# facebookresearch/faiss

Hardware: NVIDIA B200
Metric: queries/sec (GpuIndexFlatL2 exact k-NN, recall@k = 1) (higher is better)
Workload: dtype f16 mma (fp32 accumulate) + f32 exact re-rank

## Files before the change

faiss_b200/__init__.py:

```python
import ctypes
import json
import os

import numpy as np

from ._lib import lib, check, FaissError

METRIC_INNER_PRODUCT = 0
METRIC_L2 = 1

_c_f = ctypes.POINTER(ctypes.c_float)
_c_i64 = ctypes.POINTER(ctypes.c_int64)
_c_u8 = ctypes.POINTER(ctypes.c_uint8)


def _is_torch(x):
    return type(x).__module__.startswith("torch")


def _ptr(x, ctype):
    if x is None:
        return ctypes.cast(None, ctype)
    if _is_torch(x):
        assert x.is_contiguous(), "tensor must be contiguous"
        return ctypes.cast(x.data_ptr(), ctype)
    assert x.flags["C_CONTIGUOUS"], "array must be C-contiguous"
    return x.ctypes.data_as(ctype)


def _as_f32(x):
    if _is_torch(x):
        import torch

        assert x.dtype == torch.float32
        return x.contiguous()
    return np.ascontiguousarray(x, dtype=np.float32)


def _as_i64(x):
    if x is None:
        return None
    if _is_torch(x):
        import torch

        assert x.dtype == torch.int64
        return x.contiguous()
    return np.ascontiguousarray(x, dtype=np.int64)


def _empty_like_residency(x, shape, dtype):
    if _is_torch(x) and x.is_cuda:
        import torch

        tdt = {np.float32: torch.float32, np.int64: torch.int64}[dtype]
        return torch.empty(shape, dtype=tdt, device=x.device)
    return np.empty(shape, dtype=dtype)


class StandardGpuResources:

    def __init__(self):
        self._h = ctypes.c_void_p()
        check(lib.faiss_StandardGpuResources_new(ctypes.byref(self._h)))

    def __del__(self):
        if getattr(self, "_h", None) and lib is not None:
            lib.faiss_StandardGpuResources_free(self._h)
            self._h = None

    def noTempMemory(self):
        check(lib.faiss_StandardGpuResources_noTempMemory(self._h))

    def setTempMemory(self, size):
        check(lib.faiss_StandardGpuResources_setTempMemory(self._h, ctypes.c_size_t(size)))

    def setPinnedMemory(self, size):
        check(lib.faiss_StandardGpuResources_setPinnedMemory(self._h, ctypes.c_size_t(size)))

    def setDefaultStream(self, device, stream):
        check(lib.faiss_StandardGpuResources_setDefaultStream(self._h, int(device), ctypes.c_void_p(int(stream))))

    def setDefaultNullStreamAllDevices(self):
        check(lib.faiss_StandardGpuResources_setDefaultNullStreamAllDevices(self._h))

    def getDefaultStream(self, device):
        out = ctypes.c_void_p()
        check(lib.faiss_StandardGpuResources_getDefaultStream(self._h, int(device), ctypes.byref(out)))
        return out.value or 0

    def syncDefaultStream(self, device):
        check(lib.faiss_StandardGpuResources_syncDefaultStream(self._h, int(device)))

    def getMemoryInfo(self):
        buf = ctypes.create_string_buffer(1 << 16)
        check(lib.faiss_StandardGpuResources_getMemoryInfo(self._h, buf, ctypes.c_size_t(len(buf))))
        raw = json.loads(buf.value.decode())
        return {int(d): {k: tuple(v) for k, v in m.items()} for d, m in raw.items()}

    def ncclInitAll(self, devices):
        arr = (ctypes.c_int * len(devices))(*[int(d) for d in devices])
        check(lib.faiss_StandardGpuResources_ncclInitAll(self._h, len(devices), arr))

    def ncclInitRank(self, device, nranks, rank, unique_id):
        unique_id = bytes(unique_id)
        assert len(unique_id) == 128
        check(lib.faiss_StandardGpuResources_ncclInitRank(self._h, int(device), int(nranks), int(rank), unique_id))

    def ncclRank(self, device):
        r, n = ctypes.c_int(), ctypes.c_int()
        check(lib.faiss_StandardGpuResources_ncclRank(self._h, int(device), ctypes.byref(r), ctypes.byref(n)))
        return r.value, n.value

    def getTempMemoryAvailable(self, device):
        out = ctypes.c_size_t()
        check(lib.faiss_StandardGpuResources_getTempMemoryAvailable(self._h, int(device), ctypes.byref(out)))
        return out.value


class Index:

    def __init__(self):
        self._h = ctypes.c_void_p()
        self._keep = []

    def __del__(self):
        if getattr(self, "_h", None) and lib is not None:
            lib.faiss_Index_free(self._h)
            self._h = None

    def _use_torch_stream(self, *tensors):
        for t in tensors:
            if t is not None and _is_torch(t) and t.is_cuda:
                import torch

                dev = t.device.index if t.device.index is not None else torch.cuda.current_device()
                for r in self._resources():
                    r.setDefaultStream(dev, torch.cuda.current_stream(dev).cuda_stream)
                return

    def _resources(self):
        return [r for r in self._keep if isinstance(r, StandardGpuResources)]

    @property
    def d(self):
        return lib.faiss_Index_d(self._h)

    @property
    def ntotal(self):
        return lib.faiss_Index_ntotal(self._h)

    @property
    def is_trained(self):
        return bool(lib.faiss_Index_is_trained(self._h))

    @property
    def metric_type(self):
        return lib.faiss_Index_metric_type(self._h)

    @property
    def verbose(self):
        return bool(lib.faiss_Index_verbose(self._h))

    @verbose.setter
    def verbose(self, v):
        lib.faiss_Index_set_verbose(self._h, int(bool(v)))

    def _check_x(self, x):
        x = _as_f32(x)
        assert x.ndim == 2 and x.shape[1] == self.d, "x must be [n, d=%d], got %s" % (self.d, tuple(x.shape))
        return x

    def train(self, x):
        x = self._check_x(x)
        self._use_torch_stream(x)
        check(lib.faiss_Index_train(self._h, ctypes.c_int64(x.shape[0]), _ptr(x, _c_f)))

    def add(self, x):
        x = self._check_x(x)
        self._use_torch_stream(x)
        check(lib.faiss_Index_add(self._h, ctypes.c_int64(x.shape[0]), _ptr(x, _c_f)))

    def add_with_ids(self, x, ids):
        x = self._check_x(x)
        ids = _as_i64(ids)
        assert ids.shape == (x.shape[0],)
        self._use_torch_stream(x, ids)
        check(lib.faiss_Index_add_with_ids(self._h, ctypes.c_int64(x.shape[0]), _ptr(x, _c_f), _ptr(ids, _c_i64)))

    def setMinPagingSize(self, size):
        check(lib.faiss_GpuIndex_setMinPagingSize(self._h, ctypes.c_size_t(size)))

    def getMinPagingSize(self):
        out = ctypes.c_size_t()
        check(lib.faiss_GpuIndex_getMinPagingSize(self._h, ctypes.byref(out)))
        return int(out.value)

    def search(self, x, k, D=None, I=None, params=None):
        x = self._check_x(x)
        n = x.shape[0]
        if D is None:
            D = _empty_like_residency(x, (n, k), np.float32)
        if I is None:
            I = _empty_like_residency(x, (n, k), np.int64)
        self._use_torch_stream(x, D, I)
        if params is not None:
            check(
                lib.faiss_Index_search_with_params(
                    self._h, ctypes.c_int64(n), _ptr(x, _c_f), ctypes.c_int64(k), params._h, _ptr(D, _c_f), _ptr(I, _c_i64)
                )
            )
            return D, I
        check(
            lib.faiss_Index_search(
                self._h, ctypes.c_int64(n), _ptr(x, _c_f), ctypes.c_int64(k), _ptr(D, _c_f), _ptr(I, _c_i64)
            )
        )
        return D, I

    def assign(self, x, k=1):
        x = self._check_x(x)
        n = x.shape[0]
        I = _empty_like_residency(x, (n, k), np.int64)
        self._use_torch_stream(x)
        check(lib.faiss_Index_assign(self._h, ctypes.c_int64(n), _ptr(x, _c_f), _ptr(I, _c_i64), ctypes.c_int64(k)))
        return I

    def reset(self):
        check(lib.faiss_Index_reset(self._h))

    def reconstruct(self, key):
        out = np.empty(self.d, dtype=np.float32)
        check(lib.faiss_Index_reconstruct(self._h, ctypes.c_int64(key), _ptr(out, _c_f)))
        return out

    def reconstruct_n(self, i0=0, ni=-1):
        if ni < 0:
            ni = self.ntotal - i0
        out = np.empty((ni, self.d), dtype=np.float32)
        check(lib.faiss_Index_reconstruct_n(self._h, ctypes.c_int64(i0), ctypes.c_int64(ni), _ptr(out, _c_f)))
        return out

    def reconstruct_batch(self, keys):
        keys = _as_i64(np.asarray(keys))
        out = np.empty((keys.shape[0], self.d), dtype=np.float32)
        check(lib.faiss_Index_reconstruct_batch(self._h, ctypes.c_int64(keys.shape[0]), _ptr(keys, _c_i64), _ptr(out, _c_f)))
        return out

    def compute_residual(self, x, key):
        x = _as_f32(x).reshape(1, -1)
        return self.compute_residual_n(x, np.array([key], dtype=np.int64))[0]

    def compute_residual_n(self, x, keys):
        x = self._check_x(x)
        keys = _as_i64(keys)
        out = _empty_like_residency(x, tuple(x.shape), np.float32)
        self._use_torch_stream(x, keys)
        check(
            lib.faiss_Index_compute_residual_n(
                self._h, ctypes.c_int64(x.shape[0]), _ptr(x, _c_f), _ptr(out, _c_f), _ptr(keys, _c_i64)
            )
        )
        return out


class SearchParametersIVF:

    def __init__(self, nprobe=1, max_codes=0):
        self._h = ctypes.c_void_p()
        check(lib.faiss_SearchParametersIVF_new_with(ctypes.byref(self._h), ctypes.c_size_t(int(nprobe)), ctypes.c_size_t(int(max_codes))))

    def __del__(self):
        if getattr(self, "_h", None) and lib is not None:
            lib.faiss_SearchParameters_free(self._h)
            self._h = None


_INTERRUPT_CB = None


def set_interrupt_callback(fn):
    global _INTERRUPT_CB
    proto = ctypes.CFUNCTYPE(ctypes.c_int, ctypes.c_void_p)
    if fn is None:
        lib.faiss_b200_set_interrupt_callback(ctypes.cast(None, proto), None)
        _INTERRUPT_CB = None
        return
    _INTERRUPT_CB = proto(lambda _ctx: 1 if fn() else 0)
    lib.faiss_b200_set_interrupt_callback(_INTERRUPT_CB, None)


class GpuIndexFlat(Index):

    def __init__(self, res, d, metric=METRIC_L2, device=0, use_tensor_cores=True, use_float16=False):
        super().__init__()
        self._keep.append(res)
        check(
            lib.faiss_GpuIndexFlat_new_with_config(
                ctypes.byref(self._h), res._h, int(d), int(metric), int(device), int(bool(use_tensor_cores)),
                int(bool(use_float16)),
            )
        )

    def copyFrom(self, xb):
        xb = _as_f32(xb)
        check(lib.faiss_GpuIndexFlat_copyFrom(self._h, ctypes.c_int64(xb.shape[0]), _ptr(xb, _c_f)))

    def copyTo(self):
        out = np.empty((self.ntotal, self.d), dtype=np.float32)
        check(lib.faiss_GpuIndexFlat_copyTo(self._h, _ptr(out, _c_f)))
        return out

    def setUseTensorCores(self, enable):
        check(lib.faiss_GpuIndexFlat_setUseTensorCores(self._h, int(bool(enable))))

    def lastSearchInfo(self):
        out = (ctypes.c_int * 2)()
        check(lib.faiss_GpuIndexFlat_lastSearchInfo(self._h, out))
        return {"tensor_cores": int(out[0]), "fallback_queries": int(out[1])}


class GpuIndexFlatL2(GpuIndexFlat):
    def __init__(self, res, d, device=0, use_tensor_cores=True, use_float16=False):
        super().__init__(res, d, METRIC_L2, device, use_tensor_cores, use_float16)


class GpuIndexFlatIP(GpuIndexFlat):
    def __init__(self, res, d, device=0, use_tensor_cores=True, use_float16=False):
        super().__init__(res, d, METRIC_INNER_PRODUCT, device, use_tensor_cores, use_float16)


class GpuIndexIVF(Index):

    @property
    def nprobe(self):
        return lib.faiss_GpuIndexIVF_nprobe(self._h)

    @nprobe.setter
    def nprobe(self, v):
        check(lib.faiss_GpuIndexIVF_set_nprobe(self._h, ctypes.c_size_t(int(v))))

    @property
    def nlist(self):
        return lib.faiss_GpuIndexIVF_nlist(self._h)

    def setClustering(self, niter=-1, seed=-1, max_points_per_centroid=-1):
        check(lib.faiss_GpuIndexIVF_set_clustering(self._h, int(niter), int(seed), int(max_points_per_centroid)))

    def reserveMemory(self, n):
        check(lib.faiss_GpuIndexIVF_reserveMemory(self._h, ctypes.c_size_t(int(n))))

    def reclaimMemory(self):
        out = ctypes.c_size_t()
        check(lib.faiss_GpuIndexIVF_reclaimMemory(self._h, ctypes.byref(out)))
        return out.value

    def getListLength(self, l):
        return lib.faiss_GpuIndexIVF_get_list_size(self._h, ctypes.c_size_t(int(l)))

    def _code_size(self):
        raise NotImplementedError

    def getListVectorData(self, l):
        n = self.getListLength(l)
        out = np.empty(n * self._code_size(), dtype=np.uint8)
        check(lib.faiss_GpuIndexIVF_getListVectorData(self._h, ctypes.c_size_t(int(l)), _ptr(out, _c_u8)))
        return out

    def getListIndices(self, l):
        n = self.getListLength(l)
        out = np.empty(n, dtype=np.int64)
        check(lib.faiss_GpuIndexIVF_getListIndices(self._h, ctypes.c_size_t(int(l)), _ptr(out, _c_i64)))
        return out

    def setCoarseCentroids(self, c):
        c = _as_f32(c)
        assert tuple(c.shape) == (self.nlist, self.d)
        check(lib.faiss_GpuIndexIVF_setCoarseCentroids(self._h, _ptr(c, _c_f)))

    def getCoarseCentroids(self):
        out = np.empty((self.nlist, self.d), dtype=np.float32)
        check(lib.faiss_GpuIndexIVF_getCoarseCentroids(self._h, _ptr(out, _c_f)))
        return out

    def setList(self, l, codes, ids):
        codes = np.ascontiguousarray(codes, dtype=np.uint8).reshape(-1)
        ids = np.ascontiguousarray(ids, dtype=np.int64)
        assert codes.size == ids.size * self._code_size()
        check(
            lib.faiss_GpuIndexIVF_setList(
                self._h, ctypes.c_size_t(int(l)), ctypes.c_int64(ids.size), _ptr(codes, _c_u8), _ptr(ids, _c_i64)
            )
        )

    def setListSizes(self, lens):
        lens = np.ascontiguousarray(lens, dtype=np.int64)
        assert lens.shape == (self.nlist,)
        check(lib.faiss_GpuIndexIVF_setListSizes(self._h, _ptr(lens, _c_i64)))

    def setIsTrained(self, v=True):
        check(lib.faiss_GpuIndexIVF_set_is_trained(self._h, int(bool(v))))

    def search_preassigned(self, x, k, assign, centroid_dis=None):
        x = self._check_x(x)
        n = x.shape[0]
        assign = _as_i64(assign)
        if centroid_dis is None:
            centroid_dis = np.zeros(assign.shape, dtype=np.float32)
            if _is_torch(x) and x.is_cuda:
                import torch

                centroid_dis = torch.zeros(tuple(assign.shape), dtype=torch.float32, device=x.device)
        centroid_dis = _as_f32(centroid_dis)
        D = _empty_like_residency(x, (n, k), np.float32)
        I = _empty_like_residency(x, (n, k), np.int64)
        self._use_torch_stream(x, assign)
        check(
            lib.faiss_GpuIndexIVF_search_preassigned(
                self._h,
                ctypes.c_int64(n),
                _ptr(x, _c_f),
                ctypes.c_int64(k),
                _ptr(assign, _c_i64),
                _ptr(centroid_dis, _c_f),
                _ptr(D, _c_f),
                _ptr(I, _c_i64),
            )
        )
        return D, I


class GpuIndexIVFFlat(GpuIndexIVF):

    def __init__(self, res, d, nlist, metric=METRIC_L2, device=0, quantizer=None):
        super().__init__()
        self._keep.append(res)
        if quantizer is not None:
            self._keep.append(quantizer)
            check(
                lib.faiss_GpuIndexIVFFlat_new_with_quantizer(
                    ctypes.byref(self._h), res._h, quantizer._h, int(d), ctypes.c_int64(nlist), int(metric), int(device)
                )
            )
            return
        check(
            lib.faiss_GpuIndexIVFFlat_new(
                ctypes.byref(self._h), res._h, int(d), ctypes.c_int64(nlist), int(metric), int(device)
            )
        )

    def _code_size(self):
        return 4 * self.d


class GpuIndexIVFPQ(GpuIndexIVF):

    def __init__(self, res, d, nlist, M, nbits=8, metric=METRIC_L2, device=0, quantizer=None):
        super().__init__()
        self._keep.append(res)
        self.M = int(M)
        if quantizer is not None:
            self._keep.append(quantizer)
            check(
                lib.faiss_GpuIndexIVFPQ_new_with_quantizer(
                    ctypes.byref(self._h), res._h, quantizer._h, int(d), ctypes.c_int64(nlist), ctypes.c_int64(M), ctypes.c_int64(nbits),
                    int(metric), int(device),
                )
            )
            return
        check(
            lib.faiss_GpuIndexIVFPQ_new(
                ctypes.byref(self._h),
                res._h,
                int(d),
                ctypes.c_int64(nlist),
                ctypes.c_int64(M),
                ctypes.c_int64(nbits),
                int(metric),
                int(device),
            )
        )

    def _code_size(self):
        return self.M

    def setPQCentroids(self, c):
        c = _as_f32(c)
        assert c.size == 256 * self.d
        check(lib.faiss_GpuIndexIVFPQ_setPQCentroids(self._h, _ptr(c, _c_f)))

    def getPQCentroids(self):
        out = np.empty((self.M, 256, self.d // self.M), dtype=np.float32)
        check(lib.faiss_GpuIndexIVFPQ_getPQCentroids(self._h, _ptr(out, _c_f)))
        return out

    def setPQClustering(self, niter=-1, seed=-1, max_points_per_centroid=-1):
        check(lib.faiss_GpuIndexIVFPQ_set_pq_clustering(self._h, int(niter), int(seed), int(max_points_per_centroid)))

    def setPrecomputedCodes(self, enable):
        check(lib.faiss_GpuIndexIVFPQ_setPrecomputedCodes(self._h, int(bool(enable))))


class IndexShards(Index):

    def __init__(self, d, threaded=False, successive_ids=True):
        super().__init__()
        check(
            lib.faiss_IndexShards_new_with_options(
                ctypes.byref(self._h), ctypes.c_int64(d), int(bool(threaded)), int(bool(successive_ids))
            )
        )
        self._shards = []

    def add_shard(self, index):
        check(lib.faiss_IndexShards_add_shard(self._h, index._h))
        self._shards.append(index)

    def _resources(self):
        out = []
        for s in self._shards:
            out.extend(s._resources())
        return out

    def remove_shard(self, index):
        check(lib.faiss_IndexShards_remove_shard(self._h, index._h))
        self._shards.remove(index)

    def at(self, i):
        return self._shards[i]

    def count(self):
        return len(self._shards)

    def lastSearchPath(self):
        return {0: "host", 1: "nccl"}.get(lib.faiss_IndexShards_lastSearchPath(self._h), "?")

    def __del__(self):
        if getattr(self, "_h", None) and lib is not None:
            lib.faiss_Index_free(self._h)
            self._h = None
        self._shards = []


class IndexShardsIVF(IndexShards):

    def __init__(self, quantizer, nlist, threaded=False, successive_ids=True):
        Index.__init__(self)
        self._keep.append(quantizer)
        check(lib.faiss_IndexShardsIVF_new(ctypes.byref(self._h), quantizer._h, ctypes.c_int64(nlist), int(bool(threaded)), int(bool(successive_ids))))
        self._shards = []

    def add_shard(self, index):
        check(lib.faiss_IndexShardsIVF_add_shard(self._h, index._h))
        self._shards.append(index)


def nccl_unique_id():
    buf = ctypes.create_string_buffer(128)
    check(lib.faiss_b200_nccl_unique_id(buf))
    return buf.raw


class DistributedIndexShards(Index):

    def __init__(self, res, local, successive_ids=True):
        super().__init__()
        self._keep.append(res)
        self._local = local
        check(lib.faiss_DistributedIndexShards_new(ctypes.byref(self._h), res._h, local._h, int(bool(successive_ids))))

    def _resources(self):
        return [r for r in self._keep if isinstance(r, StandardGpuResources)]

    def sync(self):
        check(lib.faiss_DistributedIndexShards_sync(self._h))

    def info(self):
        r, n, o = ctypes.c_int(), ctypes.c_int(), ctypes.c_int64()
        check(lib.faiss_DistributedIndexShards_info(self._h, ctypes.byref(r), ctypes.byref(n), ctypes.byref(o)))
        return {"rank": r.value, "world": n.value, "id_offset": o.value}

    def __del__(self):
        if getattr(self, "_h", None) and lib is not None:
            lib.faiss_Index_free(self._h)
            self._h = None
        self._local = None


def kmeans(res, x, k, niter=25, seed=1234, max_points_per_centroid=256, device=0):
    x = _as_f32(x)
    n, d = x.shape
    cent = np.empty((k, d), dtype=np.float32)
    obj = np.zeros(niter, dtype=np.float32)
    check(
        lib.faiss_b200_kmeans(
            res._h,
            int(device),
            ctypes.c_size_t(d),
            ctypes.c_size_t(n),
            ctypes.c_size_t(k),
            _ptr(x, _c_f),
            int(niter),
            int(seed),
            int(max_points_per_centroid),
            _ptr(cent, _c_f),
            _ptr(obj, _c_f),
        )
    )
    return cent, obj


def kmeans_ex(res, x, k, niter=25, seed=1234, max_points_per_centroid=256, metric=METRIC_L2, spherical=False, device=0):
    x = _as_f32(x)
    n, d = x.shape
    cent = np.empty((k, d), dtype=np.float32)
    obj = np.zeros(niter, dtype=np.float32)
    check(
        lib.faiss_b200_kmeans_ex(
            res._h, int(device), ctypes.c_size_t(d), ctypes.c_size_t(n), ctypes.c_size_t(k), _ptr(x, _c_f), int(niter), int(seed),
            int(max_points_per_centroid), int(metric), int(bool(spherical)), _ptr(cent, _c_f), _ptr(obj, _c_f),
        )
    )
# ... 147 lines not shown
```

faiss_b200/csrc/c_api.cu:

```cuda
#include <cstring>
#include <sstream>

#include "comm.h"
#include "faiss_b200_c.h"
#include "index.h"

using namespace fb200;

static thread_local std::string g_last_error;

#define CATCH_AND_HANDLE                              \
    catch (const fb200::FaissException& e) {          \
        g_last_error = e.what();                      \
        return -2;                                    \
    }                                                 \
    catch (const std::exception& e) {                 \
        g_last_error = e.what();                      \
        return -4;                                    \
    }                                                 \
    catch (...) {                                     \
        g_last_error = "unknown exception";           \
        return -1;                                    \
    }                                                 \
    return 0;

struct FaissStandardGpuResources_H {
    std::shared_ptr<StandardGpuResources> res;
};
struct FaissIndex_H {
    Index* index;
    std::shared_ptr<StandardGpuResources> res;
};

static Index* IX(const FaissIndex* p) {
    if (!p || !p->index)
        FB_THROW_MSG("null index handle");
    return p->index;
}
template <typename T>
static T* AS(const FaissIndex* p, const char* what) {
    T* t = dynamic_cast<T*>(IX(p));
    if (!t)
        FB_THROW_FMT("index handle is not a %s", what);
    return t;
}
static std::shared_ptr<StandardGpuResources> RES(FaissStandardGpuResources* r) {
    if (!r || !r->res)
        FB_THROW_MSG("null resources handle");
    return r->res;
}
static MetricType MT(FaissMetricType m) {
    if (m != ::METRIC_L2 && m != ::METRIC_INNER_PRODUCT)
        FB_THROW_MSG("unsupported metric type");
    return m == ::METRIC_L2 ? fb200::METRIC_L2 : fb200::METRIC_INNER_PRODUCT;
}

extern "C" {

const char* faiss_get_last_error(void) {
    return g_last_error.c_str();
}
const char* faiss_b200_version(void) {
    return "faiss_b200 0.1 (sm_100a)";
}

int faiss_StandardGpuResources_new(FaissStandardGpuResources** p) {
    try {
        auto* h = new FaissStandardGpuResources_H();
        h->res = std::make_shared<StandardGpuResources>();
        *p = h;
    }
    CATCH_AND_HANDLE
}
void faiss_StandardGpuResources_free(FaissStandardGpuResources* r) {
    delete r;
}
int faiss_StandardGpuResources_noTempMemory(FaissStandardGpuResources* r) {
    try {
        RES(r)->noTempMemory();
    }
    CATCH_AND_HANDLE
}
int faiss_StandardGpuResources_setTempMemory(FaissStandardGpuResources* r, size_t size) {
    try {
        RES(r)->setTempMemory(size);
    }
    CATCH_AND_HANDLE
}
int faiss_StandardGpuResources_setPinnedMemory(FaissStandardGpuResources* r, size_t size) {
    try {
        RES(r)->setPinnedMemory(size);
    }
    CATCH_AND_HANDLE
}
int faiss_StandardGpuResources_setDefaultStream(FaissStandardGpuResources* r, int device, void* stream) {
    try {
        RES(r)->setDefaultStream(device, (cudaStream_t)stream);
    }
    CATCH_AND_HANDLE
}
int faiss_StandardGpuResources_setDefaultNullStreamAllDevices(FaissStandardGpuResources* r) {
    try {
        RES(r)->setDefaultNullStreamAllDevices();
    }
    CATCH_AND_HANDLE
}
int faiss_StandardGpuResources_getDefaultStream(FaissStandardGpuResources* r, int device, void** out) {
    try {
        *out = (void*)RES(r)->getDefaultStream(device);
    }
    CATCH_AND_HANDLE
}
int faiss_StandardGpuResources_syncDefaultStream(FaissStandardGpuResources* r, int device) {
    try {
        DeviceScope s(device);
        RES(r)->syncDefaultStream(device);
    }
    CATCH_AND_HANDLE
}
int faiss_StandardGpuResources_getMemoryInfo(FaissStandardGpuResources* r, char* buf, size_t buflen) {
    try {
        auto info = RES(r)->getMemoryInfo();
        std::ostringstream os;
        os << "{";
        bool firstD = true;
        for (auto& dv : info) {
            if (!firstD)
                os << ",";
            firstD = false;
            os << "\"" << dv.first << "\":{";
            bool first = true;
            for (auto& kv : dv.second) {
                if (!first)
                    os << ",";
                first = false;
                os << "\"" << kv.first << "\":[" << kv.second.first << "," << kv.second.second << "]";
            }
            os << "}";
        }
        os << "}";
        std::string s = os.str();
        FB_THROW_IF_NOT_MSG(s.size() + 1 <= buflen, "buffer too small");
        memcpy(buf, s.c_str(), s.size() + 1);
    }
    CATCH_AND_HANDLE
}
int faiss_StandardGpuResources_getTempMemoryAvailable(FaissStandardGpuResources* r, int device, size_t* out) {
    try {
        RES(r)->initializeForDevice(device);
        *out = RES(r)->getTempMemoryAvailable(device);
    }
    CATCH_AND_HANDLE
}

void faiss_Index_free(FaissIndex* p) {
    if (p) {
        delete p->index;
        delete p;
    }
}
int faiss_Index_d(const FaissIndex* p) {
    return p && p->index ? p->index->d : 0;
}
int faiss_Index_is_trained(const FaissIndex* p) {
    return p && p->index ? (int)p->index->is_trained : 0;
}
idx_t faiss_Index_ntotal(const FaissIndex* p) {
    return p && p->index ? p->index->ntotal : 0;
}
FaissMetricType faiss_Index_metric_type(const FaissIndex* p) {
    return p && p->index && p->index->metric_type == fb200::METRIC_INNER_PRODUCT ? ::METRIC_INNER_PRODUCT : ::METRIC_L2;
}
int faiss_Index_verbose(const FaissIndex* p) {
    return p && p->index ? (int)p->index->verbose : 0;
}
void faiss_Index_set_verbose(FaissIndex* p, int v) {
    if (p && p->index)
        p->index->verbose = v != 0;
}
int faiss_Index_train(FaissIndex* p, idx_t n, const float* x) {
    try {
        IX(p)->train(n, x);
    }
    CATCH_AND_HANDLE
}
int faiss_Index_add(FaissIndex* p, idx_t n, const float* x) {
    try {
        IX(p)->add(n, x);
    }
    CATCH_AND_HANDLE
}
int faiss_Index_add_with_ids(FaissIndex* p, idx_t n, const float* x, const idx_t* xids) {
    try {
        IX(p)->add_with_ids(n, x, xids);
    }
    CATCH_AND_HANDLE
}
int faiss_Index_search(const FaissIndex* p, idx_t n, const float* x, idx_t k, float* D, idx_t* I) {
    try {
        IX(p)->search(n, x, k, D, I);
    }
    CATCH_AND_HANDLE
}
int faiss_Index_assign(FaissIndex* p, idx_t n, const float* x, idx_t* labels, idx_t k) {
    try {
        IX(p)->assign(n, x, labels, k);
    }
    CATCH_AND_HANDLE
}
int faiss_Index_reset(FaissIndex* p) {
    try {
        IX(p)->reset();
    }
    CATCH_AND_HANDLE
}
int faiss_Index_reconstruct(const FaissIndex* p, idx_t key, float* out) {
    try {
        IX(p)->reconstruct(key, out);
    }
    CATCH_AND_HANDLE
}
int faiss_Index_reconstruct_n(const FaissIndex* p, idx_t i0, idx_t ni, float* out) {
    try {
        IX(p)->reconstruct_n(i0, ni, out);
    }
    CATCH_AND_HANDLE
}
int faiss_Index_reconstruct_batch(const FaissIndex* p, idx_t n, const idx_t* keys, float* out) {
    try {
        IX(p)->reconstruct_batch(n, keys, out);
    }
    CATCH_AND_HANDLE
}
int faiss_Index_compute_residual(const FaissIndex* p, const float* x, float* r, idx_t key) {
    try {
        IX(p)->compute_residual(x, r, key);
    }
    CATCH_AND_HANDLE
}
int faiss_Index_compute_residual_n(const FaissIndex* p, idx_t n, const float* x, float* r, const idx_t* keys) {
    try {
        IX(p)->compute_residual_n(n, x, r, keys);
    }
    CATCH_AND_HANDLE
}

int faiss_GpuIndexFlat_new(
        FaissGpuIndex** p,
        FaissStandardGpuResources* r,
        int d,
        FaissMetricType metric,
        int device,
        int use_tc) {
    try {
        GpuIndexFlatConfig c;
        c.device = device;
        c.useTensorCores = use_tc != 0;
        auto res = RES(r);
        auto* h = new FaissIndex_H();
        h->res = res;
        h->index = new GpuIndexFlat(res, d, MT(metric), c);
        *p = h;
    }
    CATCH_AND_HANDLE
}
int faiss_GpuIndexFlat_new_with_config(
        FaissGpuIndex** p,
        FaissStandardGpuResources* r,
        int d,
        FaissMetricType metric,
        int device,
        int use_tc,
        int use_float16) {
    try {
        GpuIndexFlatConfig c;
        c.device = device;
        c.useTensorCores = use_tc != 0;
        c.useFloat16 = use_float16 != 0;
        auto res = RES(r);
        auto* h = new FaissIndex_H();
        h->res = res;
        h->index = new GpuIndexFlat(res, d, MT(metric), c);
        *p = h;
    }
    CATCH_AND_HANDLE
}
int faiss_GpuIndexFlatL2_new(FaissGpuIndex** p, FaissStandardGpuResources* r, int d, int device) {
    return faiss_GpuIndexFlat_new(p, r, d, ::METRIC_L2, device, 1);
}
int faiss_GpuIndexFlatIP_new(FaissGpuIndex** p, FaissStandardGpuResources* r, int d, int device) {
    return faiss_GpuIndexFlat_new(p, r, d, ::METRIC_INNER_PRODUCT, device, 1);
}
int faiss_GpuIndexFlat_copyFrom(FaissGpuIndex* p, idx_t n, const float* xb) {
    try {
        AS<GpuIndexFlat>(p, "GpuIndexFlat")->copyFrom(n, xb);
    }
    CATCH_AND_HANDLE
}
int faiss_GpuIndexFlat_copyTo(const FaissGpuIndex* p, float* out) {
    try {
        AS<GpuIndexFlat>(p, "GpuIndexFlat")->copyTo(out);
    }
    CATCH_AND_HANDLE
}
int faiss_GpuIndex_setMinPagingSize(FaissGpuIndex* p, size_t size) {
    try {
        AS<GpuIndex>(p, "GpuIndex")->setMinPagingSize(size);
    }
    CATCH_AND_HANDLE
}
int faiss_GpuIndex_getMinPagingSize(const FaissGpuIndex* p, size_t* out) {
    try {
        *out = AS<GpuIndex>(p, "GpuIndex")->getMinPagingSize();
    }
    CATCH_AND_HANDLE
}
int faiss_GpuIndexFlat_setUseTensorCores(FaissGpuIndex* p, int enable) {
    try {
        AS<GpuIndexFlat>(p, "GpuIndexFlat")->setUseTensorCores(enable != 0);
    }
    CATCH_AND_HANDLE
}
int faiss_GpuIndexFlat_lastSearchInfo(const FaissGpuIndex* p, int* out2) {
    try {
        auto* f = AS<GpuIndexFlat>(p, "GpuIndexFlat");
        out2[0] = f->lastSearchUsedTensorCores;
        out2[1] = f->lastSearchFallbackQueries;
    }
    CATCH_AND_HANDLE
}

int faiss_GpuIndexIVF_set_nprobe(FaissGpuIndex* p, size_t nprobe) {
    try {
        AS<GpuIndexIVF>(p, "GpuIndexIVF")->nprobe = nprobe;
    }
    CATCH_AND_HANDLE
}
size_t faiss_GpuIndexIVF_nprobe(const FaissGpuIndex* p) {
    auto* i = p ? dynamic_cast<GpuIndexIVF*>(p->index) : nullptr;
    return i ? i->nprobe : 0;
}
size_t faiss_GpuIndexIVF_nlist(const FaissGpuIndex* p) {
    auto* i = p ? dynamic_cast<GpuIndexIVF*>(p->index) : nullptr;
    return i ? (size_t)i->nlist : 0;
}
int faiss_GpuIndexIVF_set_clustering(FaissGpuIndex* p, int niter, int seed, int maxppc) {
    try {
        auto* i = AS<GpuIndexIVF>(p, "GpuIndexIVF");
        if (niter > 0)
            i->cp.niter = niter;
        if (seed >= 0)
            i->cp.seed = seed;
        if (maxppc > 0)
            i->cp.max_points_per_centroid = maxppc;
    }
    CATCH_AND_HANDLE
}
int faiss_GpuIndexIVF_reserveMemory(FaissGpuIndex* p, size_t n) {
    try {
        AS<GpuIndexIVF>(p, "GpuIndexIVF")->reserveMemory(n);
    }
    CATCH_AND_HANDLE
}
int faiss_GpuIndexIVF_reclaimMemory(FaissGpuIndex* p, size_t* out) {
    try {
        size_t r = AS<GpuIndexIVF>(p, "GpuIndexIVF")->reclaimMemory();
        if (out)
            *out = r;
    }
    CATCH_AND_HANDLE
}
size_t faiss_GpuIndexIVF_get_list_size(const FaissGpuIndex* p, size_t l) {
    auto* i = p ? dynamic_cast<GpuIndexIVF*>(p->index) : nullptr;
    if (!i || (idx_t)l >= i->nlist)
        return 0;
    return (size_t)i->getListLength((idx_t)l);
}
int faiss_GpuIndexIVF_getListVectorData(const FaissGpuIndex* p, size_t l, uint8_t* out) {
    try {
        auto v = AS<GpuIndexIVF>(p, "GpuIndexIVF")->getListVectorData((idx_t)l);
        if (!v.empty())
            memcpy(out, v.data(), v.size());
    }
    CATCH_AND_HANDLE
}
int faiss_GpuIndexIVF_getListIndices(const FaissGpuIndex* p, size_t l, idx_t* out) {
    try {
        auto v = AS<GpuIndexIVF>(p, "GpuIndexIVF")->getListIndices((idx_t)l);
        if (!v.empty())
            memcpy(out, v.data(), v.size() * sizeof(idx_t));
    }
    CATCH_AND_HANDLE
}
int faiss_GpuIndexIVF_setCoarseCentroids(FaissGpuIndex* p, const float* c) {
    try {
        AS<GpuIndexIVF>(p, "GpuIndexIVF")->setCoarseCentroids(c);
    }
    CATCH_AND_HANDLE
}
int faiss_GpuIndexIVF_getCoarseCentroids(const FaissGpuIndex* p, float* out) {
    try {
        AS<GpuIndexIVF>(p, "GpuIndexIVF")->getCoarseCentroids(out);
    }
    CATCH_AND_HANDLE
}
int faiss_GpuIndexIVF_setList(FaissGpuIndex* p, size_t l, idx_t len, const uint8_t* codes, const idx_t* ids) {
    try {
        AS<GpuIndexIVF>(p, "GpuIndexIVF")->setList((idx_t)l, len, codes, ids);
    }
    CATCH_AND_HANDLE
}
int faiss_GpuIndexIVF_setListSizes(FaissGpuIndex* p, const idx_t* lens) {
    try {
        AS<GpuIndexIVF>(p, "GpuIndexIVF")->setListSizes(lens);
    }
    CATCH_AND_HANDLE
}
int faiss_GpuIndexIVF_set_is_trained(FaissGpuIndex* p, int v) {
    try {
        AS<GpuIndexIVF>(p, "GpuIndexIVF")->is_trained = v != 0;
    }
    CATCH_AND_HANDLE
}
int faiss_GpuIndexIVF_search_preassigned(
        const FaissGpuIndex* p,
        idx_t n,
        const float* x,
        idx_t k,
        const idx_t* assign,
        const float* cdis,
        float* D,
        idx_t* I) {
    try {
        AS<GpuIndexIVF>(p, "GpuIndexIVF")->search_preassigned(n, x, k, assign, cdis, D, I);
    }
    CATCH_AND_HANDLE
}
int faiss_GpuIndexIVFFlat_new(
        FaissGpuIndex** p,
        FaissStandardGpuResources* r,
        int d,
        idx_t nlist,
        FaissMetricType metric,
        int device) {
    try {
        GpuIndexIVFConfig c;
        c.device = device;
        auto res = RES(r);
        auto* h = new FaissIndex_H();
        h->res = res;
        h->index = new GpuIndexIVFFlat(res, d, nlist, MT(metric), c);
        *p = h;
    }
    CATCH_AND_HANDLE
}

int faiss_GpuIndexIVFPQ_new(
        FaissGpuIndex** p,
        FaissStandardGpuResources* r,
        int d,
        idx_t nlist,
        idx_t M,
        idx_t nbits,
        FaissMetricType metric,
        int device) {
    try {
        GpuIndexIVFPQConfig c;
        c.device = device;
        auto res = RES(r);
        auto* h = new FaissIndex_H();
        h->res = res;
        h->index = new GpuIndexIVFPQ(res, d, nlist, M, nbits, MT(metric), c);
        *p = h;
    }
    CATCH_AND_HANDLE
}
int faiss_GpuIndexIVFPQ_setPQCentroids(FaissGpuIndex* p, const float* c) {
    try {
        AS<GpuIndexIVFPQ>(p, "GpuIndexIVFPQ")->setPQCentroids(c);
    }
    CATCH_AND_HANDLE
}
int faiss_GpuIndexIVFPQ_getPQCentroids(const FaissGpuIndex* p, float* out) {
    try {
        AS<GpuIndexIVFPQ>(p, "GpuIndexIVFPQ")->getPQCentroids(out);
    }
    CATCH_AND_HANDLE
}
int faiss_GpuIndexIVFPQ_set_pq_clustering(FaissGpuIndex* p, int niter, int seed, int maxppc) {
    try {
        auto* i = AS<GpuIndexIVFPQ>(p, "GpuIndexIVFPQ");
        if (niter > 0)
            i->pq_cp.niter = niter;
        if (seed >= 0)
            i->pq_cp.seed = seed;
        if (maxppc > 0)
            i->pq_cp.max_points_per_centroid = maxppc;
    }
    CATCH_AND_HANDLE
}
int faiss_GpuIndexIVFPQ_setPrecomputedCodes(FaissGpuIndex* p, int enable) {
    try {
        AS<GpuIndexIVFPQ>(p, "GpuIndexIVFPQ")->setPrecomputedCodes(enable != 0);
    }
    CATCH_AND_HANDLE
}

int faiss_IndexShards_new(FaissIndexShards** p, idx_t d) {
    return faiss_IndexShards_new_with_options(p, d, 0, 1);
}
int faiss_IndexShards_new_with_options(FaissIndexShards** p, idx_t d, int threaded, int successive_ids) {
    try {
        auto* h = new FaissIndex_H();
        h->index = new IndexShards((int)d, threaded != 0, successive_ids != 0);
        *p = h;
    }
    CATCH_AND_HANDLE
}
int faiss_IndexShards_add_shard(FaissIndexShards* p, FaissIndex* shard) {
    try {
        AS<IndexShards>(p, "IndexShards")->add_shard(IX(shard));
    }
    CATCH_AND_HANDLE
}
int faiss_IndexShards_remove_shard(FaissIndexShards* p, FaissIndex* shard) {
    try {
        AS<IndexShards>(p, "IndexShards")->remove_shard(IX(shard));
    }
    CATCH_AND_HANDLE
}
FaissIndex* faiss_IndexShards_at(FaissIndexShards*, int) {
    return nullptr;
}
int faiss_IndexShards_own_indices(const FaissIndexShards* p) {
    auto* s = p ? dynamic_cast<IndexShards*>(p->index) : nullptr;
    return s ? (int)s->own_indices : 0;
}
void faiss_IndexShards_set_own_indices(FaissIndexShards* p, int v) {
    (void)p;
    (void)v;
}
int faiss_IndexShards_successive_ids(const FaissIndexShards* p) {
    auto* s = p ? dynamic_cast<IndexShards*>(p->index) : nullptr;
    return s ? (int)s->successive_ids : 0;
}
void faiss_IndexShards_set_successive_ids(FaissIndexShards* p, int v) {
    auto* s = p ? dynamic_cast<IndexShards*>(p->index) : nullptr;
    if (s)
        s->successive_ids = v != 0;
}

struct FaissSearchParameters_H {
    SearchParameters* p;
};
int faiss_SearchParametersIVF_new_with(FaissSearchParametersIVF** out, size_t nprobe, size_t max_codes) {
    try {
        auto* sp = new SearchParametersIVF();
        sp->nprobe = nprobe;
        sp->max_codes = max_codes;
        *out = new FaissSearchParameters_H{sp};
    }
    CATCH_AND_HANDLE
}
void faiss_SearchParameters_free(FaissSearchParameters* p) {
    if (p) {
        delete p->p;
        delete p;
    }
}
int faiss_Index_search_with_params(
        const FaissIndex* p, idx_t n, const float* x, idx_t k, const FaissSearchParameters* params, float* D, idx_t* I) {
    try {
        Index* ix = IX(p);
        if (!params || !params->p) {
            ix->search(n, x, k, D, I);
        } else if (auto* g = dynamic_cast<GpuIndex*>(ix)) {
            g->search(n, x, k, D, I, params->p);
        } else {
            FB_THROW_MSG("search parameters are only supported on GPU indexes");
        }
    }
    CATCH_AND_HANDLE
}
void faiss_b200_set_interrupt_callback(int (*want_interrupt)(void*), void* ctx) {
    InterruptCallback::set(want_interrupt, ctx);
}
int faiss_GpuIndexIVFFlat_new_with_quantizer(
        FaissGpuIndex** p, FaissStandardGpuResources* r, FaissGpuIndex* coarse, int d, idx_t nlist, FaissMetricType metric, int device) {
    try {
        auto res = RES(r);
        GpuIndexIVFConfig cfg;
        cfg.device = device;
        auto* h = new FaissIndex_H{nullptr, res};
        try {
            h->index = new GpuIndexIVFFlat(res, AS<GpuIndexFlat>(coarse, "GpuIndexFlat"), d, nlist, MT(metric), cfg);
        } catch (...) {
            delete h;
            throw;
        }
        *p = h;
    }
    CATCH_AND_HANDLE
}
int faiss_GpuIndexIVFPQ_new_with_quantizer(
        FaissGpuIndex** p,
        FaissStandardGpuResources* r,
        FaissGpuIndex* coarse,
        int d,
        idx_t nlist,
        idx_t M,
        idx_t nbits,
        FaissMetricType metric,
        int device) {
    try {
        auto res = RES(r);
        GpuIndexIVFPQConfig cfg;
        cfg.device = device;
        auto* h = new FaissIndex_H{nullptr, res};
        try {
            h->index = new GpuIndexIVFPQ(res, AS<GpuIndexFlat>(coarse, "GpuIndexFlat"), d, nlist, M, nbits, MT(metric), cfg);
        } catch (...) {
            delete h;
            throw;
        }
        *p = h;
    }
    CATCH_AND_HANDLE
}

int faiss_b200_nccl_unique_id(char* out128) {
// ... 543 lines not shown
```

faiss_b200/csrc/flat_tc.cu:

```cuda
#include <cuda_fp16.h>

#include <cfloat>
#include <cmath>
#include <cub/cub.cuh>
#include <cstdlib>
#include <mutex>
#include <string>
#include <vector>

#include "comm.h"
#include "kernels.h"
#include "select.cuh"
#include "tc_ptx.cuh"
#include "flat_tc_kernel.cuh"

namespace fb200 {

void runMergeTopKKeyspace(
        const float*, const idx_t*, int64_t, int, int, int, MetricType, int64_t, float*, idx_t*, cudaStream_t);

namespace {

using namespace tc;

// ... 397 lines not shown
        }
    }
    if (lane == 0) {
        thr[q] = tNew;
        if (overflow)
            flags[q] = 1;
    }
}

__global__ void tc_pooled_thr_kernel(int nq, const float* __restrict__ contrib, const float* __restrict__ eps, float* __restrict__ thr) {
    const int q = blockIdx.x * blockDim.x + threadIdx.x;
    if (q >= nq)
        return;
    const float T = fmaxf(contrib[q], -contrib[nq + q]);
    if (T > -CUDART_INF_F) {
        const float t = nextafterf(T - eps[q], -CUDART_INF_F);
        thr[q] = fmaxf(thr[q], t);
    }
}

template <bool IS_L2, bool YH>
__global__ void tc_rerank_kernel(
        int nq,
        int d,
        int k,
        int LIST,
        int KL,
        const float* __restrict__ Q,
        const void* __restrict__ Y,
        const int* __restrict__ perm,
        const int* __restrict__ baseId,
        const float* __restrict__ baseKey,
        const float* __restrict__ thr,
        float* __restrict__ outD,
        idx_t* __restrict__ outI) {
    extern __shared__ __align__(16) unsigned char smem_raw[];
    const int warp = threadIdx.x >> 5;
    const int lane = lane_id();
    const int q = blockIdx.x * (blockDim.x >> 5) + warp;
    if (q >= nq)
        return;
    constexpr int BUF = 64;
    unsigned char* base = smem_raw + SmemTopK<int>::bytes(KL, BUF) * warp;
    WarpTopK<int> w;
    w.init(reinterpret_cast<float*>(base), reinterpret_cast<int*>(base + sizeof(float) * (KL + BUF)), KL, BUF, k);
    const float* qp = Q + (int64_t)q * d;
    const int* bi = baseId + (int64_t)q * LIST;
    const float tq = thr ? thr[q] : -CUDART_INF_F;
    for (int e0 = 0; e0 < LIST; e0 += 32) {
        int id = bi[e0 + lane];
        const bool present = id != IdLimits<int>::max();
        bool valid = present;
        if (valid && thr)
            valid = -baseKey[(int64_t)q * LIST + e0 + lane] > tq;
        if (valid && perm)
            id = perm[id];
        float acc = 0.f;
        if (valid) {
            const int64_t yo = (int64_t)id * d;
            int i = 0;
            if ((d & 3) == 0) {
#pragma unroll 8
                for (; i < d; i += 4) {
                    const float4 a4 = *reinterpret_cast<const float4*>(qp + i);
                    const float4 b4 = row_load4<YH>(Y, yo + i);
                    const float aa[4] = {a4.x, a4.y, a4.z, a4.w};
                    const float bb[4] = {b4.x, b4.y, b4.z, b4.w};
#pragma unroll
                    for (int u = 0; u < 4; u++) {
                        if (IS_L2) {
                            float df = aa[u] - bb[u];
                            acc = fmaf(df, df, acc);
                        } else {
                            acc = fmaf(aa[u], bb[u], acc);
                        }
                    }
                }
            }
            for (; i < d; i++) {
                float a = qp[i], b = row_load1<YH>(Y, yo + i);
                if (IS_L2) {
                    float df = a - b;
                    acc = fmaf(df, df, acc);
                } else {
                    acc = fmaf(a, b, acc);
                }
            }
            if (!IS_L2)
                acc = -acc;
        }
        if (!__any_sync(kFullMask, present))
            break;
        w.add(valid, acc, id);
    }
    w.finish();
    for (int j = lane; j < k; j += 32) {
        int id = w.q.ids[j];
        bool ok = id != IdLimits<int>::max();
        float key = w.q.keys[j];
        outD[(int64_t)q * k + j] = ok ? (IS_L2 ? key : -key) : (IS_L2 ? FLT_MAX : -FLT_MAX);
        outI[(int64_t)q * k + j] = ok ? (idx_t)id : -1;
    }
}

__global__ void tc_init_base_kernel(float* baseKey, int* baseId, int64_t count) {
    int64_t i = (int64_t)blockIdx.x * blockDim.x + threadIdx.x;
    if (i < count) {
        baseKey[i] = CUDART_INF_F;
        baseId[i] = IdLimits<int>::max();
    }
}

template <bool IS_L2, bool YH>
__global__ void tc_argmin_finish_kernel(
        int nq,
        int d,
        int slices,
        int parts,
        const uint2* __restrict__ cand,
        int cap,
        const int* __restrict__ candCount,
        const float* __restrict__ eps,
        const float* __restrict__ Q,
        const void* __restrict__ Y,
        const int* __restrict__ perm,
        float* __restrict__ outD,
        idx_t* __restrict__ outI,
        int* __restrict__ flags) {
    const int warp = threadIdx.x >> 5;
    const int lane = lane_id();
    const int q = blockIdx.x * (blockDim.x >> 5) + warp;
    if (q >= nq)
        return;
    const int pair = q / kPairM, prow = q % kPairM;
    const int qPairs = (nq + kPairM - 1) / kPairM;
    const int nseg = slices * parts;
    float m = -CUDART_INF_F;
    int overflow = 0;
    for (int si = 0; si < nseg; si++) {
        const int s = si / parts, h = si - s * parts;
        const long long seg = ((long long)(s * qPairs + pair) * kPairM + prow) * parts + h;
        int c = candCount[seg];
        if (c > cap) {
            overflow = 1;
            c = cap;
        }
        const uint2* sp = cand + seg * cap;
        for (int e = lane; e < c; e += 32)
            m = fmaxf(m, __uint_as_float(sp[e].x));
    }
#pragma unroll
    for (int o = 16; o > 0; o >>= 1)
        m = fmaxf(m, __shfl_xor_sync(kFullMask, m, o));
    const float t = nextafterf(m - 2.f * eps[q], -CUDART_INF_F);
    float bestD = CUDART_INF_F;
    int bestI = IdLimits<int>::max();
    const float* qp = Q + (int64_t)q * d;
    for (int si = 0; si < nseg; si++) {
        const int s = si / parts, h = si - s * parts;
        const long long seg = ((long long)(s * qPairs + pair) * kPairM + prow) * parts + h;
        const int c = min(candCount[seg], cap);
        const uint2* sp = cand + seg * cap;
        for (int e0 = 0; e0 < c; e0 += 32) {
            const int e = e0 + lane;
            const uint2 v = e < c ? sp[e] : make_uint2(0, 0);
            if (e < c && __uint_as_float(v.x) > t) {
                int id = (int)v.y;
                if (perm)
                    id = perm[id];
                const int64_t yo = (int64_t)id * d;
                float acc = 0.f;
                for (int i = 0; i < d; i++) {
                    const float a = qp[i], b = row_load1<YH>(Y, yo + i);
                    if (IS_L2) {
                        const float df = a - b;
                        acc = fmaf(df, df, acc);
                    } else {
                        acc = fmaf(a, b, acc);
                    }
                }
                if (!IS_L2)
                    acc = -acc;
                if (acc < bestD || (acc == bestD && id < bestI)) {
                    bestD = acc;
                    bestI = id;
                }
            }
        }
    }
#pragma unroll
    for (int o = 16; o > 0; o >>= 1) {
        const float od = __shfl_xor_sync(kFullMask, bestD, o);
        const int oi = __shfl_xor_sync(kFullMask, bestI, o);
        if (od < bestD || (od == bestD && oi < bestI)) {
            bestD = od;
            bestI = oi;
        }
    }
    if (lane == 0) {
        const bool ok = bestI != IdLimits<int>::max();
        outD[q] = ok ? (IS_L2 ? bestD : -bestD) : (IS_L2 ? FLT_MAX : -FLT_MAX);
        outI[q] = ok ? (idx_t)bestI : -1;
        if (overflow || !ok)
            flags[q] = 1;
    }
}

__global__ void tc_collect_flags_kernel(const int* flags, int nq, int* list, int* count) {
    int q = blockIdx.x * blockDim.x + threadIdx.x;
    if (q < nq && flags[q]) {
        int pos = atomicAdd(count, 1);
        list[pos] = q;
    }
}
__global__ void tc_gather_queries_kernel(const float* Q, const int* list, int d, float* out) {
    int i = blockIdx.x;
    int q = list[i];
    for (int j = threadIdx.x; j < d; j += blockDim.x)
        out[(int64_t)i * d + j] = Q[(int64_t)q * d + j];
}
__global__ void tc_scatter_results_kernel(
        const float* D,
        const idx_t* I,
        const int* list,
        int k,
        float* outD,
        idx_t* outI) {
    int i = blockIdx.x;
    int q = list[i];
    for (int j = threadIdx.x; j < k; j += blockDim.x) {
        outD[(int64_t)q * k + j] = D[(int64_t)i * k + j];
        outI[(int64_t)q * k + j] = I[(int64_t)i * k + j];
    }
}

typedef CUresult (*PFN_encodeTiled)(
        CUtensorMap*,
        CUtensorMapDataType,
        cuuint32_t,
        void*,
        const cuuint64_t*,
        const cuuint64_t*,
        const cuuint32_t*,
        const cuuint32_t*,
        CUtensorMapInterleave,
        CUtensorMapSwizzle,
        CUtensorMapL2promotion,
        CUtensorMapFloatOOBfill);

PFN_encodeTiled getEncodeTiled() {
    static PFN_encodeTiled fn = nullptr;
    static std::once_flag once;
    std::call_once(once, [] {
        void* p = nullptr;
        cudaDriverEntryPointQueryResult qres;
        cudaError_t err = cudaGetDriverEntryPoint("cuTensorMapEncodeTiled", &p, cudaEnableDefault, &qres);
        if (err == cudaSuccess && qres == cudaDriverEntryPointSuccess)
            fn = reinterpret_cast<PFN_encodeTiled>(p);
    });
    FB_THROW_IF_NOT_MSG(fn != nullptr, "cuTensorMapEncodeTiled not available from the driver");
    return fn;
}

CUtensorMap makeTileMap(const __half* base, int64_t rows, int dpad, int boxRows, int boxK = 0) {
    CUtensorMap m;
    cuuint64_t dims[3] = {(cuuint64_t)kKBlock, (cuuint64_t)rows, (cuuint64_t)(dpad / kKBlock)};
    cuuint64_t strides[2] = {(cuuint64_t)dpad * 2, (cuuint64_t)kKBlock * 2};
    cuuint32_t box[3] = {(cuuint32_t)kKBlock, (cuuint32_t)boxRows, (cuuint32_t)(boxK > 0 ? boxK : dpad / kKBlock)};
    cuuint32_t estr[3] = {1, 1, 1};
    CUresult r = getEncodeTiled()(
            &m,
            CU_TENSOR_MAP_DATA_TYPE_FLOAT16,
            3,
            const_cast<__half*>(base),
            dims,
            strides,
            box,
            estr,
            CU_TENSOR_MAP_INTERLEAVE_NONE,
            CU_TENSOR_MAP_SWIZZLE_128B,
            CU_TENSOR_MAP_L2_PROMOTION_L2_256B,
            CU_TENSOR_MAP_FLOAT_OOB_FILL_NONE);
    FB_THROW_IF_NOT_FMT(r == CUDA_SUCCESS, "cuTensorMapEncodeTiled failed with %d", (int)r);
    return m;
}

unsigned long long gcd64(unsigned long long a, unsigned long long b) {
    while (b) {
        unsigned long long t = a % b;
        a = b;
        b = t;
    }
    return a;
}

struct SmemPlan {
    int yStages;
    size_t bytes;
    int ksplit;
};

constexpr int kMaxKB = 4;

SmemPlan planSmem(int KB) {
    const size_t qtiles = (size_t)2 * KB * kTileM * kKBlock * 2;
    const size_t fixed = 1024  + 512  + qtiles;
    if (KB <= 2) {
        const size_t stage = (size_t)KB * kTileN * kKBlock * 2;
        const size_t budget = 220 * 1024;
        int ys = (int)std::min<size_t>(kMaxYStages, (budget - fixed) / stage);
        return {ys, fixed + ys * stage, 0};
    }
    FB_THROW_IF_NOT_MSG(KB <= kMaxKB, "dimension too large for the tensor-core Flat kernel");
    const size_t stage = (size_t)kTileN * kKBlock * 2;
    const size_t budget = 226 * 1024;
    int ys = (int)std::min<size_t>(kMaxYStages, (budget - fixed) / stage);
    FB_THROW_IF_NOT(ys >= 3);
    return {ys, fixed + ys * stage, 1};
}

int tcParts() {
    static const int parts = getenv("FB200_TC_PARTS") ? atoi(getenv("FB200_TC_PARTS")) : 4;
    return parts == 2 ? 2 : 4;
}

template <bool DUMP>
void launchTc(const CUtensorMap& mq, const CUtensorMap& my, const TcParams& p, int grid, size_t smem, cudaStream_t stream, bool self = false) {
    static const bool dbg = getenv("FB200_TC_DEBUG_SKIP") && atoi(getenv("FB200_TC_DEBUG_SKIP")) != 0;
    const int parts = tcParts();
    auto kern = parts == 2 ? (dbg ? flat_tc_kernel<DUMP, 1, 2> : flat_tc_kernel<DUMP, 0, 2>)
                           : (dbg ? flat_tc_kernel<DUMP, 1, 4> : flat_tc_kernel<DUMP, 0, 4>);
    if (self && !DUMP)
        kern = parts == 2 ? flat_tc_kernel<false, 0, 2, true> : flat_tc_kernel<false, 0, 4, true>;
    CUDA_VERIFY(cudaFuncSetAttribute(kern, cudaFuncAttributeMaxDynamicSharedMemorySize, (int)smem));
    KernelTiming::begin("flat_tc", stream);
    kern<<<grid, tcThreads(parts), smem, stream>>>(mq, my, p);
    KernelTiming::end("flat_tc", stream);
    CUDA_CHECK_LAST();
}

}

void runAbsMax(const void* x, int64_t count, float* out, cudaStream_t stream, int yHalf) {
    if (count == 0)
        return;
    int blocks = (int)std::min<int64_t>(1184, ceil_div(count, 256));
    absmax_kernel<<<blocks, 256, 0, stream>>>(x, yHalf, count, out);
    CUDA_CHECK_LAST();
}

void runMaxOf(const float* x, int64_t count, float* out, cudaStream_t stream) {
    runAbsMax(x, count, out, stream, 0);
}

void runFlatTcPrepareRows(
        GpuResources* res,
        int device,
        const void* Y,
        int64_t n,
        int d,
        int dpad,
        float scale,
        MetricType metric,
        __half* Y16,
        float* bias,
        int* perm,
        float* tileMaxBias,
        float* norms,
        cudaStream_t stream,
        int yHalf) {
    if (n == 0)
        return;
    const int warps = 8;
    const unsigned rowBlocks = (unsigned)ceil_div(n, warps);
    const int isL2 = metric == METRIC_L2 ? 1 : 0;
    tc_prepare_rows_kernel<<<rowBlocks, warps * 32, 0, stream>>>(Y, yHalf, n, d, dpad, scale, isL2, nullptr, nullptr, nullptr, norms);
    CUDA_CHECK_LAST();
    if (perm) {
        auto keysOut = res->temp(device, sizeof(float) * n);
        auto valsIn = res->temp(device, sizeof(int) * n);
        tc_iota_kernel<<<(unsigned)ceil_div(n, 256), 256, 0, stream>>>(valsIn.as<int>(), n);
        CUDA_CHECK_LAST();
        size_t tmpBytes = 0;
        CUDA_VERIFY(cub::DeviceRadixSort::SortPairs(
                nullptr, tmpBytes, norms, keysOut.as<float>(), valsIn.as<int>(), perm, (int)n, 0, 32, stream));
        auto tmp = res->temp(device, tmpBytes);
        CUDA_VERIFY(cub::DeviceRadixSort::SortPairs(
                tmp.data, tmpBytes, norms, keysOut.as<float>(), valsIn.as<int>(), perm, (int)n, 0, 32, stream));
    }
    tc_prepare_rows_kernel<<<rowBlocks, warps * 32, 0, stream>>>(Y, yHalf, n, d, dpad, scale, isL2, perm, Y16, bias, nullptr);
    CUDA_CHECK_LAST();
    const int64_t numTiles = ceil_div(n, kTileN);
    tc_tile_max_bias_kernel<<<(unsigned)ceil_div(numTiles, warps), warps * 32, 0, stream>>>(bias, numTiles, tileMaxBias);
    CUDA_CHECK_LAST();
}

bool flatTcSupported(int d, int k, int64_t n) {
    int dpad = (int)round_up(d, kKBlock);
    return dpad <= kMaxKB * kKBlock && k >= 1 && k <= 2048 && n >= (k == 1 ? 2048 : 32768) && n < (int64_t(1) << 31) - 512;
}

void runFlatTcScoresDebug(
        const __half* Q16,
        int64_t nq,
        const __half* Y16,
        int64_t n,
        int dpad,
        float* S,
        cudaStream_t stream) {
    FB_THROW_IF_NOT(dpad % kKBlock == 0 && dpad <= kMaxKB * kKBlock);
    const int KB = dpad / kKBlock;
    SmemPlan sp = planSmem(KB);
    CUtensorMap my = makeTileMap(Y16, n, dpad, kTileN, sp.ksplit);
    const int64_t numTiles = ceil_div(n, kTileN);
    const int64_t qPairs = ceil_div(nq, kPairM);
    __half* qpad = nullptr;
    CUDA_VERIFY(cudaMallocAsync(&qpad, sizeof(__half) * qPairs * kPairM * dpad, stream));
    CUDA_VERIFY(cudaMemsetAsync(qpad, 0, sizeof(__half) * qPairs * kPairM * dpad, stream));
    CUDA_VERIFY(cudaMemcpyAsync(qpad, Q16, sizeof(__half) * nq * dpad, cudaMemcpyDeviceToDevice, stream));
    float* one = nullptr;
    CUDA_VERIFY(cudaMallocAsync(&one, sizeof(float), stream));
    float h1 = 1.f;
    CUDA_VERIFY(cudaMemcpyAsync(one, &h1, sizeof(float), cudaMemcpyHostToDevice, stream));
    TcParams p{};
    p.slices = 1;
    p.qPairs = (int)qPairs;
    p.numUnits = (int)qPairs;
    CUtensorMap mq = makeTileMap(qpad, qPairs * kPairM, dpad, kTileM);
    p.tileBegin = 0;
    p.tileEnd = (int)numTiles;
    p.tilesPerSlice = (int)numTiles;
    p.permA = 1;
    p.permB = 0;
    p.numTiles = (unsigned long long)numTiles;
    p.KB = KB;
    p.ksplit = sp.ksplit;
    p.kSteps = dpad / 16;
    p.yStages = sp.yStages;
    p.invScalePtr = one;
    p.bias = nullptr;
    p.tileMaxBias = nullptr;
    p.thr = nullptr;
    p.cand = nullptr;
    p.cap = 0;
    p.candCount = nullptr;
    p.dump = S;
    p.dumpLd = numTiles * kTileN;
    p.nq = (int)nq;
    int dev = 0, sms = 0;
    CUDA_VERIFY(cudaGetDevice(&dev));
    CUDA_VERIFY(cudaDeviceGetAttribute(&sms, cudaDevAttrMultiProcessorCount, dev));
    launchTc<true>(mq, my, p, (int)std::min<int64_t>(p.numUnits, sms), sp.bytes, stream);
    CUDA_VERIFY(cudaFreeAsync(qpad, stream));
    CUDA_VERIFY(cudaFreeAsync(one, stream));
}

void runFlatTcSearch(
        GpuResources* res,
        int device,
        const float* Q,
        int64_t nqAll,
        const void* Y,
        const __half* Y16,
        const float* bias,
        const int* perm,
        const float* tileMaxBias,
        float yScale,
        float yMaxNorm,
        int64_t n,
        int d,
        int dpad,
        int k,
        MetricType metric,
        float* outD,
        idx_t* outI,
        cudaStream_t stream,
        const FlatTcShard* shard,
        int yHalf) {
    if (nqAll == 0)
        return;
    FB_THROW_IF_NOT(flatTcSupported(d, k, n));
    const int KB = dpad / kKBlock;
    const SmemPlan sp = planSmem(KB);
    const int sms = res->numSMs(device);
    const int64_t T = ceil_div(n, kTileN);
    const int nShards = shard ? shard->comm->size() : 1;
    const int64_t Tsched = shard ? std::max<int64_t>(T, shard->maxTiles) : T;
    const int kFrac = (k + nShards - 1) / nShards;
    const int LIST = std::max(128, next_pow2(2 * k));
    const int KL = std::max(64, next_pow2(k));

    unsigned long long A = (unsigned long long)((double)T * 0.6180339887498949);
    if (A < 1)
        A = 1;
    while (gcd64(A, (unsigned long long)T) != 1)
        A++;
    const unsigned long long B = (unsigned long long)(T / 3);

    const float c1 = 1.01f * (ldexpf(1.f, -10) + (float)dpad * ldexpf(1.f, -22));
    const float c2 = (float)(dpad + 16) * ldexpf(1.f, -24);

    CUtensorMap mapY = makeTileMap(Y16, n, dpad, kTileN, sp.ksplit);

    static const int r0Env = getenv("FB200_TC_R0") ? atoi(getenv("FB200_TC_R0")) : 0;
    int r0Tiles = std::max(r0Env > 0 ? r0Env : std::max(1, (40 * k + kTileN - 1) / kTileN), (k + 127) / 128 * 2);
    if (nShards > 1)
        r0Tiles = std::max<int>((r0Tiles + nShards - 1) / nShards, std::max(2, (2 * kFrac + kTileN - 1) / kTileN));
    static const bool selSortEnv = getenv("FB200_TC_SELECT") && std::string(getenv("FB200_TC_SELECT")) == "sort";
    const bool useBisect = LIST <= 256 && !selSortEnv;
    if (useBisect)
        r0Tiles = std::min(r0Tiles, std::max(2, kSelCap * 3 / 4 / kTileN));
    static const bool noStream = getenv("FB200_TC_NO_STREAM") && atoi(getenv("FB200_TC_NO_STREAM")) != 0;
    const bool streaming = k == 1 && !shard && !noStream;
    const int64_t kQFloor = r0Tiles > 64 ? 2048 : 16384;
    const int64_t kQBatch = streaming ? (int64_t)sms * kPairM * 4
                                      : std::min<int64_t>(131072, std::max<int64_t>(kQFloor, (int64_t)kPairM * 1024 / r0Tiles));
    for (int64_t qb = 0; qb < nqAll; qb += kQBatch) {
        const int64_t nq = std::min(kQBatch, nqAll - qb);
        const float* Qb = Q + qb * d;
        const int64_t qPairs = ceil_div(nq, kPairM);

        auto q16 = res->temp(device, sizeof(__half) * qPairs * kPairM * dpad);
        auto scal = res->temp(device, sizeof(float) * 4);
        auto eps = res->temp(device, sizeof(float) * nq);
        auto thr = res->temp(device, sizeof(float) * nq);
        auto flags = res->temp(device, sizeof(int) * (nq + 1));
        auto baseKey = res->temp(device, streaming ? sizeof(float) : sizeof(float) * nq * LIST);
        auto baseId = res->temp(device, streaming ? sizeof(int) : sizeof(int) * nq * LIST);

        CUDA_VERIFY(cudaMemsetAsync(scal.data, 0, sizeof(float) * 4, stream));
        CUDA_VERIFY(cudaMemsetAsync(flags.data, 0, sizeof(int) * (nq + 1), stream));
        CUDA_VERIFY(cudaMemsetAsync(q16.data, 0, sizeof(__half) * qPairs * kPairM * dpad, stream));
        float* sc = scal.as<float>();
        runAbsMax(Qb, nq * d, sc + 0, stream);
        tc_query_scale_kernel<<<1, 1, 0, stream>>>(sc + 0, yScale, sc + 1, sc + 2);
        CUDA_CHECK_LAST();
        tc_prepare_queries_kernel<<<(unsigned)ceil_div(nq, 8), 256, 0, stream>>>(
                Qb, nq, d, dpad, sc + 1, c1, c2, yMaxNorm, q16.as<__half>(), eps.as<float>(), thr.as<float>());
        CUDA_CHECK_LAST();
        if (!streaming) {
            int64_t cnt = nq * LIST;
            tc_init_base_kernel<<<(unsigned)ceil_div(cnt, 256), 256, 0, stream>>>(
                    baseKey.as<float>(), baseId.as<int>(), cnt);
            CUDA_CHECK_LAST();
        }

        struct Round {
            int begin, end, slices, tilesPerSlice, cap;
        };
        const int parts = tcParts();
        std::vector<Round> rounds;
        {
            int64_t seen = 0;
            while (seen < Tsched) {
                static const double gEarly = getenv("FB200_TC_G_EARLY") ? atof(getenv("FB200_TC_G_EARLY")) : 4.0;
                static const double gLate = getenv("FB200_TC_G_LATE") ? atof(getenv("FB200_TC_G_LATE")) : 4.0;
                static const int64_t lateFrom = getenv("FB200_TC_LATE_FROM") ? atol(getenv("FB200_TC_LATE_FROM")) : 8192;
                static const double gShard = getenv("FB200_TC_G_SHARD") ? atof(getenv("FB200_TC_G_SHARD")) : 8.0;
                const double g = nShards > 1 ? std::max(gEarly, std::min(gShard, 2.0 * nShards)) : (seen >= lateFrom ? gLate : gEarly);
                int64_t end = seen == 0 ? std::min<int64_t>(Tsched, r0Tiles)
                                        : std::min<int64_t>(Tsched, (int64_t)(seen * g));
                if (Tsched - end < end / 4)
                    end = Tsched;
                if (streaming)
                    end = Tsched;
                int64_t tiles = end - seen;
                int bestS = 1;
                double bestCost = 1e300;
                int64_t maxS = std::max<int64_t>(1, std::min<int64_t>(512, tiles / 8));
                for (int64_t S = 1; S <= maxS; S++) {
                    int64_t tps = ceil_div(tiles, S);
                    int64_t units = qPairs * ceil_div(tiles, tps);
                    int64_t waves = ceil_div(units, sms);
                    double cost = (double)waves * (double)(tps + 6);
                    if (cost < bestCost * 0.999) {
                        bestCost = cost;
                        bestS = (int)S;
                    }
                }
                int64_t tps = ceil_div(tiles, bestS);
                int S = (int)ceil_div(tiles, tps);
                int cap;
                if (streaming) {
                    cap = 64;
                } else if (seen == 0) {
                    cap = (int)(tps * (kTileN / parts));
                } else {
                    double expect = 1.5 * k * ((double)tps / (double)seen) / parts;
                    cap = next_pow2((int)std::min<double>(1 << 20, 4.0 * expect + 32.0));
                    cap = std::max(cap, 32);
                }
                rounds.push_back({(int)seen, (int)end, S, (int)tps, cap});
                seen = end;
            }
        }
        size_t arenaBytes = 0, countBytes = 0;
        for (auto& r : rounds) {
            size_t units = (size_t)qPairs * r.slices;
            arenaBytes = std::max(arenaBytes, units * tcSegsPerUnit(parts) * (size_t)r.cap * sizeof(uint2));
            countBytes = std::max(countBytes, units * tcSegsPerUnit(parts) * sizeof(int));
        }
        auto arena = res->temp(device, arenaBytes);
        auto counts = res->temp(device, countBytes);

        const int selWarps = (int)std::max<size_t>(1, std::min<size_t>(8, (48 * 1024) / SmemTopK<int>::bytes(LIST, kSelectBuf)));
        const size_t selSmem = SmemTopK<int>::bytes(LIST, kSelectBuf) * selWarps;
        CUDA_VERIFY(cudaFuncSetAttribute(tc_select_kernel, cudaFuncAttributeMaxDynamicSharedMemorySize, (int)selSmem));

        GpuMemoryReservation contrib;
        if (shard)
            contrib = res->temp(device, sizeof(float) * 2 * nq);
        for (auto& r : rounds) {
            TcParams p{};
            p.slices = r.slices;
            p.qPairs = (int)qPairs;
            p.numUnits = (int)(qPairs * r.slices);
            CUtensorMap mapQ = makeTileMap(q16.as<__half>(), qPairs * kPairM, dpad, kTileM);
            p.tileBegin = (int)std::min<int64_t>(r.begin, T);
            p.tileEnd = (int)std::min<int64_t>(r.end, T);
            p.tilesPerSlice = r.tilesPerSlice;
            p.permA = A;
            p.permB = B;
            p.numTiles = (unsigned long long)T;
            p.KB = KB;
            p.ksplit = sp.ksplit;
            p.kSteps = (d + 15) / 16;
            p.yStages = sp.yStages;
            p.invScalePtr = sc + 2;
            p.bias = bias;
            p.tileMaxBias = tileMaxBias;
            p.tileMinBias = tileMaxBias + T + 1;
            p.thr = thr.as<float>();
            p.eps = eps.as<float>();
            p.cand = arena.as<uint2>();
            p.cap = r.cap;
            p.candCount = counts.as<int>();
            p.dump = nullptr;
            p.dumpLd = 0;
            p.nq = (int)nq;
            if (p.tileBegin < p.tileEnd) {
                launchTc<false>(mapQ, mapY, p, std::min(p.numUnits, sms), sp.bytes, stream, streaming);
            } else {
                CUDA_VERIFY(cudaMemsetAsync(counts.data, 0, (size_t)p.numUnits * tcSegsPerUnit(parts) * sizeof(int), stream));
            }
            if (streaming) {
                const int fw = 8;
                float* oD1 = outD + qb;
                idx_t* oI1 = outI + qb;
                KernelTiming::begin("tc_argmin_finish", stream);
                auto launchFin = [&](auto kern) {
                    kern<<<(unsigned)ceil_div(nq, fw), fw * 32, 0, stream>>>(
                            (int)nq, d, r.slices, parts, arena.as<uint2>(), r.cap, counts.as<int>(), eps.as<float>(), Qb, Y, perm,
                            oD1, oI1, flags.as<int>());
                };
                if (metric == METRIC_L2)
                    yHalf ? launchFin(tc_argmin_finish_kernel<true, true>) : launchFin(tc_argmin_finish_kernel<true, false>);
                else
                    yHalf ? launchFin(tc_argmin_finish_kernel<false, true>) : launchFin(tc_argmin_finish_kernel<false, false>);
                KernelTiming::end("tc_argmin_finish", stream);
                CUDA_CHECK_LAST();
                continue;
            }
            KernelTiming::begin("tc_select", stream);
            if (useBisect) {
                const size_t bsmem = sizeof(uint2) * kSelCap * kSelWarps;
                CUDA_VERIFY(cudaFuncSetAttribute(tc_select_bisect_kernel, cudaFuncAttributeMaxDynamicSharedMemorySize, (int)bsmem));
                tc_select_bisect_kernel<<<(unsigned)ceil_div(nq, kSelWarps), kSelWarps * 32, bsmem, stream>>>(
                        (int)nq, k, LIST, r.slices, parts, arena.as<uint2>(), r.cap, counts.as<int>(), eps.as<float>(),
                        baseKey.as<float>(), baseId.as<int>(), thr.as<float>(), flags.as<int>(),
                        shard ? contrib.as<float>() : nullptr, kFrac);
            } else {
                tc_select_kernel<<<(unsigned)ceil_div(nq, selWarps), selWarps * 32, selSmem, stream>>>(
                        (int)nq,
                        k,
                        LIST,
                        r.slices,
                        parts,
                        arena.as<uint2>(),
                        r.cap,
                        counts.as<int>(),
                        eps.as<float>(),
                        baseKey.as<float>(),
                        baseId.as<int>(),
                        thr.as<float>(),
                        flags.as<int>(),
                        shard ? contrib.as<float>() : nullptr,
                        kFrac);
            }
            KernelTiming::end("tc_select", stream);
            CUDA_CHECK_LAST();
            if (shard) {
                KernelTiming::begin("tc_pool", stream);
                shard->comm->allReduceMax(contrib.as<float>(), (size_t)2 * nq, stream);
                tc_pooled_thr_kernel<<<(unsigned)ceil_div(nq, 256), 256, 0, stream>>>(
                        (int)nq, contrib.as<float>(), eps.as<float>(), thr.as<float>());
                KernelTiming::end("tc_pool", stream);
                CUDA_CHECK_LAST();
            }
        }

        if (!streaming) {
            const int rrWarps = (int)std::max<size_t>(1, std::min<size_t>(8, (48 * 1024) / SmemTopK<int>::bytes(KL, 64)));
            const size_t rrSmem = SmemTopK<int>::bytes(KL, 64) * rrWarps;
            float* oD = outD + qb * k;
            idx_t* oI = outI + qb * k;
            auto launchRr = [&](auto kern) {
                CUDA_VERIFY(cudaFuncSetAttribute(kern, cudaFuncAttributeMaxDynamicSharedMemorySize, (int)rrSmem));
                kern<<<(unsigned)ceil_div(nq, rrWarps), rrWarps * 32, rrSmem, stream>>>(
                        (int)nq, d, k, LIST, KL, Qb, Y, perm, baseId.as<int>(), baseKey.as<float>(),
                        shard ? thr.as<float>() : nullptr, oD, oI);
            };
            KernelTiming::begin("tc_rerank", stream);
            if (metric == METRIC_L2)
                yHalf ? launchRr(tc_rerank_kernel<true, true>) : launchRr(tc_rerank_kernel<true, false>);
            else
                yHalf ? launchRr(tc_rerank_kernel<false, true>) : launchRr(tc_rerank_kernel<false, false>);
            KernelTiming::end("tc_rerank", stream);
            CUDA_CHECK_LAST();
        }

        {
            auto list = res->temp(device, sizeof(int) * nq);
            int* countDev = flags.as<int>() + nq;
            tc_collect_flags_kernel<<<(unsigned)ceil_div(nq, 256), 256, 0, stream>>>(
                    flags.as<int>(), (int)nq, list.as<int>(), countDev);
            CUDA_CHECK_LAST();
            int nflag = 0;
            CUDA_VERIFY(cudaMemcpyAsync(&nflag, countDev, sizeof(int), cudaMemcpyDeviceToHost, stream));
            CUDA_VERIFY(cudaStreamSynchronize(stream));
            if (nflag > 0) {
                auto fq = res->temp(device, sizeof(float) * (size_t)nflag * d);
                auto fD = res->temp(device, sizeof(float) * (size_t)nflag * k);
                auto fI = res->temp(device, sizeof(idx_t) * (size_t)nflag * k);
                tc_gather_queries_kernel<<<nflag, 128, 0, stream>>>(Qb, list.as<int>(), d, fq.as<float>());
                CUDA_CHECK_LAST();
                runFlatExact(res, device, fq.as<float>(), nflag, Y, n, d, k, metric, 0, fD.as<float>(), fI.as<idx_t>(), stream, yHalf);
                tc_scatter_results_kernel<<<nflag, 128, 0, stream>>>(
                        fD.as<float>(), fI.as<idx_t>(), list.as<int>(), k, outD + qb * k, outI + qb * k);
                CUDA_CHECK_LAST();
                CUDA_VERIFY(cudaStreamSynchronize(stream));
            }
            lastFlatTcFallbacks() = nflag;
        }
    }
}

int& lastFlatTcFallbacks() {
    static thread_local int v = 0;
    return v;
}

}
```

faiss_b200/csrc/flat_tc_kernel.cuh:

```cuda
#pragma once

#include <cuda_fp16.h>

#include "select.cuh"
#include "tc_ptx.cuh"

namespace fb200 {
namespace tc {

constexpr int kTileM = 128;
constexpr int kPairM = 256;
constexpr int kTileN = 256;
constexpr int kKBlock = 64;
constexpr int kMaxParts = 4;
constexpr int kMaxYStages = 6;
__host__ __device__ constexpr int tcThreads(int parts) {
    return 64 + 128 * parts;
}
__host__ __device__ constexpr int tcSegsPerUnit(int parts) {
    return kPairM * parts;
}

struct TcParams {
    int numUnits;
    int slices;
    int qPairs;
    int tileBegin;
    int tileEnd;
    int tilesPerSlice;
    unsigned long long permA, permB, numTiles;
    int KB;
    int kSteps;
    int ksplit;
    int yStages;
    const float* invScalePtr;
    const float* bias;
    const float* tileMaxBias;
    const float* tileMinBias;
    const float* thr;
    const float* eps;
    uint2* cand;
    int cap;
    int* candCount;
    float* dump;
    long long dumpLd;
    int nq;
};

__device__ __forceinline__ int perm_tile(const TcParams& p, int pos) {
    return (int)(((unsigned long long)pos * p.permA + p.permB) % p.numTiles);
}

template <bool DUMP, bool SELF>
__device__ __forceinline__ void epi_filter32(
        const TcParams& p,
        const uint32_t (&r)[32],
        int q,
        long long colBase,
        float inv,
        float& thr,
        float slack,
        float maxb,
        uint2* buf,
        int& cnt,
        float minb = 0.f) {
    if (DUMP) {
        if (q < p.nq) {
            float* dst = p.dump + (long long)q * p.dumpLd + colBase;
#pragma unroll
            for (int j = 0; j < 32; j++)
                dst[j] = __uint_as_float(r[j]);
        }
        return;
    }
    float mg[4];
#pragma unroll
    for (int g = 0; g < 4; g++) {
        const int o = 8 * g;
        const float a = ptx::max3(__uint_as_float(r[o + 0]), __uint_as_float(r[o + 1]), __uint_as_float(r[o + 2]));
        const float c = ptx::max3(__uint_as_float(r[o + 3]), __uint_as_float(r[o + 4]), __uint_as_float(r[o + 5]));
        mg[g] = ptx::max3(a, c, fmaxf(__uint_as_float(r[o + 6]), __uint_as_float(r[o + 7])));
    }
    const float m = ptx::max3(mg[0], mg[1], fmaxf(mg[2], mg[3]));
    if (SELF) {
        thr = fmaxf(thr, nextafterf(fmaf(m, inv, minb) - slack, -CUDART_INF_F));
    }
    if (fmaf(m, inv, maxb) > thr) {
        const float* bias = p.bias + colBase;
        const unsigned rowBase = (unsigned)colBase;
#pragma unroll
        for (int g = 0; g < 4; g++) {
            if (fmaf(mg[g], inv, maxb) > thr) {
#pragma unroll
                for (int j = 8 * g; j < 8 * g + 8; j++) {
                    const float v = fmaf(__uint_as_float(r[j]), inv, __ldg(bias + j));
                    if (v > thr) {
                        if (cnt < p.cap)
                            buf[cnt] = make_uint2(__float_as_uint(v), rowBase + j);
                        cnt++;
                        if (SELF)
                            thr = fmaxf(thr, nextafterf(v - slack, -CUDART_INF_F));
                    }
                }
            }
        }
    }
}

template <bool DUMP, bool SELF>
__device__ __forceinline__ void epi_filter64(
        const TcParams& p,
        const uint32_t (&r0)[32],
        const uint32_t (&r1)[32],
        int q,
        long long colBase,
        float inv,
        float& thr,
        float slack,
        float maxb,
        uint2* buf,
        int& cnt,
        float minb = 0.f) {
    epi_filter32<DUMP, SELF>(p, r0, q, colBase, inv, thr, slack, maxb, buf, cnt, minb);
    epi_filter32<DUMP, SELF>(p, r1, q, colBase + 32, inv, thr, slack, maxb, buf, cnt, minb);
}

template <bool DUMP, int DBG, int PARTS, bool SELF = false>
__global__ void __launch_bounds__(tcThreads(PARTS), 1) flat_tc_kernel(
        const __grid_constant__ CUtensorMap mapQ,
        const __grid_constant__ CUtensorMap mapY,
        const TcParams p) {
    extern __shared__ unsigned char smem_dyn[];
    unsigned char* smem = reinterpret_cast<unsigned char*>(
            (reinterpret_cast<uintptr_t>(smem_dyn) + 1023) & ~uintptr_t(1023));
    const int qBytes = p.KB * kTileM * kKBlock * 2;
    const int stageBytes = (p.ksplit ? 1 : p.KB) * kTileN * kKBlock * 2;
    unsigned char* sQ = smem;
    unsigned char* sY = smem + 2 * qBytes;
    uint64_t* bars = reinterpret_cast<uint64_t*>(sY + (size_t)p.yStages * stageBytes);
    uint64_t* q_full = bars + 0;
    uint64_t* q_empty = bars + 1;
    uint64_t* y_full = bars + 2;
    uint64_t* y_empty = y_full + kMaxYStages;
    uint64_t* t_full = y_empty + kMaxYStages;
    uint64_t* t_empty = t_full + 2;
    uint32_t* tmem_slot = reinterpret_cast<uint32_t*>(t_empty + 2);

    const int warp = threadIdx.x >> 5;
    const int lane = threadIdx.x & 31;
    constexpr int kEpiWarps = 4 * PARTS;
    constexpr int kColsPerThread = kTileN / PARTS;

    if (warp == 0 && lane == 0) {
        ptx::prefetch_tensormap(&mapQ);
        ptx::prefetch_tensormap(&mapY);
        ptx::mbar_init(q_full, 1);
        ptx::mbar_init(q_empty, 1);
        for (int i = 0; i < p.yStages; i++) {
            ptx::mbar_init(&y_full[i], 1);
            ptx::mbar_init(&y_empty[i], 1);
        }
        for (int i = 0; i < 2; i++) {
            ptx::mbar_init(&t_full[i], 1);
            ptx::mbar_init(&t_empty[i], kEpiWarps);
        }
        ptx::fence_barrier_init();
    }
    if (warp == 1) {
        ptx::tmem_alloc<512>(tmem_slot);
    }
    ptx::tc_fence_before();
    __syncthreads();
    ptx::tc_fence_after();
    const uint32_t tmem_base = *tmem_slot;

    if (warp == 0) {
        if (lane == 0) {
            int ys = 0;
            uint32_t yphase = 0;
            int it = 0;
            for (int u = blockIdx.x; u < p.numUnits; u += gridDim.x, it++) {
                const int pair = u % p.qPairs;
                const int sl = u / p.qPairs;
                ptx::mbar_wait(q_empty, (it & 1) ^ 1);
                ptx::mbar_arrive_expect_tx(q_full, (uint32_t)(2 * qBytes));
                ptx::tma_load_3d(sQ, &mapQ, q_full, 0, pair * kPairM, 0);
                ptx::tma_load_3d(sQ + qBytes, &mapQ, q_full, 0, pair * kPairM + kTileM, 0);
                const int pb = p.tileBegin + sl * p.tilesPerSlice;
                const int pe = min(p.tileEnd, pb + p.tilesPerSlice);
                for (int pp = pb; pp < pe; pp++) {
                    const int t = perm_tile(p, pp);
                    const int loads = p.ksplit ? 2 * p.KB : 1;
                    for (int l = 0; l < loads; l++) {
                        ptx::mbar_wait(&y_empty[ys], yphase ^ 1);
                        ptx::mbar_arrive_expect_tx(&y_full[ys], (uint32_t)stageBytes);
                        ptx::tma_load_3d(sY + (size_t)ys * stageBytes, &mapY, &y_full[ys], 0, t * kTileN, p.ksplit ? l % p.KB : 0);
                        if (++ys == p.yStages) {
                            ys = 0;
                            yphase ^= 1;
                        }
                    }
                }
            }
        }
    } else if (warp == 1) {
        if (lane == 0) {
            constexpr uint32_t idesc = ptx::make_idesc_f16(kTileM, kTileN);
            int ys = 0;
            uint32_t yphase = 0, tphase = 0;
            int it = 0;
            const uint32_t sQaddr = ptx::smem_u32(sQ);
            const uint32_t sYaddr = ptx::smem_u32(sY);
            const int qkb = kTileM * kKBlock * 2;
            const int ykb = kTileN * kKBlock * 2;
            for (int u = blockIdx.x; u < p.numUnits; u += gridDim.x, it++) {
                const int sl = u / p.qPairs;
                const int pb = p.tileBegin + sl * p.tilesPerSlice;
                const int pe = min(p.tileEnd, pb + p.tilesPerSlice);
                ptx::mbar_wait(q_full, it & 1);
                ptx::tc_fence_after();
                for (int pp = pb; pp < pe; pp++) {
                    if (p.ksplit) {
#pragma unroll 1
                        for (int h = 0; h < 2; h++) {
                            ptx::mbar_wait(&t_empty[h], tphase ^ 1);
                            ptx::tc_fence_after();
                            const uint32_t dcol = tmem_base + (uint32_t)h * kTileN;
                            const uint32_t qaddr = sQaddr + (uint32_t)h * (uint32_t)qBytes;
                            for (int kb = 0; kb < p.KB; kb++) {
                                ptx::mbar_wait(&y_full[ys], yphase);
                                ptx::tc_fence_after();
                                const uint32_t yaddr = sYaddr + (uint32_t)ys * (uint32_t)stageBytes;
                                const int k4n = min(4, p.kSteps - 4 * kb);
                                for (int k4 = 0; k4 < k4n; k4++) {
                                    uint64_t da = ptx::make_smem_desc_sw128(qaddr + kb * qkb + k4 * 32);
                                    uint64_t db = ptx::make_smem_desc_sw128(yaddr + k4 * 32);
                                    ptx::mma_f16_ss(dcol, da, db, idesc, (kb | k4) != 0 ? 1u : 0u);
                                }
                                ptx::mma_commit(&y_empty[ys]);
                                if (++ys == p.yStages) {
                                    ys = 0;
                                    yphase ^= 1;
                                }
                            }
                            ptx::mma_commit(&t_full[h]);
                        }
                        tphase ^= 1;
                        continue;
                    }
                    ptx::mbar_wait(&y_full[ys], yphase);
                    ptx::tc_fence_after();
                    const uint32_t yaddr = sYaddr + (uint32_t)ys * (uint32_t)stageBytes;
#pragma unroll 1
                    for (int h = 0; h < 2; h++) {
                        ptx::mbar_wait(&t_empty[h], tphase ^ 1);
                        ptx::tc_fence_after();
                        const uint32_t dcol = tmem_base + (uint32_t)h * kTileN;
                        const uint32_t qaddr = sQaddr + (uint32_t)h * (uint32_t)qBytes;
                        for (int ks = 0; ks < p.kSteps; ks++) {
                            const int kb = ks >> 2, k4 = ks & 3;
                            uint64_t da = ptx::make_smem_desc_sw128(qaddr + kb * qkb + k4 * 32);
                            uint64_t db = ptx::make_smem_desc_sw128(yaddr + kb * ykb + k4 * 32);
                            ptx::mma_f16_ss(dcol, da, db, idesc, ks != 0 ? 1u : 0u);
                        }
                        ptx::mma_commit(&t_full[h]);
                    }
                    ptx::mma_commit(&y_empty[ys]);
                    tphase ^= 1;
                    if (++ys == p.yStages) {
                        ys = 0;
                        yphase ^= 1;
                    }
                }
                ptx::mma_commit(q_empty);
            }
        }
    } else {
        const int ew = warp - 2;
        const int quarter = warp & 3;
        const int half = ew >> 2;
        const int row = quarter * 32 + lane;
        const float inv = *p.invScalePtr;
        const uint32_t lane_acc = tmem_base + ((uint32_t)(quarter * 32) << 16) + (uint32_t)(half * kColsPerThread);
        uint32_t tphase = 0;
        const int permStep = (int)(p.permA % p.numTiles);
        for (int u = blockIdx.x; u < p.numUnits; u += gridDim.x) {
            const int pair = u % p.qPairs;
            const int sl = u / p.qPairs;
            const int q0 = pair * kPairM + row;
            const int q1 = q0 + kTileM;
            float thr0 = (!DUMP && q0 < p.nq) ? p.thr[q0] : CUDART_INF_F;
            float thr1 = (!DUMP && q1 < p.nq) ? p.thr[q1] : CUDART_INF_F;
            const float slack0 = (SELF && q0 < p.nq) ? 2.f * p.eps[q0] : 0.f;
            const float slack1 = (SELF && q1 < p.nq) ? 2.f * p.eps[q1] : 0.f;
            const long long seg0 = ((long long)u * kPairM + row) * PARTS + half;
            const long long seg1 = ((long long)u * kPairM + kTileM + row) * PARTS + half;
            uint2* buf0 = DUMP ? nullptr : p.cand + seg0 * p.cap;
            uint2* buf1 = DUMP ? nullptr : p.cand + seg1 * p.cap;
            int cnt0 = 0, cnt1 = 0;
            const int pb = p.tileBegin + sl * p.tilesPerSlice;
            const int pe = min(p.tileEnd, pb + p.tilesPerSlice);

            uint32_t a0[32], a1[PARTS == 2 ? 32 : 1];
            int t = pb < pe ? perm_tile(p, pb) : 0;
            float maxbNext = (!DUMP && pb < pe) ? __ldg(p.tileMaxBias + t) : 0.f;
            float minbNext = (SELF && pb < pe) ? __ldg(p.tileMinBias + t) : 0.f;
            for (int pp = pb; pp < pe; pp++) {
                const long long colBase = (long long)t * kTileN + half * kColsPerThread;
                const float maxb = maxbNext;
                const float minb = minbNext;
                t += permStep;
                if (t >= (int)p.numTiles)
                    t -= (int)p.numTiles;
                if (!DUMP && pp + 1 < pe)
                    maxbNext = __ldg(p.tileMaxBias + t);
                if (SELF && pp + 1 < pe)
                    minbNext = __ldg(p.tileMinBias + t);
#pragma unroll 1
                for (int h = 0; h < 2; h++) {
                    const int q = h ? q1 : q0;
                    float thr = h ? thr1 : thr0;
                    const float slack = h ? slack1 : slack0;
                    uint2* buf = h ? buf1 : buf0;
                    int cnt = h ? cnt1 : cnt0;
                    const uint32_t acc = lane_acc + (uint32_t)h * kTileN;
                    ptx::mbar_wait(&t_full[h], tphase);
                    ptx::tc_fence_after();
#pragma unroll 1
                    for (int blk = 0; blk < 2; blk++) {
                        if constexpr (PARTS == 2) {
                            ptx::tmem_ld_32x32b_x32(acc + (uint32_t)(blk * 64), a0);
                            ptx::tmem_ld_32x32b_x32(acc + (uint32_t)(blk * 64 + 32), a1);
                        } else {
                            ptx::tmem_ld_32x32b_x32(acc + (uint32_t)(blk * 32), a0);
                        }
                        ptx::tmem_ld_wait();
                        if (blk == 1) {
                            ptx::tc_fence_before();
                            __syncwarp();
                            if (lane == 0)
                                ptx::mbar_arrive(&t_empty[h]);
                        }
                        if (DBG == 0) {
                            if constexpr (PARTS == 2)
                                epi_filter64<DUMP, SELF>(p, a0, a1, q, colBase + blk * 64, inv, thr, slack, maxb, buf, cnt, minb);
                            else
                                epi_filter32<DUMP, SELF>(p, a0, q, colBase + blk * 32, inv, thr, slack, maxb, buf, cnt, minb);
                        }
                    }
                    if (h) {
                        cnt1 = cnt;
                        if (SELF)
                            thr1 = thr;
                    } else {
                        cnt0 = cnt;
                        if (SELF)
                            thr0 = thr;
                    }
                }
                tphase ^= 1;
            }
            if (!DUMP) {
                p.candCount[seg0] = cnt0;
                p.candCount[seg1] = cnt1;
            }
        }
    }

    ptx::tc_fence_before();
    __syncthreads();
    if (warp == 1) {
        ptx::tc_fence_after();
        ptx::tmem_dealloc<512>(tmem_base);
    }
}

}
}
```

faiss_b200/csrc/index.cu:

```cuda
#include "index.h"

#include "comm.h"

#include <algorithm>
#include <cfloat>
#include <chrono>
#include <condition_variable>
#include <cmath>
#include <cstring>
#include <future>
#include <mutex>
#include <numeric>
#include <random>
#include <thread>

namespace fb200 {

namespace {

double now_ms() {
    return std::chrono::duration<double, std::milli>(std::chrono::steady_clock::now().time_since_epoch()).count();
}

void validateKSelect(idx_t k) {
// ... 225 lines not shown
    g_intCtx = ctx;
}
void InterruptCallback::clear() {
    set(nullptr, nullptr);
}
bool InterruptCallback::is_interrupted() {
    std::lock_guard<std::mutex> g(g_intMu);
    return g_intFn != nullptr && g_intFn(g_intCtx) != 0;
}
void InterruptCallback::check() {
    if (is_interrupted())
        FB_THROW_MSG("computation interrupted");
}

void GpuIndex::search(idx_t n, const float* x, idx_t k, float* distances, idx_t* labels, const SearchParameters* params) const {
    FB_THROW_IF_NOT_MSG(!params || params->sel == nullptr, "GPU index does not support IDSelector search parameters");
    struct Guard {
        const SearchParameters*& slot;
        ~Guard() {
            slot = nullptr;
        }
    } guard{callParams_};
    callParams_ = params;
    search(n, x, k, distances, labels);
}

void GpuIndex::search(idx_t n, const float* x, idx_t k, float* distances, idx_t* labels) const {
    DeviceScope scope(config_.device);
    FB_THROW_IF_NOT_MSG(this->is_trained, "Index not trained");
    validateKSelect(k);
    if (n == 0)
        return;
    FB_THROW_IF_NOT_MSG(x && distances && labels, "null pointer passed to search");
    auto stream = stream_();
    constexpr size_t kSearchPageBytes = size_t(256) << 20;
    const bool hostQueries = getDeviceForAddress(x) != config_.device;
    idx_t maxQ = idx_t(1) << 18;
    if (hostQueries && (size_t)n * d * sizeof(float) >= minPagedSize_)
        maxQ = std::min<idx_t>(maxQ, (idx_t)(kSearchPageBytes / (sizeof(float) * d)));
    maxQ = std::min<idx_t>(maxQ, (idx_t)((size_t(1) << 30) / ((size_t)k * 12 * 8)));
    maxQ = std::max<idx_t>(maxQ, 1);
    if (hostQueries && (size_t)n * d * sizeof(float) >= minPagedSize_ && searchFromCpuPaged_(n, x, k, distances, labels, maxQ))
        return;
    for (idx_t i0 = 0; i0 < n; i0 += maxQ) {
        InterruptCallback::check();
        const idx_t nb = std::min(maxQ, n - i0);
        DeviceView<float> xv(resources_.get(), config_.device, x + (size_t)i0 * d, (size_t)nb * d, stream);
        DeviceOut<float> dv(resources_.get(), config_.device, distances + (size_t)i0 * k, (size_t)nb * k);
        DeviceOut<idx_t> lv(resources_.get(), config_.device, labels + (size_t)i0 * k, (size_t)nb * k);
        searchImpl_(nb, xv.ptr, (int)k, dv.ptr, lv.ptr);
        dv.finish(stream);
        lv.finish(stream);
        if (dv.staged || lv.staged || xv.hold.data)
            CUDA_VERIFY(cudaStreamSynchronize(stream));
    }
}

bool GpuIndex::searchFromCpuPaged_(idx_t n, const float* x, idx_t k, float* distances, idx_t* labels, idx_t maxQ) const {
    auto pinned = resources_->getPinnedMemory();
    const size_t half = pinned.second / 2;
    const idx_t pageQ = std::min<idx_t>(maxQ, (idx_t)(half / (sizeof(float) * d)));
    if (!pinned.first || pageQ < 1 || n <= pageQ)
        return false;
    auto stream = stream_();
    auto copyStream = resources_->getAsyncCopyStream(config_.device);
    const idx_t numPages = ceil_div(n, pageQ);
    GpuMemoryReservation devBuf[2] = {
            resources_->temp(config_.device, sizeof(float) * (size_t)pageQ * d),
            resources_->temp(config_.device, sizeof(float) * (size_t)pageQ * d)};
    float* pin[2] = {reinterpret_cast<float*>(pinned.first), reinterpret_cast<float*>((char*)pinned.first + half)};
    cudaEvent_t ready[2];
    for (auto& e : ready)
        CUDA_VERIFY(cudaEventCreateWithFlags(&e, cudaEventDisableTiming));

    std::mutex mu;
    std::condition_variable cv;
    idx_t issued = 0;
    idx_t consumed = 0;
    bool abort = false;
    std::string stagerError;
    const int device = config_.device;
    std::thread stager([&] {
        try {
            CUDA_VERIFY(cudaSetDevice(device));
            for (idx_t p = 0; p < numPages; p++) {
                {
                    std::unique_lock<std::mutex> lk(mu);
                    cv.wait(lk, [&] { return abort || p < consumed + 2; });
                    if (abort)
                        return;
                }
                const int b = (int)(p & 1);
                const idx_t i0 = p * pageQ, nb = std::min(pageQ, n - i0);
                const size_t bytes = sizeof(float) * (size_t)nb * d;
                std::memcpy(pin[b], x + (size_t)i0 * d, bytes);
                CUDA_VERIFY(cudaMemcpyAsync(devBuf[b].data, pin[b], bytes, cudaMemcpyHostToDevice, copyStream));
                CUDA_VERIFY(cudaEventRecord(ready[b], copyStream));
                {
                    std::lock_guard<std::mutex> lk(mu);
                    issued = p + 1;
                }
                cv.notify_all();
            }
        } catch (const std::exception& e) {
            std::lock_guard<std::mutex> lk(mu);
            stagerError = e.what();
            abort = true;
            cv.notify_all();
        }
    });
    auto finish = [&](bool failed) {
        {
            std::lock_guard<std::mutex> lk(mu);
            if (failed)
                abort = true;
        }
        cv.notify_all();
        stager.join();
        cudaStreamSynchronize(copyStream);
        for (auto& e : ready)
            cudaEventDestroy(e);
    };
    try {
        for (idx_t p = 0; p < numPages; p++) {
            InterruptCallback::check();
            {
                std::unique_lock<std::mutex> lk(mu);
                cv.wait(lk, [&] { return abort || issued > p; });
                if (abort)
                    FB_THROW_FMT("query staging failed: %s", stagerError.c_str());
            }
            const int b = (int)(p & 1);
            const idx_t i0 = p * pageQ, nb = std::min(pageQ, n - i0);
            CUDA_VERIFY(cudaStreamWaitEvent(stream, ready[b], 0));
            DeviceOut<float> dv(resources_.get(), config_.device, distances + (size_t)i0 * k, (size_t)nb * k);
            DeviceOut<idx_t> lv(resources_.get(), config_.device, labels + (size_t)i0 * k, (size_t)nb * k);
            searchImpl_(nb, devBuf[b].as<float>(), (int)k, dv.ptr, lv.ptr);
            dv.finish(stream);
            lv.finish(stream);
            CUDA_VERIFY(cudaStreamSynchronize(stream));
            {
                std::lock_guard<std::mutex> lk(mu);
                consumed = p + 1;
            }
            cv.notify_all();
        }
    } catch (...) {
        finish(true);
        throw;
    }
    finish(false);
    return true;
}

void GpuIndex::compute_residual(const float* x, float* residual, idx_t key) const {
    compute_residual_n(1, x, residual, &key);
}
void GpuIndex::compute_residual_n(idx_t, const float*, float*, const idx_t*) const {
    FB_THROW_MSG("compute_residual not implemented for this type of index");
}

GpuIndexFlat::GpuIndexFlat(
        std::shared_ptr<GpuResources> resources,
        int dims,
        MetricType metric,
        GpuIndexFlatConfig config)
        : GpuIndex(std::move(resources), dims, metric, 0, config),
          flatConfig_(config),
          vecs_(resources_.get(), config.device, AllocType::FlatData),
          vecs16_(resources_.get(), config.device, AllocType::FlatData),
          y16_(resources_.get(), config.device, AllocType::FlatData),
          bias_(resources_.get(), config.device, AllocType::FlatData),
          perm_(resources_.get(), config.device, AllocType::FlatData),
          tileMaxBias_(resources_.get(), config.device, AllocType::FlatData) {
    this->is_trained = true;
    dpad_ = (int)round_up(dims, 64);
}

GpuIndexFlat::~GpuIndexFlat() {}

void GpuIndexFlat::reset() {
    DeviceScope scope(config_.device);
    vecs_.clear();
    vecs16_.clear();
    y16_.clear();
    bias_.clear();
    perm_.clear();
    tileMaxBias_.clear();
    tcDirty_ = true;
    this->ntotal = 0;
}

void GpuIndexFlat::train(idx_t, const float*) {
}

void GpuIndexFlat::copyFrom(idx_t n, const float* xb) {
    reset();
    if (n > 0)
        add(n, xb);
}

void GpuIndexFlat::copyTo(float* out) const {
    reconstruct_n(0, ntotal, out);
}

void GpuIndexFlat::add(idx_t n, const float* x) {
    GpuIndex::add_with_ids(n, x, nullptr);
}

void GpuIndexFlat::add_with_ids(idx_t n, const float* x, const idx_t* ids) {
    FB_THROW_IF_NOT_MSG(ids == nullptr, "add_with_ids not supported");
    GpuIndex::add_with_ids(n, x, nullptr);
}

void GpuIndexFlat::addImpl_(idx_t n, const float* xDev, const idx_t* idsDev) {
    FB_THROW_IF_NOT_MSG(idsDev == nullptr, "add_with_ids not supported");
    auto stream = stream_();
    if (flatConfig_.useFloat16) {
        const size_t old = vecs16_.size(), cnt = (size_t)n * d;
        vecs16_.resize(old + cnt, stream);
        float_to_half_kernel<<<(unsigned)std::min<size_t>(ceil_div(cnt, (size_t)256), 65535 * 16), 256, 0, stream>>>(
                xDev, vecs16_.data() + old, nullptr, (int64_t)cnt);
        CUDA_CHECK_LAST();
    } else {
        vecs_.append(xDev, (size_t)n * d, stream);
    }
    this->ntotal += n;
    tcDirty_ = true;
}

const float* GpuIndexFlat::roundedQueries_(idx_t n, const float* xDev, GpuMemoryReservation& hold) const {
    if (!flatConfig_.useFloat16 || n == 0)
        return xDev;
    auto stream = stream_();
    const size_t cnt = (size_t)n * d;
    hold = resources_->temp(config_.device, sizeof(float) * cnt);
    float_to_half_kernel<<<(unsigned)std::min<size_t>(ceil_div(cnt, (size_t)256), 65535 * 16), 256, 0, stream>>>(
            xDev, nullptr, hold.as<float>(), (int64_t)cnt);
    CUDA_CHECK_LAST();
    return hold.as<float>();
}

void GpuIndexFlat::replaceVectorsDevice(idx_t n, const float* xDev) {
    DeviceScope scope(config_.device);
    auto stream = stream_();
    if (flatConfig_.useFloat16) {
        vecs16_.resize(0, stream);
        this->ntotal = 0;
        if (n > 0)
            addImpl_(n, xDev, nullptr);
        return;
    }
    vecs_.resize((size_t)n * d, stream);
    if (n > 0)
        CUDA_VERIFY(cudaMemcpyAsync(vecs_.data(), xDev, sizeof(float) * n * d, cudaMemcpyDeviceToDevice, stream));
    this->ntotal = n;
    tcDirty_ = true;
}

void GpuIndexFlat::prepareTensorCoreData_() const {
    if (!tcDirty_)
        return;
    auto stream = stream_();
    const idx_t n = this->ntotal;
    const int64_t padRows = round_up(n, 256) + 256;
    y16_.resize((size_t)n * dpad_, stream);
    bias_.resize((size_t)padRows, stream);
    tileMaxBias_.resize((size_t)(padRows / 256) * 2, stream);
    const bool sorted = metric_type == METRIC_L2;
    if (sorted)
        perm_.resize((size_t)n, stream);
    else
        perm_.clear();
    auto scal = resources_->temp(config_.device, sizeof(float) * 2);
    auto norms = resources_->temp(config_.device, sizeof(float) * n);
    CUDA_VERIFY(cudaMemsetAsync(scal.data, 0, sizeof(float) * 2, stream));
    runAbsMax(rows_(), n * (int64_t)d, scal.as<float>(), stream, yHalf_());
    float h[2] = {0.f, 0.f};
    CUDA_VERIFY(cudaMemcpyAsync(h, scal.data, sizeof(float), cudaMemcpyDeviceToHost, stream));
    CUDA_VERIFY(cudaStreamSynchronize(stream));
    float scale = 1.f;
    if (h[0] > 0.f) {
        int e;
        std::frexp(h[0], &e);
        scale = std::ldexp(1.f, 14 - e);
    }
    fill_float_kernel<<<(unsigned)ceil_div(padRows, 256), 256, 0, stream>>>(bias_.data(), padRows, -INFINITY);
    CUDA_CHECK_LAST();
    runFlatTcPrepareRows(
            resources_.get(), config_.device, rows_(), n, d, dpad_, scale, metric_type, y16_.data(), bias_.data(),
            sorted ? perm_.data() : nullptr, tileMaxBias_.data(), norms.as<float>(), stream, yHalf_());
    runMaxOf(norms.as<float>(), n, scal.as<float>() + 1, stream);
    CUDA_VERIFY(cudaMemcpyAsync(h, scal.data, sizeof(float) * 2, cudaMemcpyDeviceToHost, stream));
    CUDA_VERIFY(cudaStreamSynchronize(stream));
    yScale_ = scale;
    yMaxNorm_ = std::sqrt(h[1]) * 1.0001f;
    tcDirty_ = false;
}

void GpuIndexFlat::searchImpl_(idx_t n, const float* xDev, int k, float* dDev, idx_t* iDev) const {
    auto stream = stream_();
    lastSearchUsedTensorCores = 0;
    lastSearchFallbackQueries = 0;
    if (this->ntotal == 0) {
        std::vector<float> hd((size_t)n * k, metric_type == METRIC_L2 ? FLT_MAX : -FLT_MAX);
        std::vector<idx_t> hi((size_t)n * k, -1);
        CUDA_VERIFY(cudaMemcpyAsync(dDev, hd.data(), hd.size() * sizeof(float), cudaMemcpyHostToDevice, stream));
        CUDA_VERIFY(cudaMemcpyAsync(iDev, hi.data(), hi.size() * sizeof(idx_t), cudaMemcpyHostToDevice, stream));
        CUDA_VERIFY(cudaStreamSynchronize(stream));
        return;
    }
    const bool tc = flatConfig_.useTensorCores && flatTcSupported(d, k, this->ntotal) && n >= 16;
    GpuMemoryReservation qHold;
    xDev = roundedQueries_(n, xDev, qHold);
    if (tc) {
        prepareTensorCoreData_();
        runFlatTcSearch(
                resources_.get(), config_.device, xDev, n, rows_(), y16_.data(), bias_.data(),
                metric_type == METRIC_L2 ? perm_.data() : nullptr, tileMaxBias_.data(), yScale_,
                yMaxNorm_, this->ntotal, d, dpad_, k, metric_type, dDev, iDev, stream, nullptr, yHalf_());
        lastSearchUsedTensorCores = 1;
        lastSearchFallbackQueries = lastFlatTcFallbacks();
    } else {
        runFlatExact(
                resources_.get(), config_.device, xDev, n, rows_(), this->ntotal, d, k, metric_type, 0, dDev, iDev,
                stream, yHalf_());
    }
}

bool GpuIndexFlat::shardPoolingEligible(int k, idx_t n) const {
    return flatConfig_.useTensorCores && this->ntotal > 0 && flatTcSupported(d, k, this->ntotal) && n >= 16;
}

void GpuIndexFlat::searchShardDevice(idx_t n, const float* xDev, int k, float* dDev, idx_t* iDev, const FlatTcShard* flatShard) const {
    if (!flatShard) {
        searchImpl_(n, xDev, k, dDev, iDev);
        return;
    }
    FB_THROW_IF_NOT_MSG(shardPoolingEligible(k, n), "pooled sharded search requested on a shard that cannot take the tensor-core path");
    auto stream = stream_();
    prepareTensorCoreData_();
    GpuMemoryReservation qHold;
    xDev = roundedQueries_(n, xDev, qHold);
    runFlatTcSearch(
            resources_.get(), config_.device, xDev, n, rows_(), y16_.data(), bias_.data(),
            metric_type == METRIC_L2 ? perm_.data() : nullptr, tileMaxBias_.data(), yScale_, yMaxNorm_, this->ntotal, d,
            dpad_, k, metric_type, dDev, iDev, stream, flatShard, yHalf_());
    lastSearchUsedTensorCores = 1;
    lastSearchFallbackQueries = lastFlatTcFallbacks();
}

void GpuIndexFlat::reconstruct(idx_t key, float* out) const {
    reconstruct_n(key, 1, out);
}

void GpuIndexFlat::reconstruct_n(idx_t i0, idx_t num, float* out) const {
    DeviceScope scope(config_.device);
    if (num == 0)
        return;
    FB_THROW_IF_NOT_MSG(i0 >= 0 && i0 + num <= this->ntotal, "reconstruct: index out of bounds");
    auto stream = stream_();
    if (flatConfig_.useFloat16) {
        const idx_t step = std::max<idx_t>(1, (idx_t)((size_t(64) << 20) / (sizeof(float) * d)));
        for (idx_t r = 0; r < num; r += step) {
            const idx_t m = std::min(step, num - r);
            const size_t cnt = (size_t)m * d;
            DeviceOut<float> ov(resources_.get(), config_.device, out + (size_t)r * d, cnt);
            half_to_float_kernel<<<(unsigned)std::min<size_t>(ceil_div(cnt, (size_t)256), 65535 * 16), 256, 0, stream>>>(
                    vecs16_.data() + (size_t)(i0 + r) * d, ov.ptr, (int64_t)cnt);
            CUDA_CHECK_LAST();
            ov.finish(stream);
            CUDA_VERIFY(cudaStreamSynchronize(stream));
        }
        return;
    }
    CUDA_VERIFY(cudaMemcpyAsync(out, vecs_.data() + (size_t)i0 * d, sizeof(float) * num * d, cudaMemcpyDefault, stream));
    CUDA_VERIFY(cudaStreamSynchronize(stream));
}

void GpuIndexFlat::reconstruct_batch(idx_t n, const idx_t* keys, float* out) const {
    DeviceScope scope(config_.device);
    if (n == 0)
        return;
    auto stream = stream_();
    DeviceView<idx_t> kv(resources_.get(), config_.device, keys, n, stream);
    DeviceOut<float> ov(resources_.get(), config_.device, out, (size_t)n * d);
    runGatherRows(rows_(), kv.ptr, n, d, ov.ptr, stream, yHalf_());
    ov.finish(stream);
    CUDA_VERIFY(cudaStreamSynchronize(stream));
}

void GpuIndexFlat::compute_residual(const float* x, float* residual, idx_t key) const {
    compute_residual_n(1, x, residual, &key);
}

void GpuIndexFlat::compute_residual_n(idx_t n, const float* xs, float* residuals, const idx_t* keys) const {
    DeviceScope scope(config_.device);
    if (n == 0)
        return;
    auto stream = stream_();
    DeviceView<float> xv(resources_.get(), config_.device, xs, (size_t)n * d, stream);
    DeviceView<idx_t> kv(resources_.get(), config_.device, keys, n, stream);
    DeviceOut<float> ov(resources_.get(), config_.device, residuals, (size_t)n * d);
    runCalcResidual(xv.ptr, rows_(), kv.ptr, n, d, ov.ptr, stream, yHalf_());
    ov.finish(stream);
    CUDA_VERIFY(cudaStreamSynchronize(stream));
}

void rand_perm(int* perm, size_t n, int64_t seed) {
    std::iota(perm, perm + n, 0);
    std::mt19937 mt((unsigned int)seed);
    for (size_t i = 0; i + 1 < n; i++) {
        int i2 = (int)(i + mt() % (n - i));
        std::swap(perm[i], perm[i2]);
    }
}

int split_clusters(size_t d, size_t k, size_t n, float* hassign, float* centroids) {
    const float EPS = 1.f / 1024.f;
    FB_THROW_IF_NOT_MSG(n > k, "split_clusters: n must exceed k to find a non-empty donor centroid");
    std::mt19937 mt(1234u);
    size_t nsplit = 0;
    for (size_t ci = 0; ci < k; ci++) {
        if (hassign[ci] != 0)
            continue;
        size_t cj = 0, tries = 0;
        const size_t maxTries = 10 * k;
        bool found = false;
        for (cj = 0; tries < maxTries; cj = (cj + 1) % k) {
            float p = (hassign[cj] - 1.0) / (float)(n - k);
            float r = mt() / float(mt.max());
            if (r < p) {
                found = true;
                break;
            }
            tries++;
        }
        if (!found) {
            cj = 0;
            for (size_t j = 1; j < k; j++)
                if (hassign[j] > hassign[cj])
                    cj = j;
        }
        memcpy(centroids + ci * d, centroids + cj * d, sizeof(float) * d);
        for (size_t j = 0; j < d; j++) {
            if (j % 2 == 0) {
                centroids[ci * d + j] *= 1 + EPS;
                centroids[cj * d + j] *= 1 - EPS;
            } else {
                centroids[ci * d + j] *= 1 - EPS;
                centroids[cj * d + j] *= 1 + EPS;
            }
        }
        hassign[ci] = hassign[cj] / 2;
        hassign[cj] -= hassign[ci];
        nsplit++;
    }
    return (int)nsplit;
}

void Clustering::train(idx_t nx, const float* x_in, GpuIndexFlat& index) {
    FB_THROW_IF_NOT_FMT(
            nx >= (idx_t)k,
            "Number of training points (%ld) should be at least as large as number of clusters (%zd)",
            (long)nx,
            k);
    FB_THROW_IF_NOT_FMT((size_t)index.d == d, "Index dimension %d not the same as data dimension %d", index.d, (int)d);
    FB_THROW_IF_NOT_MSG(!frozen_centroids, "Clustering: frozen_centroids (input centroids) is not supported by faiss_b200");
    GpuResources* res = index.getResources().get();
    const int device = index.getDevice();
    DeviceScope scope(device);
    cudaStream_t stream = res->getDefaultStream(device);
    const double t0 = now_ms();

    DeviceView<float> xall(res, device, x_in, (size_t)nx * d, stream);
    const float* x = xall.ptr;
    GpuMemoryReservation sub;
    if ((size_t)nx > k * (size_t)max_points_per_centroid) {
        FB_THROW_IF_NOT_MSG(nx <= (idx_t)0x7fffffff, "Dataset too large for standard subsampling");
        if (verbose)
            printf("Sampling a subset of %zd / %ld for training\n", k * max_points_per_centroid, (long)nx);
        std::vector<int> perm(nx);
        rand_perm(perm.data(), nx, seed);
        idx_t nnew = (idx_t)(k * max_points_per_centroid);
        auto pd = res->temp(device, sizeof(int) * nnew);
        CUDA_VERIFY(cudaMemcpyAsync(pd.data, perm.data(), sizeof(int) * nnew, cudaMemcpyHostToDevice, stream));
        sub = res->device_alloc(device, sizeof(float) * nnew * d, AllocType::Other);
        gather_rows_int_kernel<<<(unsigned)nnew, std::min<int>(256, (int)d), 0, stream>>>(
                x, pd.as<int>(), nnew, (int)d, sub.as<float>());
        CUDA_CHECK_LAST();
        CUDA_VERIFY(cudaStreamSynchronize(stream));
        x = sub.as<float>();
        nx = nnew;
    } else if ((size_t)nx < k * (size_t)min_points_per_centroid) {
        fprintf(stderr,
                "WARNING clustering %ld points to %zd centroids: please provide at least %ld training points\n",
                (long)nx,
                k,
                (long)(k * min_points_per_centroid));
    }

    centroids.resize(d * k);
    auto cDev = res->device_alloc(device, sizeof(float) * k * d, AllocType::Other);

    if ((size_t)nx == k) {
        CUDA_VERIFY(cudaMemcpyAsync(centroids.data(), x, sizeof(float) * d * k, cudaMemcpyDeviceToHost, stream));
        CUDA_VERIFY(cudaStreamSynchronize(stream));
        iteration_stats.push_back({0.f, 0.0, 0.0, 1.0, 0});
        index.reset();
        index.add(k, centroids.data());
        return;
    }
    if (verbose)
        printf("Clustering %ld points in %zdD to %zd clusters, redo %d times, %d iterations\n",
               (long)nx, d, k, nredo, niter);

    auto assign = res->device_alloc(device, sizeof(idx_t) * nx, AllocType::Other);
    auto dis = res->device_alloc(device, sizeof(float) * nx, AllocType::Other);
    auto sums = res->device_alloc(device, sizeof(float) * k * d, AllocType::Other);
    auto countsBuf = res->device_alloc(device, sizeof(float) * k, AllocType::Other);
    auto objBuf = res->device_alloc(device, sizeof(double), AllocType::Other);

    const bool lower_is_better = index.metric_type == METRIC_L2;
    float best_obj = lower_is_better ? HUGE_VALF : -HUGE_VALF;
    std::vector<ClusteringIterationStats> best_stats;
    std::vector<float> best_centroids;
    double t_search_tot = 0;

    for (int redo = 0; redo < nredo; redo++) {
        {
            std::vector<int> perm(nx);
            rand_perm(perm.data(), nx, (int64_t)seed + 1 + redo * 15486557L);
            auto pd = res->temp(device, sizeof(int) * k);
            CUDA_VERIFY(cudaMemcpyAsync(pd.data, perm.data(), sizeof(int) * k, cudaMemcpyHostToDevice, stream));
            gather_rows_int_kernel<<<(unsigned)k, std::min<int>(256, (int)d), 0, stream>>>(
                    x, pd.as<int>(), (int64_t)k, (int)d, cDev.as<float>());
            CUDA_CHECK_LAST();
            runKmeansPostProcess(cDev.as<float>(), (int64_t)k, (int)d, spherical, int_centroids, stream);
            CUDA_VERIFY(cudaStreamSynchronize(stream));
        }
        if (index.ntotal != 0)
            index.reset();
        if (!index.is_trained)
            index.train(k, cDev.as<float>());
        index.add(k, cDev.as<float>());

        float obj = 0;
        std::vector<float> hassign(k);
        for (int it = 0; it < niter; it++) {
            const double t0s = now_ms();
            index.searchDevice(nx, x, 1, dis.as<float>(), assign.as<idx_t>());
            CUDA_VERIFY(cudaMemsetAsync(objBuf.data, 0, sizeof(double), stream));
            sum_kernel<<<296, 256, 0, stream>>>(dis.as<float>(), nx, objBuf.as<double>());
            CUDA_CHECK_LAST();
            CUDA_VERIFY(cudaMemsetAsync(sums.data, 0, sizeof(float) * k * d, stream));
            CUDA_VERIFY(cudaMemsetAsync(countsBuf.data, 0, sizeof(float) * k, stream));
            runKmeansAccumulate(x, assign.as<idx_t>(), nx, (int)d, (int64_t)k, sums.as<float>(), countsBuf.as<float>(), stream);
            runKmeansFinalize(sums.as<float>(), countsBuf.as<float>(), (int64_t)k, (int)d, cDev.as<float>(), stream);
            double hobj = 0;
            CUDA_VERIFY(cudaMemcpyAsync(&hobj, objBuf.data, sizeof(double), cudaMemcpyDeviceToHost, stream));
            CUDA_VERIFY(cudaMemcpyAsync(hassign.data(), countsBuf.data, sizeof(float) * k, cudaMemcpyDeviceToHost, stream));
            CUDA_VERIFY(cudaStreamSynchronize(stream));
            t_search_tot += now_ms() - t0s;
            obj = (float)hobj;

            int nsplit = 0;
            double imb = 0;
            {
                double tot = 0, uf = 0;
                bool anyEmpty = false;
                for (size_t c = 0; c < k; c++) {
                    tot += hassign[c];
                    uf += (double)hassign[c] * hassign[c];
                    anyEmpty |= hassign[c] == 0;
                }
                imb = tot > 0 ? uf * k / (tot * tot) : 0;
                if (anyEmpty) {
                    CUDA_VERIFY(cudaMemcpyAsync(
                            centroids.data(), cDev.data, sizeof(float) * k * d, cudaMemcpyDeviceToHost, stream));
                    CUDA_VERIFY(cudaStreamSynchronize(stream));
                    nsplit = split_clusters(d, k, nx, hassign.data(), centroids.data());
                    CUDA_VERIFY(cudaMemcpyAsync(
                            cDev.data, centroids.data(), sizeof(float) * k * d, cudaMemcpyHostToDevice, stream));
                }
            }
            iteration_stats.push_back({obj, (now_ms() - t0) / 1000.0, t_search_tot / 1000.0, imb, nsplit});
            if (verbose) {
                printf("  Iteration %d (%.2f s, search %.2f s): objective=%g imbalance=%.3f nsplit=%d       \r",
                       it, (now_ms() - t0) / 1000.0, t_search_tot / 1000.0, obj, imb, nsplit);
                fflush(stdout);
            }
            runKmeansPostProcess(cDev.as<float>(), (int64_t)k, (int)d, spherical, int_centroids, stream);
            if (update_index) {
                index.reset();
                index.train(k, cDev.as<float>());
                index.add(k, cDev.as<float>());
            } else {
                index.replaceVectorsDevice(k, cDev.as<float>());
            }
            InterruptCallback::check();
            if (it > 0) {
                const float prev = iteration_stats[iteration_stats.size() - 2].obj;
                if (prev != 0 && std::fabs((double)prev - (double)obj) / std::fabs((double)prev) <= 0.0)
                    break;
            }
        }
        if (verbose)
            printf("\n");
        CUDA_VERIFY(cudaMemcpyAsync(centroids.data(), cDev.data, sizeof(float) * k * d, cudaMemcpyDeviceToHost, stream));
        CUDA_VERIFY(cudaStreamSynchronize(stream));
        if (nredo > 1) {
            if ((lower_is_better && obj < best_obj) || (!lower_is_better && obj > best_obj)) {
                best_centroids = centroids;
                best_stats = iteration_stats;
                best_obj = obj;
            }
            index.reset();
        }
    }
    if (nredo > 1) {
        centroids = best_centroids;
        iteration_stats = best_stats;
        index.reset();
        index.add(k, best_centroids.data());
    }
}

namespace {
__global__ void scatter_rows_kernel(const float* src, const int* srcRow, const int* dstRow, int64_t n, int d, float* dst) {
    const int64_t i = blockIdx.x;
    if (i >= n)
        return;
    for (int j = threadIdx.x; j < d; j += blockDim.x)
        dst[(int64_t)dstRow[i] * d + j] = src[(int64_t)srcRow[i] * d + j];
}
__global__ void store_obj_kernel(const double* acc, float* out) {
    *out = (float)*acc;
}
}

void Clustering::trainSharded(idx_t nLocal, const float* x_in, GpuIndexFlat& index, const Communicator& comm) {
    FB_THROW_IF_NOT_FMT((size_t)index.d == d, "Index dimension %d not the same as data dimension %d", index.d, (int)d);
    FB_THROW_IF_NOT_MSG(!frozen_centroids, "Clustering: frozen_centroids (input centroids) is not supported by faiss_b200");
    FB_THROW_IF_NOT_MSG(nredo == 1, "sharded clustering supports nredo == 1");
    GpuResources* res = index.getResources().get();
    const int device = index.getDevice();
    DeviceScope scope(device);
    cudaStream_t stream = res->getDefaultStream(device);
    const double t0 = now_ms();
    splitSeconds = 0;

    DeviceView<float> xall(res, device, x_in, (size_t)nLocal * d, stream);
// ... 1176 lines not shown
```

faiss_b200/csrc/index.h:

```cpp
#pragma once

#include <memory>
#include <string>
#include <vector>

#include "common.h"
#include "kernels.h"
#include "resources.h"

namespace fb200 {

template <typename T>
class DeviceVector {
   public:
    DeviceVector(GpuResources* res, int device, AllocType type) : res_(res), device_(device), type_(type) {}
    ~DeviceVector() {
        clear();
    }
    DeviceVector(const DeviceVector&) = delete;
    DeviceVector& operator=(const DeviceVector&) = delete;

    T* data() const {
        return data_;
    }
    size_t size() const {
        return size_;
    }
    size_t capacity() const {
        return cap_;
    }
    void clear() {
        if (data_)
            res_->deallocMemory(device_, data_);
        data_ = nullptr;
        size_ = cap_ = 0;
    }
    void reserve(size_t n, cudaStream_t stream, bool exact = false) {
        if (n <= cap_)
            return;
        size_t ncap = exact ? n : std::max(n, cap_ + cap_ / 2);
        AllocRequest r;
        r.type = type_;
        r.device = device_;
        r.space = MemorySpace::Device;
        r.stream = stream;
        r.size = ncap * sizeof(T);
        T* nd = (T*)res_->allocMemory(r);
        if (size_ > 0) {
            CUDA_VERIFY(cudaMemcpyAsync(nd, data_, size_ * sizeof(T), cudaMemcpyDeviceToDevice, stream));
            CUDA_VERIFY(cudaStreamSynchronize(stream));
        }
        if (data_)
            res_->deallocMemory(device_, data_);
        data_ = nd;
        cap_ = ncap;
    }
    void resize(size_t n, cudaStream_t stream) {
        reserve(n, stream);
        size_ = n;
    }
    void append(const T* src, size_t n, cudaStream_t stream) {
        if (n == 0)
            return;
        reserve(size_ + n, stream);
        CUDA_VERIFY(cudaMemcpyAsync(data_ + size_, src, n * sizeof(T), cudaMemcpyDefault, stream));
        size_ += n;
    }

   private:
    GpuResources* res_;
    int device_;
    AllocType type_;
    T* data_ = nullptr;
    size_t size_ = 0, cap_ = 0;
};

struct Index {
    int d;
    idx_t ntotal = 0;
    bool verbose = false;
    bool is_trained = true;
    MetricType metric_type;
    float metric_arg = 0.f;

    explicit Index(int d_ = 0, MetricType m = METRIC_L2) : d(d_), metric_type(m) {}
    virtual ~Index() = default;

    virtual void train(idx_t , const float* ) {}
    virtual void add(idx_t n, const float* x) = 0;
    virtual void add_with_ids(idx_t n, const float* x, const idx_t* xids);
    virtual void search(idx_t n, const float* x, idx_t k, float* distances, idx_t* labels) const = 0;
    virtual void assign(idx_t n, const float* x, idx_t* labels, idx_t k = 1) const;
    virtual void reset() = 0;
    virtual void reconstruct(idx_t key, float* recons) const;
    virtual void reconstruct_batch(idx_t n, const idx_t* keys, float* recons) const;
    virtual void reconstruct_n(idx_t i0, idx_t ni, float* recons) const;
    virtual void compute_residual(const float* x, float* residual, idx_t key) const;
    virtual void compute_residual_n(idx_t n, const float* xs, float* residuals, const idx_t* keys) const;
};

struct SearchParameters {
    void* sel = nullptr;
    virtual ~SearchParameters() {}
};
struct SearchParametersIVF : SearchParameters {
    size_t nprobe = 1;
    size_t max_codes = 0;
    SearchParameters* quantizer_params = nullptr;
};

struct InterruptCallback {
    typedef int (*Fn)(void* ctx);
    static void set(Fn fn, void* ctx);
    static void clear();
    static bool is_interrupted();
    static void check();
};

struct GpuIndexConfig {
    int device = 0;
    MemorySpace memorySpace = MemorySpace::Device;
};

class GpuIndex : public Index {
   public:
    GpuIndex(std::shared_ptr<GpuResources> resources, int dims, MetricType metric, float metricArg, GpuIndexConfig config);

    int getDevice() const {
        return config_.device;
    }
    std::shared_ptr<GpuResources> getResources() {
        return resources_;
    }
    void setMinPagingSize(size_t size) {
        minPagedSize_ = size;
    }
    size_t getMinPagingSize() const {
        return minPagedSize_;
    }

    void add(idx_t n, const float* x) override;
    void add_with_ids(idx_t n, const float* x, const idx_t* ids) override;
    void search(idx_t n, const float* x, idx_t k, float* distances, idx_t* labels) const override;
    void search(idx_t n, const float* x, idx_t k, float* distances, idx_t* labels, const SearchParameters* params) const;
    void assign(idx_t n, const float* x, idx_t* labels, idx_t k = 1) const override;
    void compute_residual(const float* x, float* residual, idx_t key) const override;
    void compute_residual_n(idx_t n, const float* xs, float* residuals, const idx_t* keys) const override;

   protected:
    mutable const SearchParameters* callParams_ = nullptr;
    virtual bool addImplRequiresIDs_() const = 0;
    virtual void addImpl_(idx_t n, const float* xDev, const idx_t* idsDev) = 0;
    virtual void searchImpl_(idx_t n, const float* xDev, int k, float* dDev, idx_t* iDev) const = 0;
    bool searchFromCpuPaged_(idx_t n, const float* x, idx_t k, float* distances, idx_t* labels, idx_t maxQ) const;

   public:
    virtual void searchShardDevice(idx_t n, const float* xDev, int k, float* dDev, idx_t* iDev, const FlatTcShard* flatShard) const {
        (void)flatShard;
        searchImpl_(n, xDev, k, dDev, iDev);
    }
    virtual bool shardPoolingEligible(int , idx_t ) const {
        return false;
    }

   protected:
    cudaStream_t stream_() const {
        return resources_->getDefaultStream(config_.device);
    }

    std::shared_ptr<GpuResources> resources_;
    GpuIndexConfig config_;
    size_t minPagedSize_ = size_t(256) << 20;
};

struct GpuIndexFlatConfig : GpuIndexConfig {
    bool useFloat16 = false;
    bool useTensorCores = true;
};

class GpuIndexFlat : public GpuIndex {
   public:
    GpuIndexFlat(
            std::shared_ptr<GpuResources> resources,
            int dims,
            MetricType metric,
            GpuIndexFlatConfig config = GpuIndexFlatConfig());
    ~GpuIndexFlat() override;

    void copyFrom(idx_t n, const float* xb);
    void copyTo(float* xbOut) const;
    size_t getNumVecs() const {
        return (size_t)ntotal;
    }

    void reset() override;
    void train(idx_t n, const float* x) override;
    void add(idx_t n, const float* x) override;
    void add_with_ids(idx_t n, const float* x, const idx_t* ids) override;
    void reconstruct(idx_t key, float* out) const override;
    void reconstruct_n(idx_t i0, idx_t num, float* out) const override;
    void reconstruct_batch(idx_t n, const idx_t* keys, float* out) const override;
    void compute_residual(const float* x, float* residual, idx_t key) const override;
    void compute_residual_n(idx_t n, const float* xs, float* residuals, const idx_t* keys) const override;

    void searchDevice(idx_t n, const float* xDev, int k, float* dDev, idx_t* iDev) const {
        searchImpl_(n, xDev, k, dDev, iDev);
    }
    void searchShardDevice(idx_t n, const float* xDev, int k, float* dDev, idx_t* iDev, const FlatTcShard* flatShard) const override;
    bool shardPoolingEligible(int k, idx_t n) const override;
    const float* vectorsDevice() const {
        FB_THROW_IF_NOT_MSG(!flatConfig_.useFloat16, "fp32 row access on a float16 GpuIndexFlat");
        return vecs_.data();
    }
    bool usesFloat16() const {
        return flatConfig_.useFloat16;
    }
    void setUseTensorCores(bool v) {
        flatConfig_.useTensorCores = v;
    }
    void replaceVectorsDevice(idx_t n, const float* xDev);
    mutable int lastSearchUsedTensorCores = 0;
    mutable int lastSearchFallbackQueries = 0;

   protected:
    bool addImplRequiresIDs_() const override {
        return false;
    }
    void addImpl_(idx_t n, const float* xDev, const idx_t* idsDev) override;
    void searchImpl_(idx_t n, const float* xDev, int k, float* dDev, idx_t* iDev) const override;
    void prepareTensorCoreData_() const;

    const void* rows_() const {
        return flatConfig_.useFloat16 ? (const void*)vecs16_.data() : (const void*)vecs_.data();
    }
    int yHalf_() const {
        return flatConfig_.useFloat16 ? 1 : 0;
    }
    const float* roundedQueries_(idx_t n, const float* xDev, GpuMemoryReservation& hold) const;

    GpuIndexFlatConfig flatConfig_;
    DeviceVector<float> vecs_;
    DeviceVector<__half> vecs16_;
    mutable DeviceVector<__half> y16_;
    mutable DeviceVector<float> bias_;
    mutable DeviceVector<int> perm_;
    mutable DeviceVector<float> tileMaxBias_;
    mutable bool tcDirty_ = true;
    mutable float yScale_ = 1.f;
    mutable float yMaxNorm_ = 0.f;
    mutable int dpad_ = 0;
};

class GpuIndexFlatL2 : public GpuIndexFlat {
   public:
    GpuIndexFlatL2(std::shared_ptr<GpuResources> r, int dims, GpuIndexFlatConfig c = GpuIndexFlatConfig())
            : GpuIndexFlat(std::move(r), dims, METRIC_L2, c) {}
};
class GpuIndexFlatIP : public GpuIndexFlat {
   public:
    GpuIndexFlatIP(std::shared_ptr<GpuResources> r, int dims, GpuIndexFlatConfig c = GpuIndexFlatConfig())
            : GpuIndexFlat(std::move(r), dims, METRIC_INNER_PRODUCT, c) {}
};

struct ClusteringParameters {
    int niter = 25;
    int nredo = 1;
    bool verbose = false;
    bool spherical = false;
    bool int_centroids = false;
    bool update_index = false;
    bool frozen_centroids = false;
    int min_points_per_centroid = 39;
    int max_points_per_centroid = 256;
    int seed = 1234;
};

struct ClusteringIterationStats {
    float obj;
    double time;
    double time_search;
    double imbalance_factor;
    int nsplit;
};

struct Clustering : ClusteringParameters {
    size_t d;
    size_t k;
    std::vector<float> centroids;
    std::vector<ClusteringIterationStats> iteration_stats;

    Clustering(int d, int k) : d(d), k(k) {}
    Clustering(int d, int k, const ClusteringParameters& cp) : ClusteringParameters(cp), d(d), k(k) {}
    void train(idx_t n, const float* x, GpuIndexFlat& index);
    void trainSharded(idx_t nLocal, const float* xLocal, GpuIndexFlat& index, const Communicator& comm);
    double splitSeconds = 0;
};

void trainProductQuantizer(
        std::shared_ptr<GpuResources> resources,
        int device,
        idx_t n,
        const float* xDev,
        int d,
        int M,
        const ClusteringParameters& cp,
        float* pqOut);

void rand_perm(int* perm, size_t n, int64_t seed);
int split_clusters(size_t d, size_t k, size_t n, float* hassign, float* centroids);

class IvfLists {
   public:
    IvfLists(GpuResources* res, int device, int64_t nlist, int codeSize, bool pqInterleaved = false);
    ~IvfLists();
    void reset();
    void reserve(size_t totalVecs, cudaStream_t stream);
    void reserveLists(const int64_t* lens, cudaStream_t stream);
    idx_t append(idx_t n, const uint8_t* rowsDev, const idx_t* idsDev, const idx_t* assignDev, cudaStream_t stream);
    void setListFromHost(int64_t l, int64_t len, const uint8_t* codes, const idx_t* ids, cudaStream_t stream);
    void getListToHost(int64_t l, uint8_t* codes, idx_t* ids, cudaStream_t stream) const;
    int64_t listLength(int64_t l) const {
        return hLen_[l];
    }
    size_t reclaim(cudaStream_t stream);

    const int64_t* dStart() const {
        return dStart_;
    }
    const int* dLen() const {
        return dLen_;
    }
    const uint8_t* codes() const {
        return codes_;
    }
    const idx_t* ids() const {
        return ids_;
    }
    int64_t nlist() const {
        return nlist_;
    }
    int codeSize() const {
        return codeSize_;
    }
    int maxListLength() const;
    int64_t arenaElems() const {
        return arenaElems_;
    }
    bool interleaved() const {
        return interleaved_;
    }

   private:
    void relayout_(const std::vector<int64_t>& newCap, cudaStream_t stream);
    void uploadMeta_(cudaStream_t stream);

    GpuResources* res_;
    int device_;
    int64_t nlist_;
    int codeSize_;
    bool interleaved_ = false;
    uint8_t* codes_ = nullptr;
    idx_t* ids_ = nullptr;
    int64_t arenaElems_ = 0;
    std::vector<int64_t> hStart_, hCap_;
    std::vector<int> hLen_;
    int64_t* dStart_ = nullptr;
    int* dLen_ = nullptr;
    int* dCounts_ = nullptr;
};

enum IndicesOptions { INDICES_CPU = 0, INDICES_IVF = 1, INDICES_32_BIT = 2, INDICES_64_BIT = 3 };

struct GpuIndexIVFConfig : GpuIndexConfig {
    IndicesOptions indicesOptions = INDICES_64_BIT;
    GpuIndexFlatConfig flatConfig;
    bool allowCpuCoarseQuantizer = false;
};

class GpuIndexIVF : public GpuIndex {
   public:
    GpuIndexIVF(
            std::shared_ptr<GpuResources> resources,
            int dims,
            MetricType metric,
            idx_t nlist,
            int codeSize,
            GpuIndexIVFConfig config,
            bool pqInterleaved = false);
    ~GpuIndexIVF() override;

    idx_t nlist;
    size_t nprobe = 1;
    size_t max_codes = 0;
    GpuIndexFlat* quantizer = nullptr;
    uint64_t coarseEpoch = 0;
    bool own_fields = true;
    ClusteringParameters cp;

    idx_t getNumLists() const {
        return nlist;
    }
    idx_t getListLength(idx_t listId) const;
    std::vector<uint8_t> getListVectorData(idx_t listId) const;
    std::vector<idx_t> getListIndices(idx_t listId) const;
    void reserveMemory(size_t numVecs);
    void setListSizes(const idx_t* lens);
    size_t reclaimMemory();
    void reset() override;
    void setQuantizer(GpuIndexFlat* coarse);
    void setCoarseCentroids(const float* centroidsHostOrDev);
    void getCoarseCentroids(float* out) const;
    void setList(idx_t listId, idx_t len, const uint8_t* codes, const idx_t* ids);

    void search_preassigned(
            idx_t n,
            const float* x,
            idx_t k,
            const idx_t* assign,
            const float* centroid_dis,
            float* distances,
            idx_t* labels) const;

   protected:
    bool addImplRequiresIDs_() const override {
        return true;
    }
    void trainQuantizer_(idx_t n, const float* xDev);
    virtual bool quantizerOnlyTraining_() const {
        return true;
    }
    void searchImpl_(idx_t n, const float* xDev, int k, float* dDev, idx_t* iDev) const override;
    virtual void scanImpl_(
            idx_t n,
            const float* xDev,
            const idx_t* probesDev,
            const float* coarseDisDev,
            int nprobe,
            int k,
            float* dDev,
            idx_t* iDev) const = 0;

    GpuIndexIVFConfig ivfConfig_;
    std::unique_ptr<IvfLists> lists_;
};

class GpuIndexIVFFlat : public GpuIndexIVF {
   public:
    GpuIndexIVFFlat(
            std::shared_ptr<GpuResources> resources,
            int dims,
            idx_t nlist,
            MetricType metric = METRIC_L2,
            GpuIndexIVFConfig config = GpuIndexIVFConfig());
    GpuIndexIVFFlat(
            std::shared_ptr<GpuResources> resources,
            GpuIndexFlat* coarseQuantizer,
            int dims,
            idx_t nlist,
            MetricType metric = METRIC_L2,
            GpuIndexIVFConfig config = GpuIndexIVFConfig());
    void train(idx_t n, const float* x) override;

   protected:
    void addImpl_(idx_t n, const float* xDev, const idx_t* idsDev) override;
    void scanImpl_(idx_t, const float*, const idx_t*, const float*, int, int, float*, idx_t*) const override;
};

struct GpuIndexIVFPQConfig : GpuIndexIVFConfig {
    bool useFloat16LookupTables = false;
    bool usePrecomputedTables = false;
    bool interleavedLayout = false;
    bool useMMCodeDistance = false;
};

class GpuIndexIVFPQ : public GpuIndexIVF {
   public:
    GpuIndexIVFPQ(
            std::shared_ptr<GpuResources> resources,
            int dims,
            idx_t nlist,
            idx_t subQuantizers,
            idx_t bitsPerCode,
            MetricType metric = METRIC_L2,
            GpuIndexIVFPQConfig config = GpuIndexIVFPQConfig());
    GpuIndexIVFPQ(
            std::shared_ptr<GpuResources> resources,
            GpuIndexFlat* coarseQuantizer,
            int dims,
            idx_t nlist,
            idx_t subQuantizers,
            idx_t bitsPerCode,
            MetricType metric = METRIC_L2,
            GpuIndexIVFPQConfig config = GpuIndexIVFPQConfig());
    ~GpuIndexIVFPQ() override;

    int getNumSubQuantizers() const {
        return M_;
    }
    int getBitsPerCode() const {
        return nbits_;
    }
    int getCentroidsPerSubQuantizer() const {
        return 1 << nbits_;
    }
    void setPrecomputedCodes(bool enable) {
        usePrecomputed_ = enable;
        precomputedExplicit_ = true;
    }
    bool getPrecomputedCodes() const {
        return usePrecomputed_;
    }
    ClusteringParameters pq_cp;
    void train(idx_t n, const float* x) override;
    void setPQCentroids(const float* c);
    void getPQCentroids(float* out) const;

   protected:
    bool quantizerOnlyTraining_() const override {
        return false;
    }
    void trainResidualQuantizer_(idx_t n, const float* xDev);
    void addImpl_(idx_t n, const float* xDev, const idx_t* idsDev) override;
    void scanImpl_(idx_t, const float*, const idx_t*, const float*, int, int, float*, idx_t*) const override;

    int M_, nbits_;
// ... 104 lines not shown
```

faiss_b200/csrc/kernels.h:

```cpp
#pragma once

#include <cuda_fp16.h>

#include "common.h"
#include "resources.h"

namespace fb200 {

void runL2Norms(const float* x, int64_t n, int d, float* norms, cudaStream_t stream);

void runFlatExact(
        GpuResources* res,
        int device,
        const float* Q,
        int64_t nq,
        const void* Y,
        int64_t n,
        int d,
        int k,
        MetricType metric,
        int64_t idBase,
        float* outD,
        idx_t* outI,
        cudaStream_t stream,
        int yHalf = 0);

void runFlatArgmin(
        GpuResources* res,
        int device,
        const float* Q,
        int64_t nq,
        const float* Y,
        int64_t n,
        int d,
        MetricType metric,
        float* outD,
        idx_t* outI,
        cudaStream_t stream);

void runMergeTopK(
        const float* inD,
        const idx_t* inI,
        int64_t rows,
        int nlists,
        int kin,
        const idx_t* idOffsets,
        int k,
        MetricType metric,
        float* outD,
        idx_t* outI,
        cudaStream_t stream);

void runMergeTopKListMajor(
        const float* inD,
        const idx_t* inI,
        int64_t rows,
        int nlists,
        int kin,
        const idx_t* idOffsets,
        int k,
        MetricType metric,
        float* outD,
        idx_t* outI,
        cudaStream_t stream);

void runCalcResidual(
        const float* x,
        const void* centroids,
        const idx_t* assign,
        int64_t n,
        int d,
        float* out,
        cudaStream_t stream,
        int yHalf = 0);
void runGatherRows(const void* src, const idx_t* ids, int64_t n, int d, float* out, cudaStream_t stream, int yHalf = 0);

struct FlatTcPlan;

void runFlatTcPrepareRows(
        GpuResources* res,
        int device,
        const void* Y,
        int64_t n,
        int d,
        int dpad,
        float scale,
        MetricType metric,
        __half* Y16,
        float* bias,
        int* perm,
        float* tileMaxBias,
        float* norms,
        cudaStream_t stream,
        int yHalf = 0);

void runAbsMax(const void* x, int64_t count, float* out , cudaStream_t stream, int yHalf = 0);
void runMaxOf(const float* x, int64_t count, float* out , cudaStream_t stream);

bool flatTcSupported(int d, int k, int64_t n);

class Communicator;
struct FlatTcShard {
    const Communicator* comm;
    int64_t maxTiles;
};

void runFlatTcSearch(
        GpuResources* res,
        int device,
        const float* Q,
        int64_t nq,
        const void* Y,
        const __half* Y16,
        const float* bias,
        const int* perm,
        const float* tileMaxBias,
        float yScale,
        float yMaxNorm,
        int64_t n,
        int d,
        int dpad,
        int k,
        MetricType metric,
        float* outD,
        idx_t* outI,
        cudaStream_t stream,
        const FlatTcShard* shard = nullptr,
        int yHalf = 0);

int& lastFlatTcFallbacks();

void runFlatTcScoresDebug(
        const __half* Q16,
        int64_t nq,
        const __half* Y16,
        int64_t n,
        int dpad,
        float* S,
        cudaStream_t stream);

void runKmeansAccumulate(
        const float* x,
        const idx_t* assign,
        int64_t n,
        int d,
        int64_t k,
        float* sums ,
        float* counts ,
        cudaStream_t stream);
void runKmeansFinalize(
        const float* sums,
        const float* counts,
        int64_t k,
        int d,
        float* centroids ,
        cudaStream_t stream);

void runKmeansPostProcess(float* centroids, int64_t k, int d, bool spherical, bool intCentroids, cudaStream_t stream);

void runPQEncode(
        const float* resid,
        int64_t n,
        int d,
        int M,
        int ksub,
        const float* pqCentroids ,
        uint8_t* codes ,
        cudaStream_t stream);

void runIvfCountAssign(const idx_t* assign, int64_t n, int64_t nlist, int* counts , cudaStream_t stream);
void runIvfAppendOffsets(
        const idx_t* assign,
        int64_t n,
        int64_t nlist,
        const int* listLenBefore ,
        int* offsets ,
        int* scratch ,
        cudaStream_t stream);
void runIvfScatter(
        const uint8_t* rows,
        const idx_t* ids,
        const idx_t* assign,
        const int* offsets,
        int64_t n,
        int codeSize,
        const int64_t* listStart ,
        uint8_t* arenaCodes,
        idx_t* arenaIds,
        cudaStream_t stream);

void runIvfFlatScan(
        GpuResources* res,
        int device,
        const float* Q,
        int64_t nq,
        int d,
        const idx_t* probes,
        int nprobe,
        const int64_t* listStart,
        const int* listLen,
        const float* arenaVecs,
        const idx_t* arenaIds,
        int64_t arenaElems,
        int k,
        MetricType metric,
        float* outD,
        idx_t* outI,
        cudaStream_t stream);

void runIvfPqScan(
        GpuResources* res,
        int device,
        const float* Q,
        int64_t nq,
        int d,
        const idx_t* probes,
        const float* coarseDis,
        int nprobe,
        const float* coarseCentroids ,
        const float* pqCentroids ,
        int M,
        const int64_t* listStart,
        const int* listLen,
        const uint8_t* arenaCodes,
        const idx_t* arenaIds,
        int k,
        MetricType metric,
        float* outD,
        idx_t* outI,
        cudaStream_t stream);

inline bool ivfPqInterleavedSupported(int M) {
    return (M == 16 || M == 32);
}
void runIvfPqScatterInterleaved(
        const uint8_t* codesFlat,
        const idx_t* ids,
        const idx_t* assign,
        const int* offsets,
        int64_t n,
        int M,
        const int64_t* listStart,
        uint8_t* arenaCodes,
        idx_t* arenaIds,
        cudaStream_t stream);
void runIvfPqListToInterleaved(const uint8_t* flat, int64_t len, int M, uint8_t* listCodes, cudaStream_t stream);
void runIvfPqListFromInterleaved(const uint8_t* listCodes, int64_t len, int M, uint8_t* flat, cudaStream_t stream);

void runIvfPqPrecomputeTerm2(
        const float* coarse, const float* pqT, int64_t nlist, int d, int M, float* term2, cudaStream_t stream);

void runIvfPqScanInterleaved(
        GpuResources* res,
        int device,
        const float* Q,
        int64_t nq,
        int d,
        const idx_t* probes,
        const float* coarseDis,
        int nprobe,
        const float* coarseCentroids,
        const float* pqCentroidsT,
        const float* term2,
        int M,
        const int64_t* listStart,
        const int* listLen,
        const uint8_t* arenaCodes,
        const idx_t* arenaIds,
        int64_t arenaElems,
        int k,
        MetricType metric,
        float* outD,
        idx_t* outI,
        cudaStream_t stream);

}
```

faiss_b200/csrc/tc_ptx.cuh:

```cuda
#pragma once

#include <cuda.h>
#include <cuda_runtime.h>

#include <cstdint>

namespace fb200 {
namespace ptx {

__device__ __forceinline__ uint32_t smem_u32(const void* p) {
    return static_cast<uint32_t>(__cvta_generic_to_shared(p));
}

__device__ __forceinline__ bool elect_one() {
    uint32_t pred = 0;
    asm volatile(
            "{\n"
            ".reg .pred P;\n"
            "elect.sync _|P, 0xffffffff;\n"
            "selp.u32 %0, 1, 0, P;\n"
            "}\n"
            : "=r"(pred));
    return pred != 0;
}

__device__ __forceinline__ void mbar_init(uint64_t* bar, uint32_t count) {
    asm volatile("mbarrier.init.shared::cta.b64 [%0], %1;" ::"r"(smem_u32(bar)), "r"(count));
}
__device__ __forceinline__ void fence_barrier_init() {
    asm volatile("fence.mbarrier_init.release.cluster;" ::: "memory");
}
__device__ __forceinline__ void fence_proxy_async() {
    asm volatile("fence.proxy.async.shared::cta;" ::: "memory");
}
__device__ __forceinline__ void mbar_arrive(uint64_t* bar) {
    asm volatile("mbarrier.arrive.shared::cta.b64 _, [%0];" ::"r"(smem_u32(bar)) : "memory");
}
__device__ __forceinline__ void mbar_arrive_expect_tx(uint64_t* bar, uint32_t bytes) {
    asm volatile("mbarrier.arrive.expect_tx.shared::cta.b64 _, [%0], %1;" ::"r"(smem_u32(bar)), "r"(bytes)
                 : "memory");
}
__device__ __forceinline__ bool mbar_try_wait(uint64_t* bar, uint32_t parity) {
    uint32_t ok;
    asm volatile(
            "{\n"
            ".reg .pred P;\n"
            "mbarrier.try_wait.parity.shared::cta.b64 P, [%1], %2;\n"
            "selp.u32 %0, 1, 0, P;\n"
            "}\n"
            : "=r"(ok)
            : "r"(smem_u32(bar)), "r"(parity)
            : "memory");
    return ok != 0;
}
__device__ __forceinline__ void mbar_wait(uint64_t* bar, uint32_t parity) {
    while (!mbar_try_wait(bar, parity)) {
    }
}

__device__ __forceinline__ void prefetch_tensormap(const void* desc) {
    asm volatile("prefetch.tensormap [%0];" ::"l"(reinterpret_cast<uint64_t>(desc)) : "memory");
}
__device__ __forceinline__ void tma_load_3d(
        void* smem_dst,
        const void* desc,
        uint64_t* bar,
        int32_t c0,
        int32_t c1,
        int32_t c2) {
    asm volatile(
            "cp.async.bulk.tensor.3d.shared::cluster.global.mbarrier::complete_tx::bytes"
            " [%0], [%1, {%3, %4, %5}], [%2];"
            ::"r"(smem_u32(smem_dst)),
            "l"(reinterpret_cast<uint64_t>(desc)),
            "r"(smem_u32(bar)),
            "r"(c0),
            "r"(c1),
            "r"(c2)
            : "memory");
}

__device__ __forceinline__ void bulk_load_1d(void* smem_dst, const void* gsrc, uint32_t bytes, uint64_t* bar) {
    asm volatile(
            "cp.async.bulk.shared::cluster.global.mbarrier::complete_tx::bytes [%0], [%1], %2, [%3];"
            ::"r"(smem_u32(smem_dst)),
            "l"(reinterpret_cast<uint64_t>(gsrc)),
            "r"(bytes),
            "r"(smem_u32(bar))
            : "memory");
}

__device__ __forceinline__ float4 lds128(uint32_t addr) {
    float4 v;
    asm volatile("ld.shared.v4.f32 {%0, %1, %2, %3}, [%4];" : "=f"(v.x), "=f"(v.y), "=f"(v.z), "=f"(v.w) : "r"(addr));
    return v;
}
__device__ __forceinline__ int lds32(uint32_t addr) {
    int v;
    asm volatile("ld.shared.b32 %0, [%1];" : "=r"(v) : "r"(addr));
    return v;
}
__device__ __forceinline__ void sts32(uint32_t addr, int v) {
    asm volatile("st.shared.b32 [%0], %1;" ::"r"(addr), "r"(v) : "memory");
}

__device__ __forceinline__ void fma2(float& o0, float& o1, float a0, float a1, float s, float c0, float c1) {
    asm("{\n.reg .b64 ra, rs, rc, rd;\nmov.b64 ra, {%2,%3};\nmov.b64 rs, {%4,%4};\nmov.b64 rc, {%5,%6};\n"
        "fma.rn.f32x2 rd, ra, rs, rc;\nmov.b64 {%0,%1}, rd;\n}"
        : "=f"(o0), "=f"(o1)
        : "f"(a0), "f"(a1), "f"(s), "f"(c0), "f"(c1));
}
__device__ __forceinline__ float max3(float a, float b, float c) {
    float d;
    asm("max.f32 %0, %1, %2, %3;" : "=f"(d) : "f"(a), "f"(b), "f"(c));
    return d;
}

template <uint32_t kCols>
__device__ __forceinline__ void tmem_alloc(uint32_t* smem_dst) {
    asm volatile("tcgen05.alloc.cta_group::1.sync.aligned.shared::cta.b32 [%0], %1;" ::"r"(smem_u32(smem_dst)),
                 "n"(kCols)
                 : "memory");
    asm volatile("tcgen05.relinquish_alloc_permit.cta_group::1.sync.aligned;" ::: "memory");
}
template <uint32_t kCols>
__device__ __forceinline__ void tmem_dealloc(uint32_t taddr) {
    asm volatile("tcgen05.dealloc.cta_group::1.sync.aligned.b32 %0, %1;" ::"r"(taddr), "n"(kCols) : "memory");
}
__device__ __forceinline__ void tc_fence_before() {
    asm volatile("tcgen05.fence::before_thread_sync;" ::: "memory");
}
__device__ __forceinline__ void tc_fence_after() {
    asm volatile("tcgen05.fence::after_thread_sync;" ::: "memory");
}
__device__ __forceinline__ void mma_f16_ss(
        uint32_t tmem_d,
        uint64_t desc_a,
        uint64_t desc_b,
        uint32_t idesc,
        uint32_t accumulate) {
    asm volatile(
            "{\n"
            ".reg .pred p;\n"
            "setp.ne.b32 p, %4, 0;\n"
            "tcgen05.mma.cta_group::1.kind::f16 [%0], %1, %2, %3, p;\n"
            "}\n" ::"r"(tmem_d),
            "l"(desc_a),
            "l"(desc_b),
            "r"(idesc),
            "r"(accumulate)
            : "memory");
}
__device__ __forceinline__ void mma_commit(uint64_t* bar) {
    asm volatile("tcgen05.commit.cta_group::1.mbarrier::arrive::one.shared::cluster.b64 [%0];" ::"r"(smem_u32(bar))
                 : "memory");
}
__device__ __forceinline__ void tmem_ld_32x32b_x32(uint32_t taddr, uint32_t (&r)[32]) {
    asm volatile(
            "tcgen05.ld.sync.aligned.32x32b.x32.b32 "
            "{%0, %1, %2, %3, %4, %5, %6, %7, %8, %9, %10, %11, %12, %13, %14, %15, "
            "%16, %17, %18, %19, %20, %21, %22, %23, %24, %25, %26, %27, %28, %29, %30, %31}, [%32];"
            : "=r"(r[0]), "=r"(r[1]), "=r"(r[2]), "=r"(r[3]), "=r"(r[4]), "=r"(r[5]), "=r"(r[6]), "=r"(r[7]),
              "=r"(r[8]), "=r"(r[9]), "=r"(r[10]), "=r"(r[11]), "=r"(r[12]), "=r"(r[13]), "=r"(r[14]),
              "=r"(r[15]), "=r"(r[16]), "=r"(r[17]), "=r"(r[18]), "=r"(r[19]), "=r"(r[20]), "=r"(r[21]),
              "=r"(r[22]), "=r"(r[23]), "=r"(r[24]), "=r"(r[25]), "=r"(r[26]), "=r"(r[27]), "=r"(r[28]),
              "=r"(r[29]), "=r"(r[30]), "=r"(r[31])
            : "r"(taddr)
            : "memory");
}
__device__ __forceinline__ void tmem_ld_wait() {
    asm volatile("tcgen05.wait::ld.sync.aligned;" ::: "memory");
}

__device__ __forceinline__ uint64_t make_smem_desc_sw128(uint32_t smem_addr) {
    uint64_t d = 0;
    d |= (uint64_t)((smem_addr & 0x3ffff) >> 4);
    d |= (uint64_t)1 << 16;
    d |= (uint64_t)(1024 >> 4) << 32;
    d |= (uint64_t)1 << 46;
    d |= (uint64_t)2 << 61;
    return d;
}
__host__ __device__ constexpr uint32_t make_idesc_f16(int M, int N) {
    return (1u << 4) | (0u << 7) | (0u << 10) | ((uint32_t)(N >> 3) << 17) | ((uint32_t)(M >> 4) << 24);
}

}
}
```

include/faiss_b200_c.h:

```cpp
#ifndef FAISS_B200_C_H
#define FAISS_B200_C_H

#include <stddef.h>
#include <stdint.h>

#ifdef __cplusplus
extern "C" {
#endif

#if defined(__GNUC__)
#define FB200_API __attribute__((visibility("default")))
#else
#define FB200_API
#endif

typedef int64_t idx_t;

typedef enum FaissErrorCode {
    OK = 0,
    UNKNOWN_EXCEPT = -1,
    FAISS_EXCEPT = -2,
    STD_EXCEPT = -4
} FaissErrorCode;

typedef enum FaissMetricType {
    METRIC_INNER_PRODUCT = 0,
    METRIC_L2 = 1
} FaissMetricType;

typedef struct FaissIndex_H FaissIndex;
typedef struct FaissIndex_H FaissGpuIndex;
typedef struct FaissIndex_H FaissIndexShards;
typedef struct FaissStandardGpuResources_H FaissStandardGpuResources;

FB200_API const char* faiss_get_last_error(void);
FB200_API const char* faiss_b200_version(void);

FB200_API int faiss_StandardGpuResources_new(FaissStandardGpuResources** p_res);
FB200_API void faiss_StandardGpuResources_free(FaissStandardGpuResources* res);
FB200_API int faiss_StandardGpuResources_noTempMemory(FaissStandardGpuResources* res);
FB200_API int faiss_StandardGpuResources_setTempMemory(FaissStandardGpuResources* res, size_t size);
FB200_API int faiss_StandardGpuResources_setPinnedMemory(FaissStandardGpuResources* res, size_t size);
FB200_API int faiss_StandardGpuResources_setDefaultStream(FaissStandardGpuResources* res, int device, void* cuda_stream);
FB200_API int faiss_StandardGpuResources_setDefaultNullStreamAllDevices(FaissStandardGpuResources* res);
FB200_API int faiss_StandardGpuResources_getDefaultStream(FaissStandardGpuResources* res, int device, void** out_stream);
FB200_API int faiss_StandardGpuResources_syncDefaultStream(FaissStandardGpuResources* res, int device);
FB200_API int faiss_StandardGpuResources_getMemoryInfo(FaissStandardGpuResources* res, char* buf, size_t buflen);
FB200_API int faiss_StandardGpuResources_getTempMemoryAvailable(FaissStandardGpuResources* res, int device, size_t* out);

FB200_API void faiss_Index_free(FaissIndex* index);
FB200_API int faiss_Index_d(const FaissIndex* index);
FB200_API int faiss_Index_is_trained(const FaissIndex* index);
FB200_API idx_t faiss_Index_ntotal(const FaissIndex* index);
FB200_API FaissMetricType faiss_Index_metric_type(const FaissIndex* index);
FB200_API int faiss_Index_verbose(const FaissIndex* index);
FB200_API void faiss_Index_set_verbose(FaissIndex* index, int v);
FB200_API int faiss_Index_train(FaissIndex* index, idx_t n, const float* x);
FB200_API int faiss_Index_add(FaissIndex* index, idx_t n, const float* x);
FB200_API int faiss_Index_add_with_ids(FaissIndex* index, idx_t n, const float* x, const idx_t* xids);
FB200_API int faiss_Index_search(const FaissIndex* index, idx_t n, const float* x, idx_t k, float* distances, idx_t* labels);
FB200_API int faiss_Index_assign(FaissIndex* index, idx_t n, const float* x, idx_t* labels, idx_t k);
FB200_API int faiss_Index_reset(FaissIndex* index);
FB200_API int faiss_Index_reconstruct(const FaissIndex* index, idx_t key, float* recons);
FB200_API int faiss_Index_reconstruct_n(const FaissIndex* index, idx_t i0, idx_t ni, float* recons);
FB200_API int faiss_Index_reconstruct_batch(const FaissIndex* index, idx_t n, const idx_t* keys, float* recons);
FB200_API int faiss_Index_compute_residual(const FaissIndex* index, const float* x, float* residual, idx_t key);
FB200_API int faiss_Index_compute_residual_n(const FaissIndex* index, idx_t n, const float* x, float* residuals, const idx_t* keys);

FB200_API int faiss_GpuIndex_setMinPagingSize(FaissGpuIndex* index, size_t size);
FB200_API int faiss_GpuIndex_getMinPagingSize(const FaissGpuIndex* index, size_t* out_size);

FB200_API int faiss_GpuIndexFlat_new(FaissGpuIndex** p_index, FaissStandardGpuResources* res, int d, FaissMetricType metric, int device, int use_tensor_cores);
FB200_API int faiss_GpuIndexFlat_new_with_config(FaissGpuIndex** p_index, FaissStandardGpuResources* res, int d, FaissMetricType metric, int device, int use_tensor_cores, int use_float16);
FB200_API int faiss_GpuIndexFlatL2_new(FaissGpuIndex** p_index, FaissStandardGpuResources* res, int d, int device);
FB200_API int faiss_GpuIndexFlatIP_new(FaissGpuIndex** p_index, FaissStandardGpuResources* res, int d, int device);
FB200_API int faiss_GpuIndexFlat_copyFrom(FaissGpuIndex* index, idx_t n, const float* xb);
FB200_API int faiss_GpuIndexFlat_copyTo(const FaissGpuIndex* index, float* xb_out);
FB200_API int faiss_GpuIndexFlat_setUseTensorCores(FaissGpuIndex* index, int enable);
FB200_API int faiss_GpuIndexFlat_lastSearchInfo(const FaissGpuIndex* index, int* out2);

FB200_API int faiss_GpuIndexIVF_set_nprobe(FaissGpuIndex* index, size_t nprobe);
FB200_API size_t faiss_GpuIndexIVF_nprobe(const FaissGpuIndex* index);
FB200_API size_t faiss_GpuIndexIVF_nlist(const FaissGpuIndex* index);
FB200_API int faiss_GpuIndexIVF_set_clustering(FaissGpuIndex* index, int niter, int seed, int max_points_per_centroid);
FB200_API int faiss_GpuIndexIVF_reserveMemory(FaissGpuIndex* index, size_t num_vecs);
FB200_API int faiss_GpuIndexIVF_reclaimMemory(FaissGpuIndex* index, size_t* reclaimed);
FB200_API size_t faiss_GpuIndexIVF_get_list_size(const FaissGpuIndex* index, size_t list_no);
FB200_API int faiss_GpuIndexIVF_getListVectorData(const FaissGpuIndex* index, size_t list_no, uint8_t* codes_out);
FB200_API int faiss_GpuIndexIVF_getListIndices(const FaissGpuIndex* index, size_t list_no, idx_t* ids_out);
FB200_API int faiss_GpuIndexIVF_setCoarseCentroids(FaissGpuIndex* index, const float* centroids);
FB200_API int faiss_GpuIndexIVF_getCoarseCentroids(const FaissGpuIndex* index, float* centroids_out);
FB200_API int faiss_GpuIndexIVF_setList(FaissGpuIndex* index, size_t list_no, idx_t len, const uint8_t* codes, const idx_t* ids);
FB200_API int faiss_GpuIndexIVF_setListSizes(FaissGpuIndex* index, const idx_t* lens);
FB200_API int faiss_GpuIndexIVF_set_is_trained(FaissGpuIndex* index, int v);
FB200_API int faiss_GpuIndexIVF_search_preassigned(const FaissGpuIndex* index, idx_t n, const float* x, idx_t k, const idx_t* assign, const float* centroid_dis, float* distances, idx_t* labels);

FB200_API int faiss_GpuIndexIVFFlat_new(FaissGpuIndex** p_index, FaissStandardGpuResources* res, int d, idx_t nlist, FaissMetricType metric, int device);

FB200_API int faiss_GpuIndexIVFPQ_new(FaissGpuIndex** p_index, FaissStandardGpuResources* res, int d, idx_t nlist, idx_t M, idx_t nbits, FaissMetricType metric, int device);
FB200_API int faiss_GpuIndexIVFPQ_setPQCentroids(FaissGpuIndex* index, const float* centroids );
FB200_API int faiss_GpuIndexIVFPQ_getPQCentroids(const FaissGpuIndex* index, float* centroids_out);
FB200_API int faiss_GpuIndexIVFPQ_set_pq_clustering(FaissGpuIndex* index, int niter, int seed, int max_points_per_centroid);
FB200_API int faiss_GpuIndexIVFPQ_setPrecomputedCodes(FaissGpuIndex* index, int enable);

FB200_API int faiss_IndexShards_new(FaissIndexShards** p_index, idx_t d);
FB200_API int faiss_IndexShards_new_with_options(FaissIndexShards** p_index, idx_t d, int threaded, int successive_ids);
FB200_API int faiss_IndexShards_add_shard(FaissIndexShards* index, FaissIndex* shard);
FB200_API int faiss_IndexShards_remove_shard(FaissIndexShards* index, FaissIndex* shard);
FB200_API FaissIndex* faiss_IndexShards_at(FaissIndexShards* index, int i);
FB200_API int faiss_IndexShards_own_indices(const FaissIndexShards* index);
FB200_API void faiss_IndexShards_set_own_indices(FaissIndexShards* index, int v);
FB200_API int faiss_IndexShards_successive_ids(const FaissIndexShards* index);
FB200_API void faiss_IndexShards_set_successive_ids(FaissIndexShards* index, int v);

typedef struct FaissSearchParameters_H FaissSearchParameters;
typedef struct FaissSearchParameters_H FaissSearchParametersIVF;
FB200_API int faiss_SearchParametersIVF_new_with(FaissSearchParametersIVF** p_sp, size_t nprobe, size_t max_codes);
FB200_API void faiss_SearchParameters_free(FaissSearchParameters* sp);
FB200_API int faiss_Index_search_with_params(const FaissIndex* index, idx_t n, const float* x, idx_t k, const FaissSearchParameters* params, float* distances, idx_t* labels);
FB200_API void faiss_b200_set_interrupt_callback(int (*want_interrupt)(void* ctx), void* ctx);
FB200_API int faiss_GpuIndexIVFFlat_new_with_quantizer(FaissGpuIndex** p_index, FaissStandardGpuResources* res, FaissGpuIndex* coarse, int d, idx_t nlist, FaissMetricType metric, int device);
FB200_API int faiss_GpuIndexIVFPQ_new_with_quantizer(FaissGpuIndex** p_index, FaissStandardGpuResources* res, FaissGpuIndex* coarse, int d, idx_t nlist, idx_t M, idx_t nbits, FaissMetricType metric, int device);

FB200_API int faiss_b200_nccl_unique_id(char* out128);
FB200_API int faiss_StandardGpuResources_ncclInitRank(FaissStandardGpuResources* res, int device, int nranks, int rank, const char* unique_id128);
FB200_API int faiss_StandardGpuResources_ncclInitAll(FaissStandardGpuResources* res, int ndev, const int* devices);
FB200_API int faiss_StandardGpuResources_ncclRank(FaissStandardGpuResources* res, int device, int* rank, int* nranks);
FB200_API int faiss_IndexShardsIVF_new(FaissIndexShards** p_index, FaissGpuIndex* quantizer, idx_t nlist, int threaded, int successive_ids);
FB200_API int faiss_IndexShardsIVF_add_shard(FaissIndexShards* index, FaissIndex* shard);
FB200_API int faiss_IndexShards_lastSearchPath(const FaissIndexShards* index);
FB200_API int faiss_DistributedIndexShards_new(FaissIndexShards** p_index, FaissStandardGpuResources* res, FaissGpuIndex* local_shard, int successive_ids);
FB200_API int faiss_DistributedIndexShards_sync(FaissIndexShards* index);
FB200_API int faiss_DistributedIndexShards_info(const FaissIndexShards* index, int* rank, int* nranks, idx_t* id_offset);
FB200_API int b200_shards_search(FaissStandardGpuResources* res, FaissGpuIndex* local_shard, int successive_ids, idx_t n, const float* x, idx_t k, float* distances, idx_t* labels);

FB200_API int faiss_b200_kmeans(FaissStandardGpuResources* res, int device, size_t d, size_t n, size_t k, const float* x, int niter, int seed, int max_points_per_centroid, float* centroids_out , float* obj_out );

FB200_API int faiss_b200_kmeans_ex(FaissStandardGpuResources* res, int device, size_t d, size_t n, size_t k, const float* x, int niter, int seed, int max_points_per_centroid, FaissMetricType metric, int spherical, float* centroids_out, float* obj_out);
FB200_API int faiss_b200_kmeans_sharded(FaissStandardGpuResources* res, int device, size_t d, size_t n_local, size_t k, const float* x_local, int niter, int seed, float* centroids_out, float* obj_out, double* stats_out);
FB200_API int faiss_b200_pq_train(FaissStandardGpuResources* res, int device, size_t d, size_t M, size_t n, const float* x, int niter, int seed, float* centroids_out);

FB200_API int faiss_b200_bfKnn(FaissStandardGpuResources* res, int device, FaissMetricType metric, idx_t k, int dims, const float* vectors, idx_t num_vectors, const float* queries, idx_t num_queries, float* out_distances, idx_t* out_indices);

FB200_API long long faiss_b200_launch_count(void);
FB200_API void faiss_b200_kernel_timing(int enable);
FB200_API int faiss_b200_kernel_timing_collect(const char* name, double* ms_out, int* launches_out);

FB200_API int faiss_b200_rand_perm(int* perm, size_t n, int64_t seed);
FB200_API int faiss_b200_split_clusters(size_t d, size_t k, size_t n, float* hassign, float* centroids, int* nsplit_out);
FB200_API int faiss_b200_merge_knn_results_host(idx_t n, idx_t k, int nshard, FaissMetricType metric, const float* all_distances, const idx_t* all_labels, float* distances, idx_t* labels);

FB200_API int b200_l2_norms(FaissStandardGpuResources* res, int device, const float* x, idx_t n, int d, float* norms);
FB200_API int b200_flat_search_exact(FaissStandardGpuResources* res, int device, const float* Y, idx_t N, int d, const float* Q, idx_t nq, int k, FaissMetricType metric, float* D, idx_t* I);
FB200_API int b200_topk_merge(FaissStandardGpuResources* res, int device, const float* D_in, const idx_t* I_in, idx_t nq, int nshard, int k_in, const idx_t* id_offsets , int k, FaissMetricType metric, float* D, idx_t* I);
FB200_API int b200_flat_tc_scores_debug(FaissStandardGpuResources* res, int device, const void* Q16, idx_t nq, const void* Y16, idx_t N, int dpad, float* S);
FB200_API int b200_ivf_coarse(FaissStandardGpuResources* res, int device, const float* centroids, idx_t nlist, int d, const float* Q, idx_t nq, int nprobe, FaissMetricType metric, float* coarse_dis, idx_t* coarse_ids);
FB200_API int b200_kmeans_assign(FaissStandardGpuResources* res, int device, const float* centroids, idx_t k, int d, const float* x, idx_t n, FaissMetricType metric, float* dis, idx_t* assign);
FB200_API int b200_ivfflat_scan(FaissStandardGpuResources* res, int device, const float* Q, idx_t nq, int d, const idx_t* probes, int nprobe, const int64_t* list_start, const int* list_len, const float* arena_vecs, const idx_t* arena_ids, idx_t arena_elems, int k, FaissMetricType metric, float* D, idx_t* I);
FB200_API int b200_ivfpq_scan(FaissStandardGpuResources* res, int device, const float* Q, idx_t nq, int d, const idx_t* probes, const float* coarse_dis, int nprobe, const float* coarse_centroids, const float* pq_centroids, int M, const int64_t* list_start, const int* list_len, const uint8_t* arena_codes, const idx_t* arena_ids, int k, FaissMetricType metric, float* D, idx_t* I);
FB200_API int b200_ivf_append(FaissStandardGpuResources* res, int device, const uint8_t* rows, const idx_t* ids, const idx_t* assign, idx_t n, int code_size, idx_t nlist, const int64_t* list_start, int* list_len, uint8_t* arena_codes, idx_t* arena_ids);
FB200_API int b200_pq_encode(FaissStandardGpuResources* res, int device, const float* residuals, idx_t n, int d, int M, const float* pq_centroids, uint8_t* codes);
FB200_API int b200_kmeans_update(FaissStandardGpuResources* res, int device, const float* x, const idx_t* assign, idx_t n, int d, idx_t k, float* sums, float* counts, float* centroids);

#ifdef __cplusplus
}
#endif
#endif
```

Baseline: 434,500.

## Add 2-CTA cluster tcgen05 MMA path for round-based Flat tensor-core search

Adds a cta_group::2 variant of the Flat tensor-core kernel. Two CTAs in a cluster share one MMA issuer, and each CTA loads half of the Y tile through paired TMA, so every Y stage holds half as many rows per CTA. The freed shared memory allows more pipeline stages and halves per-CTA Y traffic for each query-pair unit. Scheduling is reworked to count units per cluster and to size the grid from cluster occupancy. The path is on by default for non-streaming, non-ksplit searches; it adds cluster sync overhead and pads queries to an even number of pairs.

```diff
diff --git a/faiss_b200/__init__.py b/faiss_b200/__init__.py
--- a/faiss_b200/__init__.py
+++ b/faiss_b200/__init__.py
@@ -316,7 +316,9 @@
     def lastSearchInfo(self):
         out = (ctypes.c_int * 2)()
         check(lib.faiss_GpuIndexFlat_lastSearchInfo(self._h, out))
-        return {"tensor_cores": int(out[0]), "fallback_queries": int(out[1])}
+        cg = ctypes.c_int()
+        check(lib.faiss_GpuIndexFlat_lastSearchCtaGroup(self._h, ctypes.byref(cg)))
+        return {"tensor_cores": int(out[0]), "fallback_queries": int(out[1]), "tc_cta_group": int(cg.value)}
 
 
 class GpuIndexFlatL2(GpuIndexFlat):
diff --git a/faiss_b200/csrc/c_api.cu b/faiss_b200/csrc/c_api.cu
--- a/faiss_b200/csrc/c_api.cu
+++ b/faiss_b200/csrc/c_api.cu
@@ -326,6 +326,12 @@
         auto* f = AS<GpuIndexFlat>(p, "GpuIndexFlat");
         out2[0] = f->lastSearchUsedTensorCores;
         out2[1] = f->lastSearchFallbackQueries;
+    }
+    CATCH_AND_HANDLE
+}
+int faiss_GpuIndexFlat_lastSearchCtaGroup(const FaissGpuIndex* p, int* out) {
+    try {
+        *out = AS<GpuIndexFlat>(p, "GpuIndexFlat")->lastSearchTcCtaGroup;
     }
     CATCH_AND_HANDLE
 }
diff --git a/faiss_b200/csrc/flat_tc.cu b/faiss_b200/csrc/flat_tc.cu
--- a/faiss_b200/csrc/flat_tc.cu
+++ b/faiss_b200/csrc/flat_tc.cu
@@ -723,11 +723,11 @@
 
 constexpr int kMaxKB = 4;
 
-SmemPlan planSmem(int KB) {
+SmemPlan planSmem(int KB, bool pair = false) {
     const size_t qtiles = (size_t)2 * KB * kTileM * kKBlock * 2;
     const size_t fixed = 1024  + 512  + qtiles;
     if (KB <= 2) {
-        const size_t stage = (size_t)KB * kTileN * kKBlock * 2;
+        const size_t stage = (size_t)KB * (pair ? kTileN / 2 : kTileN) * kKBlock * 2;
         const size_t budget = 220 * 1024;
         int ys = (int)std::min<size_t>(kMaxYStages, (budget - fixed) / stage);
         return {ys, fixed + ys * stage, 0};
@@ -756,6 +756,52 @@
     CUDA_VERIFY(cudaFuncSetAttribute(kern, cudaFuncAttributeMaxDynamicSharedMemorySize, (int)smem));
     KernelTiming::begin("flat_tc", stream);
     kern<<<grid, tcThreads(parts), smem, stream>>>(mq, my, p);
+    KernelTiming::end("flat_tc", stream);
+    CUDA_CHECK_LAST();
+}
+
+bool tc2ctaEnabled() {
+    static const bool on = !(getenv("FB200_TC_2CTA") && atoi(getenv("FB200_TC_2CTA")) == 0);
+    return on;
+}
+
+auto tc2Kernel() {
+    return tcParts() == 2 ? flat_tc2_kernel<2> : flat_tc2_kernel<4>;
+}
+
+cudaLaunchConfig_t tc2Config(int grid, size_t smem, cudaStream_t stream, cudaLaunchAttribute* attr) {
+    cudaLaunchConfig_t cfg = {};
+    cfg.gridDim = dim3((unsigned)grid);
+    cfg.blockDim = dim3((unsigned)tcThreads(tcParts()));
+    cfg.dynamicSmemBytes = smem;
+    cfg.stream = stream;
+    attr[0].id = cudaLaunchAttributeClusterDimension;
+    attr[0].val.clusterDim.x = 2;
+    attr[0].val.clusterDim.y = 1;
+    attr[0].val.clusterDim.z = 1;
+    cfg.attrs = attr;
+    cfg.numAttrs = 1;
+    return cfg;
+}
+
+int tc2ClusterSlots(size_t smem) {
+    auto kern = tc2Kernel();
+    CUDA_VERIFY(cudaFuncSetAttribute(kern, cudaFuncAttributeMaxDynamicSharedMemorySize, (int)smem));
+    cudaLaunchAttribute attr[1];
+    cudaLaunchConfig_t cfg = tc2Config(2, smem, nullptr, attr);
+    int clusters = 0;
+    CUDA_VERIFY(cudaOccupancyMaxActiveClusters(&clusters, kern, &cfg));
+    FB_THROW_IF_NOT_MSG(clusters > 0, "the 2-CTA tensor-core Flat kernel cannot be resident on this device");
+    return clusters;
+}
+
+void launchTc2(const CUtensorMap& mq, const CUtensorMap& my, const TcParams& p, int grid, size_t smem, cudaStream_t stream) {
+    auto kern = tc2Kernel();
+    CUDA_VERIFY(cudaFuncSetAttribute(kern, cudaFuncAttributeMaxDynamicSharedMemorySize, (int)smem));
+    cudaLaunchAttribute attr[1];
+    cudaLaunchConfig_t cfg = tc2Config(grid, smem, stream, attr);
+    KernelTiming::begin("flat_tc", stream);
+    CUDA_VERIFY(cudaLaunchKernelEx(&cfg, kern, mq, my, p));
     KernelTiming::end("flat_tc", stream);
     CUDA_CHECK_LAST();
 }
@@ -936,12 +982,20 @@
     const int64_t kQFloor = r0Tiles > 64 ? 2048 : 16384;
     const int64_t kQBatch = streaming ? (int64_t)sms * kPairM * 4
                                       : std::min<int64_t>(131072, std::max<int64_t>(kQFloor, (int64_t)kPairM * 1024 / r0Tiles));
+    const bool pair = !streaming && !sp.ksplit && tc2ctaEnabled();
+    const SmemPlan spRun = pair ? planSmem(KB, true) : sp;
+    const int slots = pair ? tc2ClusterSlots(spRun.bytes) : sms;
+    const int unitPairs = pair ? 2 : 1;
+    lastFlatTcCtaGroup() = unitPairs;
+    CUtensorMap mapYRun = pair ? makeTileMap(Y16, n, dpad, kTileN / 2) : mapY;
     for (int64_t qb = 0; qb < nqAll; qb += kQBatch) {
         const int64_t nq = std::min(kQBatch, nqAll - qb);
         const float* Qb = Q + qb * d;
         const int64_t qPairs = ceil_div(nq, kPairM);
-
-        auto q16 = res->temp(device, sizeof(__half) * qPairs * kPairM * dpad);
+        const int64_t qUnits = ceil_div(qPairs, unitPairs);
+        const int64_t qRows = qUnits * unitPairs * kPairM;
+
+        auto q16 = res->temp(device, sizeof(__half) * qRows * dpad);
         auto scal = res->temp(device, sizeof(float) * 4);
         auto eps = res->temp(device, sizeof(float) * nq);
         auto thr = res->temp(device, sizeof(float) * nq);
@@ -951,7 +1005,7 @@
 
         CUDA_VERIFY(cudaMemsetAsync(scal.data, 0, sizeof(float) * 4, stream));
         CUDA_VERIFY(cudaMemsetAsync(flags.data, 0, sizeof(int) * (nq + 1), stream));
-        CUDA_VERIFY(cudaMemsetAsync(q16.data, 0, sizeof(__half) * qPairs * kPairM * dpad, stream));
+        CUDA_VERIFY(cudaMemsetAsync(q16.data, 0, sizeof(__half) * qRows * dpad, stream));
         float* sc = scal.as<float>();
         runAbsMax(Qb, nq * d, sc + 0, stream);
         tc_query_scale_kernel<<<1, 1, 0, stream>>>(sc + 0, yScale, sc + 1, sc + 2);
@@ -991,8 +1045,8 @@
                 int64_t maxS = std::max<int64_t>(1, std::min<int64_t>(512, tiles / 8));
                 for (int64_t S = 1; S <= maxS; S++) {
                     int64_t tps = ceil_div(tiles, S);
-                    int64_t units = qPairs * ceil_div(tiles, tps);
-                    int64_t waves = ceil_div(units, sms);
+                    int64_t units = qUnits * ceil_div(tiles, tps);
+                    int64_t waves = ceil_div(units, slots);
                     double cost = (double)waves * (double)(tps + 6);
                     if (cost < bestCost * 0.999) {
                         bestCost = cost;
@@ -1035,8 +1089,8 @@
             TcParams p{};
             p.slices = r.slices;
             p.qPairs = (int)qPairs;
-            p.numUnits = (int)(qPairs * r.slices);
-            CUtensorMap mapQ = makeTileMap(q16.as<__half>(), qPairs * kPairM, dpad, kTileM);
+            p.numUnits = (int)(qUnits * r.slices);
+            CUtensorMap mapQ = makeTileMap(q16.as<__half>(), qRows, dpad, kTileM);
             p.tileBegin = (int)std::min<int64_t>(r.begin, T);
             p.tileEnd = (int)std::min<int64_t>(r.end, T);
             p.tilesPerSlice = r.tilesPerSlice;
@@ -1046,7 +1100,7 @@
             p.KB = KB;
             p.ksplit = sp.ksplit;
             p.kSteps = (d + 15) / 16;
-            p.yStages = sp.yStages;
+            p.yStages = spRun.yStages;
             p.invScalePtr = sc + 2;
             p.bias = bias;
             p.tileMaxBias = tileMaxBias;
@@ -1060,9 +1114,12 @@
             p.dumpLd = 0;
             p.nq = (int)nq;
             if (p.tileBegin < p.tileEnd) {
-                launchTc<false>(mapQ, mapY, p, std::min(p.numUnits, sms), sp.bytes, stream, streaming);
+                if (pair)
+                    launchTc2(mapQ, mapYRun, p, 2 * std::min(p.numUnits, slots), spRun.bytes, stream);
+                else
+                    launchTc<false>(mapQ, mapY, p, std::min(p.numUnits, sms), sp.bytes, stream, streaming);
             } else {
-                CUDA_VERIFY(cudaMemsetAsync(counts.data, 0, (size_t)p.numUnits * tcSegsPerUnit(parts) * sizeof(int), stream));
+                CUDA_VERIFY(cudaMemsetAsync(counts.data, 0, (size_t)qPairs * r.slices * tcSegsPerUnit(parts) * sizeof(int), stream));
             }
             if (streaming) {
                 const int fw = 8;
@@ -1171,4 +1228,9 @@
     return v;
 }
 
-}
+int& lastFlatTcCtaGroup() {
+    static thread_local int v = 0;
+    return v;
+}
+
+}
diff --git a/faiss_b200/csrc/flat_tc_kernel.cuh b/faiss_b200/csrc/flat_tc_kernel.cuh
--- a/faiss_b200/csrc/flat_tc_kernel.cuh
+++ b/faiss_b200/csrc/flat_tc_kernel.cuh
@@ -125,16 +125,20 @@
     epi_filter32<DUMP, SELF>(p, r1, q, colBase + 32, inv, thr, slack, maxb, buf, cnt, minb);
 }
 
-template <bool DUMP, int DBG, int PARTS, bool SELF = false>
-__global__ void __launch_bounds__(tcThreads(PARTS), 1) flat_tc_kernel(
-        const __grid_constant__ CUtensorMap mapQ,
-        const __grid_constant__ CUtensorMap mapY,
-        const TcParams p) {
+template <bool DUMP, int DBG, int PARTS, bool SELF, int CG>
+__device__ __forceinline__ void flat_tc_body(const CUtensorMap& mapQ, const CUtensorMap& mapY, const TcParams& p) {
+    constexpr bool PAIR = CG == 2;
+    static_assert(!PAIR || (!DUMP && !SELF), "the 2-CTA kernel serves the round-based search only");
     extern __shared__ unsigned char smem_dyn[];
     unsigned char* smem = reinterpret_cast<unsigned char*>(
             (reinterpret_cast<uintptr_t>(smem_dyn) + 1023) & ~uintptr_t(1023));
     const int qBytes = p.KB * kTileM * kKBlock * 2;
-    const int stageBytes = (p.ksplit ? 1 : p.KB) * kTileN * kKBlock * 2;
+    constexpr int kStageRows = PAIR ? kTileN / 2 : kTileN;
+    const int stageBytes = (p.ksplit ? 1 : p.KB) * kStageRows * kKBlock * 2;
+    const uint32_t rank = PAIR ? ptx::cluster_ctarank() : 0u;
+    const int unit0 = PAIR ? (int)(blockIdx.x >> 1) : (int)blockIdx.x;
+    const int unitStep = PAIR ? (int)(gridDim.x >> 1) : (int)gridDim.x;
+    const int qUnits = PAIR ? (p.qPairs + 1) >> 1 : p.qPairs;
     unsigned char* sQ = smem;
     unsigned char* sY = smem + 2 * qBytes;
     uint64_t* bars = reinterpret_cast<uint64_t*>(sY + (size_t)p.yStages * stageBytes);
@@ -162,15 +166,18 @@
         }
         for (int i = 0; i < 2; i++) {
             ptx::mbar_init(&t_full[i], 1);
-            ptx::mbar_init(&t_empty[i], kEpiWarps);
+            ptx::mbar_init(&t_empty[i], PAIR ? 2 * kEpiWarps : kEpiWarps);
         }
         ptx::fence_barrier_init();
     }
     if (warp == 1) {
-        ptx::tmem_alloc<512>(tmem_slot);
+        ptx::tmem_alloc<512, CG>(tmem_slot);
     }
     ptx::tc_fence_before();
-    __syncthreads();
+    if constexpr (PAIR)
+        ptx::cluster_sync();
+    else
+        __syncthreads();
     ptx::tc_fence_after();
     const uint32_t tmem_base = *tmem_slot;
 
@@ -179,13 +186,21 @@
             int ys = 0;
             uint32_t yphase = 0;
             int it = 0;
-            for (int u = blockIdx.x; u < p.numUnits; u += gridDim.x, it++) {
-                const int pair = u % p.qPairs;
-                const int sl = u / p.qPairs;
+            for (int u = unit0; u < p.numUnits; u += unitStep, it++) {
+                const int pair = (u % qUnits) * CG + (int)rank;
+                const int sl = u / qUnits;
                 ptx::mbar_wait(q_empty, (it & 1) ^ 1);
-                ptx::mbar_arrive_expect_tx(q_full, (uint32_t)(2 * qBytes));
-                ptx::tma_load_3d(sQ, &mapQ, q_full, 0, pair * kPairM, 0);
-                ptx::tma_load_3d(sQ + qBytes, &mapQ, q_full, 0, pair * kPairM + kTileM, 0);
+                if constexpr (PAIR) {
+                    const uint32_t qbar = ptx::mapa_shared(q_full, 0);
+                    if (rank == 0)
+                        ptx::mbar_arrive_expect_tx(q_full, (uint32_t)(4 * qBytes));
+                    ptx::tma_load_3d_pair(sQ, &mapQ, qbar, 0, pair * kPairM, 0);
+                    ptx::tma_load_3d_pair(sQ + qBytes, &mapQ, qbar, 0, pair * kPairM + kTileM, 0);
+                } else {
+                    ptx::mbar_arrive_expect_tx(q_full, (uint32_t)(2 * qBytes));
+                    ptx::tma_load_3d(sQ, &mapQ, q_full, 0, pair * kPairM, 0);
+                    ptx::tma_load_3d(sQ + qBytes, &mapQ, q_full, 0, pair * kPairM + kTileM, 0);
+                }
                 const int pb = p.tileBegin + sl * p.tilesPerSlice;
                 const int pe = min(p.tileEnd, pb + p.tilesPerSlice);
                 for (int pp = pb; pp < pe; pp++) {
@@ -193,8 +208,15 @@
                     const int loads = p.ksplit ? 2 * p.KB : 1;
                     for (int l = 0; l < loads; l++) {
                         ptx::mbar_wait(&y_empty[ys], yphase ^ 1);
-                        ptx::mbar_arrive_expect_tx(&y_full[ys], (uint32_t)stageBytes);
-                        ptx::tma_load_3d(sY + (size_t)ys * stageBytes, &mapY, &y_full[ys], 0, t * kTileN, p.ksplit ? l % p.KB : 0);
+                        if constexpr (PAIR) {
+                            if (rank == 0)
+                                ptx::mbar_arrive_expect_tx(&y_full[ys], (uint32_t)(2 * stageBytes));
+                            ptx::tma_load_3d_pair(sY + (size_t)ys * stageBytes, &mapY, ptx::mapa_shared(&y_full[ys], 0), 0,
+                                                  t * kTileN + (int)rank * kStageRows, 0);
+                        } else {
+                            ptx::mbar_arrive_expect_tx(&y_full[ys], (uint32_t)stageBytes);
+                            ptx::tma_load_3d(sY + (size_t)ys * stageBytes, &mapY, &y_full[ys], 0, t * kTileN, p.ksplit ? l % p.KB : 0);
+                        }
                         if (++ys == p.yStages) {
                             ys = 0;
                             yphase ^= 1;
@@ -202,25 +224,35 @@
                     }
                 }
             }
+            if constexpr (PAIR) {
+                for (int s = 0; s < p.yStages; s++) {
+                    ptx::mbar_wait(&y_empty[ys], yphase ^ 1);
+                    if (++ys == p.yStages) {
+                        ys = 0;
+                        yphase ^= 1;
+                    }
+                }
+                ptx::mbar_wait(q_empty, (it & 1) ^ 1);
+            }
         }
     } else if (warp == 1) {
-        if (lane == 0) {
-            constexpr uint32_t idesc = ptx::make_idesc_f16(kTileM, kTileN);
+        if (lane == 0 && rank == 0) {
+            constexpr uint32_t idesc = ptx::make_idesc_f16(CG * kTileM, kTileN);
             int ys = 0;
             uint32_t yphase = 0, tphase = 0;
             int it = 0;
             const uint32_t sQaddr = ptx::smem_u32(sQ);
             const uint32_t sYaddr = ptx::smem_u32(sY);
             const int qkb = kTileM * kKBlock * 2;
-            const int ykb = kTileN * kKBlock * 2;
-            for (int u = blockIdx.x; u < p.numUnits; u += gridDim.x, it++) {
-                const int sl = u / p.qPairs;
+            const int ykb = kStageRows * kKBlock * 2;
+            for (int u = unit0; u < p.numUnits; u += unitStep, it++) {
+                const int sl = u / qUnits;
                 const int pb = p.tileBegin + sl * p.tilesPerSlice;
                 const int pe = min(p.tileEnd, pb + p.tilesPerSlice);
                 ptx::mbar_wait(q_full, it & 1);
                 ptx::tc_fence_after();
                 for (int pp = pb; pp < pe; pp++) {
-                    if (p.ksplit) {
+                    if (!PAIR && p.ksplit) {
 #pragma unroll 1
                         for (int h = 0; h < 2; h++) {
                             ptx::mbar_wait(&t_empty[h], tphase ^ 1);
@@ -261,18 +293,30 @@
                             const int kb = ks >> 2, k4 = ks & 3;
                             uint64_t da = ptx::make_smem_desc_sw128(qaddr + kb * qkb + k4 * 32);
                             uint64_t db = ptx::make_smem_desc_sw128(yaddr + kb * ykb + k4 * 32);
-                            ptx::mma_f16_ss(dcol, da, db, idesc, ks != 0 ? 1u : 0u);
-                        }
-                        ptx::mma_commit(&t_full[h]);
-                    }
-                    ptx::mma_commit(&y_empty[ys]);
+                            if constexpr (PAIR)
+                                ptx::mma_f16_ss_pair(dcol, da, db, idesc, ks != 0 ? 1u : 0u);
+                            else
+                                ptx::mma_f16_ss(dcol, da, db, idesc, ks != 0 ? 1u : 0u);
+                        }
+                        if constexpr (PAIR)
+                            ptx::mma_commit_pair(&t_full[h]);
+                        else
+                            ptx::mma_commit(&t_full[h]);
+                    }
+                    if constexpr (PAIR)
+                        ptx::mma_commit_pair(&y_empty[ys]);
+                    else
+                        ptx::mma_commit(&y_empty[ys]);
                     tphase ^= 1;
                     if (++ys == p.yStages) {
                         ys = 0;
                         yphase ^= 1;
                     }
                 }
-                ptx::mma_commit(q_empty);
+                if constexpr (PAIR)
+                    ptx::mma_commit_pair(q_empty);
+                else
+                    ptx::mma_commit(q_empty);
             }
         }
     } else {
@@ -284,17 +328,19 @@
         const uint32_t lane_acc = tmem_base + ((uint32_t)(quarter * 32) << 16) + (uint32_t)(half * kColsPerThread);
         uint32_t tphase = 0;
         const int permStep = (int)(p.permA % p.numTiles);
-        for (int u = blockIdx.x; u < p.numUnits; u += gridDim.x) {
-            const int pair = u % p.qPairs;
-            const int sl = u / p.qPairs;
+        const uint32_t t_empty_leader = PAIR ? ptx::mapa_shared(t_empty, 0) : 0u;
+        for (int u = unit0; u < p.numUnits; u += unitStep) {
+            const int pair = (u % qUnits) * CG + (int)rank;
+            const int sl = u / qUnits;
             const int q0 = pair * kPairM + row;
             const int q1 = q0 + kTileM;
             float thr0 = (!DUMP && q0 < p.nq) ? p.thr[q0] : CUDART_INF_F;
             float thr1 = (!DUMP && q1 < p.nq) ? p.thr[q1] : CUDART_INF_F;
             const float slack0 = (SELF && q0 < p.nq) ? 2.f * p.eps[q0] : 0.f;
             const float slack1 = (SELF && q1 < p.nq) ? 2.f * p.eps[q1] : 0.f;
-            const long long seg0 = ((long long)u * kPairM + row) * PARTS + half;
-            const long long seg1 = ((long long)u * kPairM + kTileM + row) * PARTS + half;
+            const long long pairUnit = PAIR ? (long long)sl * p.qPairs + pair : (long long)u;
+            const long long seg0 = (pairUnit * kPairM + row) * PARTS + half;
+            const long long seg1 = (pairUnit * kPairM + kTileM + row) * PARTS + half;
             uint2* buf0 = DUMP ? nullptr : p.cand + seg0 * p.cap;
             uint2* buf1 = DUMP ? nullptr : p.cand + seg1 * p.cap;
             int cnt0 = 0, cnt1 = 0;
@@ -338,8 +384,12 @@
                         if (blk == 1) {
                             ptx::tc_fence_before();
                             __syncwarp();
-                            if (lane == 0)
-                                ptx::mbar_arrive(&t_empty[h]);
+                            if (lane == 0) {
+                                if constexpr (PAIR)
+                                    ptx::mbar_arrive_cluster(t_empty_leader + (uint32_t)h * sizeof(uint64_t));
+                                else
+                                    ptx::mbar_arrive(&t_empty[h]);
+                            }
                         }
                         if (DBG == 0) {
                             if constexpr (PARTS == 2)
@@ -360,7 +410,7 @@
                 }
                 tphase ^= 1;
             }
-            if (!DUMP) {
+            if (!DUMP && (!PAIR || pair < p.qPairs)) {
                 p.candCount[seg0] = cnt0;
                 p.candCount[seg1] = cnt1;
             }
@@ -368,12 +418,31 @@
     }
 
     ptx::tc_fence_before();
-    __syncthreads();
+    if constexpr (PAIR)
+        ptx::cluster_sync();
+    else
+        __syncthreads();
     if (warp == 1) {
         ptx::tc_fence_after();
-        ptx::tmem_dealloc<512>(tmem_base);
-    }
-}
-
-}
-}
+        ptx::tmem_dealloc<512, CG>(tmem_base);
+    }
+}
+
+template <bool DUMP, int DBG, int PARTS, bool SELF = false>
+__global__ void __launch_bounds__(tcThreads(PARTS), 1) flat_tc_kernel(
+        const __grid_constant__ CUtensorMap mapQ,
+        const __grid_constant__ CUtensorMap mapY,
+        const TcParams p) {
+    flat_tc_body<DUMP, DBG, PARTS, SELF, 1>(mapQ, mapY, p);
+}
+
+template <int PARTS>
+__global__ void __launch_bounds__(tcThreads(PARTS), 1) flat_tc2_kernel(
+        const __grid_constant__ CUtensorMap mapQ,
+        const __grid_constant__ CUtensorMap mapY,
+        const TcParams p) {
+    flat_tc_body<false, 0, PARTS, false, 2>(mapQ, mapY, p);
+}
+
+}
+}
diff --git a/faiss_b200/csrc/index.cu b/faiss_b200/csrc/index.cu
--- a/faiss_b200/csrc/index.cu
+++ b/faiss_b200/csrc/index.cu
@@ -551,6 +551,7 @@
     auto stream = stream_();
     lastSearchUsedTensorCores = 0;
     lastSearchFallbackQueries = 0;
+    lastSearchTcCtaGroup = 0;
     if (this->ntotal == 0) {
         std::vector<float> hd((size_t)n * k, metric_type == METRIC_L2 ? FLT_MAX : -FLT_MAX);
         std::vector<idx_t> hi((size_t)n * k, -1);
@@ -570,6 +571,7 @@
                 yMaxNorm_, this->ntotal, d, dpad_, k, metric_type, dDev, iDev, stream, nullptr, yHalf_());
         lastSearchUsedTensorCores = 1;
         lastSearchFallbackQueries = lastFlatTcFallbacks();
+    lastSearchTcCtaGroup = lastFlatTcCtaGroup();
     } else {
         runFlatExact(
                 resources_.get(), config_.device, xDev, n, rows_(), this->ntotal, d, k, metric_type, 0, dDev, iDev,
@@ -597,6 +599,7 @@
             dpad_, k, metric_type, dDev, iDev, stream, flatShard, yHalf_());
     lastSearchUsedTensorCores = 1;
     lastSearchFallbackQueries = lastFlatTcFallbacks();
+    lastSearchTcCtaGroup = lastFlatTcCtaGroup();
 }
 
 void GpuIndexFlat::reconstruct(idx_t key, float* out) const {
diff --git a/faiss_b200/csrc/index.h b/faiss_b200/csrc/index.h
--- a/faiss_b200/csrc/index.h
+++ b/faiss_b200/csrc/index.h
@@ -221,6 +221,7 @@
     void replaceVectorsDevice(idx_t n, const float* xDev);
     mutable int lastSearchUsedTensorCores = 0;
     mutable int lastSearchFallbackQueries = 0;
+    mutable int lastSearchTcCtaGroup = 0;
 
    protected:
     bool addImplRequiresIDs_() const override {
diff --git a/faiss_b200/csrc/kernels.h b/faiss_b200/csrc/kernels.h
--- a/faiss_b200/csrc/kernels.h
+++ b/faiss_b200/csrc/kernels.h
@@ -129,6 +129,7 @@
         int yHalf = 0);
 
 int& lastFlatTcFallbacks();
+int& lastFlatTcCtaGroup();
 
 void runFlatTcScoresDebug(
         const __half* Q16,
diff --git a/faiss_b200/csrc/tc_ptx.cuh b/faiss_b200/csrc/tc_ptx.cuh
--- a/faiss_b200/csrc/tc_ptx.cuh
+++ b/faiss_b200/csrc/tc_ptx.cuh
@@ -56,6 +56,23 @@
 __device__ __forceinline__ void mbar_wait(uint64_t* bar, uint32_t parity) {
     while (!mbar_try_wait(bar, parity)) {
     }
+}
+__device__ __forceinline__ void mbar_arrive_cluster(uint32_t cluster_addr) {
+    asm volatile("mbarrier.arrive.shared::cluster.b64 _, [%0];" ::"r"(cluster_addr) : "memory");
+}
+
+__device__ __forceinline__ uint32_t cluster_ctarank() {
+    uint32_t r;
+    asm volatile("mov.u32 %0, %%cluster_ctarank;" : "=r"(r));
+    return r;
+}
+__device__ __forceinline__ void cluster_sync() {
+    asm volatile("barrier.cluster.arrive.release.aligned;\nbarrier.cluster.wait.acquire.aligned;" ::: "memory");
+}
+__device__ __forceinline__ uint32_t mapa_shared(const void* p, uint32_t rank) {
+    uint32_t r;
+    asm volatile("mapa.shared::cluster.u32 %0, %1, %2;" : "=r"(r) : "r"(smem_u32(p)), "r"(rank));
+    return r;
 }
 
 __device__ __forceinline__ void prefetch_tensormap(const void* desc) {
@@ -80,6 +97,25 @@
             : "memory");
 }
 
+__device__ __forceinline__ void tma_load_3d_pair(
+        void* smem_dst,
+        const void* desc,
+        uint32_t bar_cluster,
+        int32_t c0,
+        int32_t c1,
+        int32_t c2) {
+    asm volatile(
+            "cp.async.bulk.tensor.3d.cta_group::2.shared::cluster.global.mbarrier::complete_tx::bytes"
+            " [%0], [%1, {%3, %4, %5}], [%2];"
+            ::"r"(smem_u32(smem_dst)),
+            "l"(reinterpret_cast<uint64_t>(desc)),
+            "r"(bar_cluster),
+            "r"(c0),
+            "r"(c1),
+            "r"(c2)
+            : "memory");
+}
+
 __device__ __forceinline__ void bulk_load_1d(void* smem_dst, const void* gsrc, uint32_t bytes, uint64_t* bar) {
     asm volatile(
             "cp.async.bulk.shared::cluster.global.mbarrier::complete_tx::bytes [%0], [%1], %2, [%3];"
@@ -116,16 +152,26 @@
     return d;
 }
 
-template <uint32_t kCols>
+template <uint32_t kCols, int CG = 1>
 __device__ __forceinline__ void tmem_alloc(uint32_t* smem_dst) {
-    asm volatile("tcgen05.alloc.cta_group::1.sync.aligned.shared::cta.b32 [%0], %1;" ::"r"(smem_u32(smem_dst)),
-                 "n"(kCols)
-                 : "memory");
-    asm volatile("tcgen05.relinquish_alloc_permit.cta_group::1.sync.aligned;" ::: "memory");
-}
-template <uint32_t kCols>
+    if constexpr (CG == 2) {
+        asm volatile("tcgen05.alloc.cta_group::2.sync.aligned.shared::cta.b32 [%0], %1;" ::"r"(smem_u32(smem_dst)),
+                     "n"(kCols)
+                     : "memory");
+        asm volatile("tcgen05.relinquish_alloc_permit.cta_group::2.sync.aligned;" ::: "memory");
+    } else {
+        asm volatile("tcgen05.alloc.cta_group::1.sync.aligned.shared::cta.b32 [%0], %1;" ::"r"(smem_u32(smem_dst)),
+                     "n"(kCols)
+                     : "memory");
+        asm volatile("tcgen05.relinquish_alloc_permit.cta_group::1.sync.aligned;" ::: "memory");
+    }
+}
+template <uint32_t kCols, int CG = 1>
 __device__ __forceinline__ void tmem_dealloc(uint32_t taddr) {
-    asm volatile("tcgen05.dealloc.cta_group::1.sync.aligned.b32 %0, %1;" ::"r"(taddr), "n"(kCols) : "memory");
+    if constexpr (CG == 2)
+        asm volatile("tcgen05.dealloc.cta_group::2.sync.aligned.b32 %0, %1;" ::"r"(taddr), "n"(kCols) : "memory");
+    else
+        asm volatile("tcgen05.dealloc.cta_group::1.sync.aligned.b32 %0, %1;" ::"r"(taddr), "n"(kCols) : "memory");
 }
 __device__ __forceinline__ void tc_fence_before() {
     asm volatile("tcgen05.fence::before_thread_sync;" ::: "memory");
@@ -151,9 +197,34 @@
             "r"(accumulate)
             : "memory");
 }
+__device__ __forceinline__ void mma_f16_ss_pair(
+        uint32_t tmem_d,
+        uint64_t desc_a,
+        uint64_t desc_b,
+        uint32_t idesc,
+        uint32_t accumulate) {
+    asm volatile(
+            "{\n"
+            ".reg .pred p;\n"
+            "setp.ne.b32 p, %4, 0;\n"
+            "tcgen05.mma.cta_group::2.kind::f16 [%0], %1, %2, %3, p;\n"
+            "}\n" ::"r"(tmem_d),
+            "l"(desc_a),
+            "l"(desc_b),
+            "r"(idesc),
+            "r"(accumulate)
+            : "memory");
+}
 __device__ __forceinline__ void mma_commit(uint64_t* bar) {
     asm volatile("tcgen05.commit.cta_group::1.mbarrier::arrive::one.shared::cluster.b64 [%0];" ::"r"(smem_u32(bar))
                  : "memory");
+}
+__device__ __forceinline__ void mma_commit_pair(uint64_t* bar) {
+    asm volatile(
+            "tcgen05.commit.cta_group::2.mbarrier::arrive::one.shared::cluster.multicast::cluster.b64 [%0], %1;"
+            ::"r"(smem_u32(bar)),
+            "h"((uint16_t)0x3)
+            : "memory");
 }
 __device__ __forceinline__ void tmem_ld_32x32b_x32(uint32_t taddr, uint32_t (&r)[32]) {
     asm volatile(
diff --git a/include/faiss_b200_c.h b/include/faiss_b200_c.h
--- a/include/faiss_b200_c.h
+++ b/include/faiss_b200_c.h
@@ -78,6 +78,7 @@
 FB200_API int faiss_GpuIndexFlat_copyTo(const FaissGpuIndex* index, float* xb_out);
 FB200_API int faiss_GpuIndexFlat_setUseTensorCores(FaissGpuIndex* index, int enable);
 FB200_API int faiss_GpuIndexFlat_lastSearchInfo(const FaissGpuIndex* index, int* out2);
+FB200_API int faiss_GpuIndexFlat_lastSearchCtaGroup(const FaissGpuIndex* index, int* out);
 
 FB200_API int faiss_GpuIndexIVF_set_nprobe(FaissGpuIndex* index, size_t nprobe);
 FB200_API size_t faiss_GpuIndexIVF_nprobe(const FaissGpuIndex* index);
```

Result: slower. 422,000, median of 6 (-2.9%).
